# junfeng-chen/position_induced_transformer

Hardware: AMD Instinct MI355X
Metric: PiT fwd+bwd samples/sec on Darcy2D (higher is better)
Workload: dtype f32; 1 GPU; darcy2d 43x43 grid->16x16 latent, pit_fixed hid64 H2 blocks4 loc0.02, RelL2 (train_darcy.py:64-111), fwd+loss+bwd, per-GPU batch 8; per_gpu_batch=8, global_batch=8, parallelism=single, launch=hipgraph, head_scale_route=host

## Files before the change

include/pit_hip.h:

```cpp
#ifndef PIT_HIP_H
#define PIT_HIP_H

#ifdef __cplusplus
extern "C" {
#endif

#define PIT_ABI_VERSION 31
#define PIT_MAX_SPACE_DIM 8
#define PIT_DSCALE_SLOTS 1024

#define PIT_METRIC_EUCLID     0
#define PIT_METRIC_PERIODIC1D 1
#define PIT_METRIC_PERIODIC2D 2

#define PIT_ERR_NULL     -1
#define PIT_ERR_SIZE     -2
#define PIT_ERR_METRIC   -3
#define PIT_ERR_UNSUPPORTED -4

int pit_version(void);
const char* pit_error_string(int code);

#define PIT_MATH_FP32 0
#define PIT_MATH_BF16 1
// ... 33 lines not shown
                   const float* head, int n_head, int head_is_scale,
                   const float* stats, float rank_w, int masked, int self_attn,
                   float* out, long ld_out, long out_bstride, int out_col0, int copy_inputs,
                   float* rowstat, float* scale_out,
                   const int* nbr_idx, const int* nbr_cnt, int nbr_cap, int coord_dims, int math_mode, void* stream);

struct pit_mlp_params_job;

struct pit_block_weights_job {
    const float* mesh; int n_pts, space_dim, metric; float period;
    int n_layers; const float* const* heads; int head_is_scale, n_head;
    float *e, *q, *inv, *rowstat, *scale_out;
};
int pit_posatt_fwd_job(const float* mesh_out, const float* mesh_in, int mesh_batch, int n_out, int n_in,
                       int space_dim, int metric, float period,
                       const float* values, int batch, int dim, long ld_values, long values_bstride,
                       const float* head, int n_head, int head_is_scale,
                       const float* stats, float rank_w, int masked, int self_attn,
                       float* out, long ld_out, long out_bstride, int out_col0, int copy_inputs,
                       float* rowstat, float* scale_out,
                       const int* nbr_idx, const int* nbr_cnt, int nbr_cap, int coord_dims, int math_mode, void* stream,
                       const struct pit_block_weights_job* job);

typedef struct pit_mlp_params_job {
    const float* x; long ldx; int rows, n0, n1, n2; const float* h; int out_gelu;
    const float* d_y; long ld_dy;
    float *d_w1, *d_b1, *d_w2, *d_b2; int accumulate; const float* scratch; int math_mode;
} pit_mlp_params_job;
#define PIT_HEAD_ACCUMULATE 1
#define PIT_HEAD_DEFER      2
#define PIT_HEAD_IS_SCALE   4
int pit_posatt_bwd(const float* mesh_out, const float* mesh_in, int mesh_batch, int n_out, int n_in,
                   int space_dim, int metric, float period,
                   const float* values, int batch, int dim, long ld_values, long values_bstride,
                   const float* head, int n_head, int head_is_scale, const float* scale,
                   const float* rowstat, int masked,
                   const float* d_out, long ld_dout, long dout_bstride, int out_col0,
                   float* d_values, long ld_dvalues, long dvalues_bstride, int add_residual,
                   float* d_head, int accumulate_head, double* workspace,
                   const int* nbr_idx, const int* nbr_cnt, int nbr_cap, int nbr_complete,
                   const int* rev_ptr, const int* rev_row, const pit_mlp_params_job* rider,
                   int coord_dims, int math_mode, void* stream);

int pit_posatt_dmesh(const float* mesh_out, const float* mesh_in, int mesh_batch, int n_out, int n_in,
                     int space_dim, int metric, float period,
                     const float* values, int batch, int dim, long ld_values, long values_bstride,
                     const float* head, int n_head, int head_is_scale, const float* scale,
                     const float* rowstat, int masked,
                     const float* d_out, long ld_dout, long dout_bstride, int out_col0,
                     const int* nbr_idx, const int* nbr_cnt, int nbr_cap, int nbr_complete,
                     const int* rev_ptr, const int* rev_row,
                     float* d_mesh_out, float* d_mesh_in, int accumulate, void* workspace, void* stream);
long pit_posatt_dmesh_workspace(int mesh_batch, int n_out, int n_in, int space_dim, int batch, int n_head);

int pit_posatt_dhead_finish(int n_layers, double* const* workspaces, float* const* d_heads,
                            const float* const* heads, const float* const* scales, const int* n_heads,
                            const int* flags, const pit_mlp_params_job* rider, void* stream);

int pit_block_supported(int n_pts, int n_head, int dim, int batch);

int pit_block_weights(const float* mesh, int n_pts, int space_dim, int metric, float period, int n_layers,
                      const float* const* heads, int head_is_scale, int n_head, float* e, float* q,
                      float* inv, float* rowstat, float* scale_out, void* stream);

int pit_block_fwd(const float* e, const float* inv, int n_pts, int n_head, int dim, int batch, float* xcat,
                  const float* w1, const float* b1, const float* w2, const float* b2, int out_gelu,
                  float* z1, float* h, float* z2, float* y, long ldy, int math_mode, void* stream);

int pit_block_bwd(const float* e, const float* inv, const float* qw, int n_pts, int n_head, int dim, int batch,
                  const float* d_xcat, const float* xcat, double* dscale,
                  const float* w1, const float* w2, const float* z1, const float* z2, int out_gelu, int n0_prev,
                  float* d_xprev, long ld_dxprev, float* scratch_prev,
                  float* d_values, long ld_dvalues,
                  const struct pit_mlp_params_job* rider, const struct pit_mlp_params_job* rider2,
                  int math_mode, void* stream);

#define PIT_SLAB_UNION_MAX 64
typedef struct pit_slab_plan {
    int n_out, n_in, cap, n_slabs, umax;
    const float* stats; float rank_w;
    const int* idx; const int* cnt;
    const float* m; const unsigned short* slot; const int* keys; const int* nkeys;
    int rows;
} pit_slab_plan;
int pit_slab_plan_build(const float* mesh_out, const float* mesh_in, int n_out, int n_in, int space_dim, int metric, float period,
                        const int* nbr_idx, const int* nbr_cnt, int cap, int rows_per_slab, float* m, unsigned short* slot,
                        int* keys, int* nkeys, int* report, void* stream);
int pit_edge_supported(int n_head, int dim, int batch, int rows_per_sample);
int pit_decoder_weights(const pit_slab_plan* plan, const float* head, int head_is_scale, int n_head, int max_union, int max_count,
                        float* pw, float* qw, float* scale_out, const float* w1, float* w1f, int dim, void* stream);
typedef struct pit_decoder_weights_job {
    const pit_slab_plan* plan; const float* head; int head_is_scale, n_head, max_union, max_count;
    float *pw, *qw, *scale_out;
    const float* w1; float* w1f; int dim;
} pit_decoder_weights_job;
int pit_decoder_fwd(const pit_slab_plan* plan, const float* values, long ld_values, long values_bstride, int batch,
                    int n_head, int dim, const float* pw,
                    const float* w1, const float* w1f, const float* b1, const float* w2, const float* b2, int n2,
                    float* x, float* z1, float* h, float* y, float* zero_buf, long zero_n,
                    const float* loss_true, const float* loss_scale, const float* loss_shift, int loss_p, double* loss_part,
                    int max_union, void* stream);
int pit_decoder_bwd(const pit_slab_plan* plan, const float* values, long ld_values, long values_bstride, int batch,
                    int n_head, int dim, const float* pw, const float* qw,
                    const float* w1, const float* w2, int n2, const float* z1,
                    const float* d_y, long ld_dy, float* dz1, float* d_values, long dvalues_bstride, double* dscale,
                    const float* loss_pred, const float* loss_true, const float* loss_scale, const float* loss_shift,
                    const float* loss_seed, int loss_p, const double* loss_part, float* d_pred, float* loss_out,
                    float* norms_out, int max_union, void* stream);
int pit_union_att_supported(int n_head, int dim, int batch, int rows_per_sample);
int pit_union_att_fwd(const pit_slab_plan* plan, const float* values, long ld_values, long values_bstride, int batch,
                      int n_head, int dim, const float* pw, void* out, long ld_out, long out_bstride, int out_bf16,
                      int max_union, void* stream);
int pit_union_att_bwd(const pit_slab_plan* plan, const float* values, long ld_values, long values_bstride, int batch,
                      int n_head, int dim, const float* pw, const float* qw,
                      const void* d_out, long ld_dout, long dout_bstride, int dout_bf16,
                      float* d_values, long ld_dvalues, long dvalues_bstride, double* dscale, int max_union, void* stream);
int pit_fold_supported(int n_head, int dim, int batch, int rows_per_sample, int n_in);
int pit_fold_weights(const pit_slab_plan* plan, const float* head, int head_is_scale, int n_head, int max_union, int max_count,
                     float* pw, float* qw, float* scale_out, unsigned short* pw16, unsigned short* qw16, void* stream);
int pit_fold_att_fwd(const pit_slab_plan* plan, const float* vw, long ld_vw, long vw_bstride, int batch, int n_head, int dim,
                     const void* pw, void* z, long ld_z, long z_bstride, int max_union, int math_mode, void* stream);
int pit_fold_att_bwd(const pit_slab_plan* plan, const float* vw, long ld_vw, long vw_bstride, int batch, int n_head, int dim,
                     const void* pw, const void* qw, const void* dz, long ld_dz, long dz_bstride,
                     float* d_vw, long ld_dvw, long dvw_bstride, double* dscale,
                     float* tiles, const int* rev_ptr, const int* rev_ent, int max_union, int math_mode, void* stream);
int pit_thin_tail_scratch_floats(void);
int pit_thin_tail_fwd(const void* z, long ldz, int rows, int n1, int n2, const float* b1, const float* w2, const float* b2,
                      float* y, long ldy, int math_mode, void* stream);
int pit_thin_tail_bwd(const void* z, long ldz, int rows, int n1, int n2, const float* b1, const float* w2,
                      const float* d_y, long ld_dy, void* dz, long ld_dz, float* d_b1, float* d_w2, float* d_b2,
                      float* scratch, int math_mode, void* stream);
int pit_linear_fwd(const float* x, long ldx, int rows, int n_in, int n_out, const float* w, const float* zero_bias,
                   float* y, long ldy, int math_mode, void* stream);
int pit_linear_bwd(const float* x, long ldx, int rows, int n_in, int n_out, const float* w, const float* d_y, long ld_dy,
                   float* d_x, long ld_dx, float* d_w, int accumulate, int math_mode, void* stream);

struct pit_block_weights_job;
int pit_encoder_fwd(const pit_slab_plan* plan, const float* mesh_in, int space_dim, int coord_dims,
                    const float* values, long ld_values, long values_bstride, int value_dim, int batch,
                    int n_head, int dim, const float* head, int head_is_scale,
                    const float* w1, const float* b1, const float* w2, const float* b2,
                    float* x, float* z1, float* h, float* z2, float* y, long ldy, float* rowstat, float* scale_out,
                    float* clear_buf, long clear_n, const struct pit_block_weights_job* weights,
                    const pit_decoder_weights_job* dec_weights, void* stream);
int pit_encoder_bwd(const pit_slab_plan* plan, const float* mesh_in, int space_dim, int coord_dims,
                    const float* values, long ld_values, long values_bstride, int value_dim, int batch,
                    int n_head, int dim, const float* scale, const float* rowstat,
                    const float* w1, const float* w2, const float* z1, const float* z2,
                    const float* d_y, long ld_dy, float* scratch, double* dscale, void* stream);

int pit_posatt_pre_supported(int n_pts, int n_head, int dim, int batch);
int pit_posatt_pre_fwd(const float* e, const float* rowstat, int n_pts, int n_head, int dim, int batch,
                       const float* values, long ld_values, long values_bstride,
                       float* out, long ld_out, long out_bstride, int out_col0, int copy_inputs, int math_mode, void* stream);
int pit_posatt_pre_bwd(const float* e, const float* q, const float* rowstat, int n_pts, int n_head, int dim, int batch,
                       const float* values, long ld_values, long values_bstride,
                       const float* d_out, long ld_dout, long dout_bstride, int out_col0,
                       float* d_values, long ld_dvalues, long dvalues_bstride, int add_residual,
                       double* workspace, int math_mode, void* stream);

int pit_satt_supported(int n_pts, int n_head, int dim, int batch, int mesh_batch);
int pit_satt_fwd(const float* mesh, int mesh_batch, int n_pts, int space_dim, int metric, float period,
                 const float* values, long ld_values, long values_bstride, int batch, int dim,
                 const float* head, int n_head, int head_is_scale, unsigned short* x16,
                 float* out, long ld_out, long out_bstride, int out_col0, int copy_inputs,
                 float* rowstat, float* scale_out, unsigned short* e_tiles, int x16_ready, void* stream);
int pit_satt_bwd(const float* mesh, int mesh_batch, int n_pts, int space_dim, int metric, float period,
                 int batch, int dim, const float* scale, int n_head, const float* rowstat,
                 const unsigned short* x16, unsigned short* g16,
                 const float* d_out, long ld_dout, long dout_bstride, int out_col0,
                 float* d_values, long ld_dvalues, long dvalues_bstride, int add_residual, double* dscale,
// ... 203 lines not shown
```

position_induced_transformer_amd/_lib.py:

```python
from __future__ import annotations

import ctypes
import os

import torch

_HERE = os.path.dirname(os.path.abspath(__file__))
LIB_PATH = os.environ.get("PIT_LIB_PATH") or os.path.join(_HERE, "csrc", "libpit_hip.so")

_P = ctypes.c_void_p
_I = ctypes.c_int
_L = ctypes.c_long
_F = ctypes.c_float

class MlpParamsJob(ctypes.Structure):
    _fields_ = [("x", _P), ("ldx", _L), ("rows", _I), ("n0", _I), ("n1", _I), ("n2", _I), ("h", _P), ("out_gelu", _I),
                ("d_y", _P), ("ld_dy", _L), ("d_w1", _P), ("d_b1", _P), ("d_w2", _P), ("d_b2", _P),
                ("accumulate", _I), ("scratch", _P), ("math_mode", _I)]


class BlockWeightsJob(ctypes.Structure):
    _fields_ = [("mesh", _P), ("n_pts", _I), ("space_dim", _I), ("metric", _I), ("period", _F),
                ("n_layers", _I), ("heads", _P), ("head_is_scale", _I), ("n_head", _I),
                ("e", _P), ("q", _P), ("inv", _P), ("rowstat", _P), ("scale_out", _P)]


class SlabPlan(ctypes.Structure):
    _fields_ = [("n_out", _I), ("n_in", _I), ("cap", _I), ("n_slabs", _I), ("umax", _I), ("stats", _P), ("rank_w", _F),
                ("idx", _P), ("cnt", _P), ("m", _P), ("slot", _P), ("keys", _P), ("nkeys", _P), ("rows", _I)]


class DecoderWeightsJob(ctypes.Structure):
    _fields_ = [("plan", _P), ("head", _P), ("head_is_scale", _I), ("n_head", _I), ("max_union", _I), ("max_count", _I),
                ("pw", _P), ("qw", _P), ("scale_out", _P), ("w1", _P), ("w1f", _P), ("dim", _I)]


SIGNATURES = {
    "pit_version": [],
    "pit_error_string": [_I],
    "pit_head_scale": [_P, _I, _P, _P],
    "pit_select_fwd": [_P, _P, _I, _I, _I, _I, _I, _F, _I, _I, _P, _P],
    "pit_select_wide_fwd": [_P, _P, _I, _I, _I, _I, _I, _F, _I, _I, _P, _P],
    "pit_plan_fwd": [_P, _P, _I, _I, _I, _I, _I, _F, _I, _P, _I, _P, _P, _P, _P, _P, _I, _P],
    "pit_lists_transpose": [_P, _P, _I, _I, _I, _I, _P, _P, _P, _P],
    "pit_neighbors_fwd": [_P, _P, _I, _I, _I, _I, _I, _F, _P, _I, _P, _P, _P, _P, _P, _P],
    "pit_posatt_fwd": [_P, _P, _I, _I, _I, _I, _I, _F,
                       _P, _I, _I, _L, _L,
                       _P, _I, _I,
                       _P, _F, _I, _I,
                       _P, _L, _L, _I, _I,
                       _P, _P, _P, _P, _I, _I, _I, _P],
    "pit_posatt_fwd_job": [_P, _P, _I, _I, _I, _I, _I, _F,
                           _P, _I, _I, _L, _L,
                           _P, _I, _I,
                           _P, _F, _I, _I,
                           _P, _L, _L, _I, _I,
                           _P, _P, _P, _P, _I, _I, _I, _P, _P],
    "pit_posatt_bwd": [_P, _P, _I, _I, _I, _I, _I, _F,
                       _P, _I, _I, _L, _L,
                       _P, _I, _I, _P,
                       _P, _I,
                       _P, _L, _L, _I,
                       _P, _L, _L, _I,
                       _P, _I, _P, _P, _P, _I, _I, _P, _P, _P, _I, _I, _P],
    "pit_posatt_dmesh": [_P, _P, _I, _I, _I, _I, _I, _F,
                         _P, _I, _I, _L, _L,
                         _P, _I, _I, _P,
                         _P, _I,
                         _P, _L, _L, _I,
                         _P, _P, _I, _I, _P, _P,
                         _P, _P, _I, _P, _P],
    "pit_posatt_dmesh_workspace": [_I, _I, _I, _I, _I, _I],
    "pit_posatt_dhead_finish": [_I, _P, _P, _P, _P, _P, _P, _P, _P],
    "pit_block_supported": [_I, _I, _I, _I],
    "pit_block_weights": [_P, _I, _I, _I, _F, _I, _P, _I, _I, _P, _P, _P, _P, _P, _P],
    "pit_block_fwd": [_P, _P, _I, _I, _I, _I, _P, _P, _P, _P, _P, _I, _P, _P, _P, _P, _L, _I, _P],
    "pit_slab_plan_build": [_P, _P, _I, _I, _I, _I, _F, _P, _P, _I, _I, _P, _P, _P, _P, _P, _P],
    "pit_fold_supported": [_I, _I, _I, _I, _I],
    "pit_fold_weights": [_P, _P, _I, _I, _I, _I, _P, _P, _P, _P, _P, _P],
    "pit_fold_att_fwd": [_P, _P, _L, _L, _I, _I, _I, _P, _P, _L, _L, _I, _I, _P],
    "pit_fold_att_bwd": [_P, _P, _L, _L, _I, _I, _I, _P, _P, _P, _L, _L, _P, _L, _L, _P, _P, _P, _P, _I, _I, _P],
    "pit_thin_tail_scratch_floats": [],
    "pit_thin_tail_fwd": [_P, _L, _I, _I, _I, _P, _P, _P, _P, _L, _I, _P],
    "pit_thin_tail_bwd": [_P, _L, _I, _I, _I, _P, _P, _P, _L, _P, _L, _P, _P, _P, _P, _I, _P],
    "pit_satt_supported": [_I, _I, _I, _I, _I],
    "pit_satt_fwd": [_P, _I, _I, _I, _I, _F, _P, _L, _L, _I, _I, _P, _I, _I, _P, _P, _L, _L, _I, _I, _P, _P, _P, _I, _P],
    "pit_satt_bwd": [_P, _I, _I, _I, _I, _F, _I, _I, _P, _I, _P, _P, _P, _P, _L, _L, _I, _P, _L, _L, _I, _P, _P, _I, _P, _P],
    "pit_satt_tiles_elems": [_I],
    "pit_mlp_chain_supported": [_I, _I, _I, _I],
    "pit_mlp_chain_fwd": [_P, _L, _I, _I, _I, _P, _P, _P, _P, _P, _P, _P, _P, _L, _P, _P],
    "pit_mlp_chain_bwd": [_I, _I, _I, _P, _P, _P, _P, _P, _L, _P, _L, _P, _P, _P, _I, _I, _P],
    "pit_cast_bf16_multi": [_I, _P, _P, _P, _P],
    "pit_linear_fwd": [_P, _L, _I, _I, _I, _P, _P, _P, _L, _I, _P],
    "pit_linear_bwd": [_P, _L, _I, _I, _I, _P, _P, _L, _P, _L, _P, _I, _I, _P],
    "pit_edge_supported": [_I, _I, _I, _I],
    "pit_decoder_weights": [_P, _P, _I, _I, _I, _I, _P, _P, _P, _P, _P, _I, _P],
    "pit_decoder_fwd": [_P, _P, _L, _L, _I, _I, _I, _P, _P, _P, _P, _P, _P, _I, _P, _P, _P, _P, _P, _L,
                        _P, _P, _P, _I, _P, _I, _P],
    "pit_decoder_bwd": [_P, _P, _L, _L, _I, _I, _I, _P, _P, _P, _P, _I, _P, _P, _L, _P, _P, _L, _P,
                        _P, _P, _P, _P, _P, _I, _P, _P, _P, _P, _I, _P],
    "pit_union_att_supported": [_I, _I, _I, _I],
    "pit_union_att_fwd": [_P, _P, _L, _L, _I, _I, _I, _P, _P, _L, _L, _I, _I, _P],
    "pit_union_att_bwd": [_P, _P, _L, _L, _I, _I, _I, _P, _P, _P, _L, _L, _I, _P, _L, _L, _P, _I, _P],
    "pit_encoder_fwd": [_P, _P, _I, _I, _P, _L, _L, _I, _I, _I, _I, _P, _I, _P, _P, _P, _P,
                        _P, _P, _P, _P, _P, _L, _P, _P, _P, _L, _P, _P, _P],
    "pit_encoder_bwd": [_P, _P, _I, _I, _P, _L, _L, _I, _I, _I, _I, _P, _P, _P, _P, _P, _P, _P, _L, _P, _P, _P],
    "pit_posatt_pre_supported": [_I, _I, _I, _I],
    "pit_posatt_pre_fwd": [_P, _P, _I, _I, _I, _I, _P, _L, _L, _P, _L, _L, _I, _I, _I, _P],
    "pit_posatt_pre_bwd": [_P, _P, _P, _I, _I, _I, _I, _P, _L, _L, _P, _L, _L, _I, _P, _L, _L, _I, _P, _I, _P],
    "pit_block_bwd": [_P, _P, _P, _I, _I, _I, _I, _P, _P, _P, _P, _P, _P, _P, _I, _I, _P, _L, _P, _P, _L, _P, _P, _I, _P],
    "pit_mlp_bf16_io_supported": [_I, _I, _I, _I, _I],
    "pit_mlp_fwd": [_P, _L, _I, _I, _I, _I, _P, _P, _P, _P, _I, _P, _P, _P, _P, _L, _I, _P],
    "pit_mlp_bwd": [_P, _L, _I, _I, _I, _I, _P, _P, _P, _P, _P, _I, _P, _L,
                    _P, _L, _P, _P, _P, _P, _I, _P, _I, _P],
    "pit_mlp_bwd_data": [_I, _I, _I, _I, _P, _P, _P, _P, _I, _P, _L, _P, _L, _P, _I, _P],
    "pit_mlp_bwd_params": [_P, _L, _I, _I, _I, _I, _P, _I, _P, _L, _P, _P, _P, _P, _I, _P, _I, _P],
    "pit_mlp_bwd_params_ordered": [_P, _L, _I, _I, _I, _I, _P, _I, _P, _L, _P, _P, _P, _P, _I, _P, _P, _P],
    "pit_mlp_bwd_params_ordered_workspace": [_I, _I, _I, _I],
    "pit_mlp_bwd_params_ordered_mfma": [_P, _L, _I, _I, _I, _I, _P, _I, _P, _L, _P, _P, _P, _P, _I, _P, _P, _P],
    "pit_mlp_bwd_params_ordered_mfma_workspace": [_I, _I, _I, _I],
    "pit_lists_sort_ranges": [_P, _P, _I, _I, _L, _P, _P],
    "pit_posatt_overflow_dv_ordered": [_P, _P, _I, _I, _I, _I, _I, _F, _I, _I, _P, _I, _I, _P, _P,
                                       _P, _L, _L, _I, _P, _L, _L, _P, _I, _I, _P],
    "pit_mlp_bwd_params_deferrable": [_I, _I, _I, _I, _I, _L],
    "pit_rel_lp_loss_fwd": [_P, _P, _P, _P, _I, _I, _I, _I, _P, _P, _P, _P],
    "pit_rel_lp_loss_fwd_grad": [_P, _P, _P, _P, _I, _I, _I, _I, _P, _P, _P, _P, _P, _P, _L, _P],
    "pit_rel_lp_loss_fwd_grad_ordered": [_P, _P, _P, _P, _I, _I, _I, _I, _P, _P, _P, _P, _P, _P, _L, _P],
    "pit_rel_lp_loss_bwd": [_P, _P, _P, _P, _I, _I, _I, _I, _P, _P, _P, _P, _P],
    "pit_plan_ragged_fwd": [_P, _P, _I, _I, _I, _I, _P, _P, _F, _I, _P, _P, _I, _P, _P, _P],
    "pit_posatt_ragged_fwd": [_P, _P, _I, _I, _I, _I, _P, _P,
                              _P, _I, _L, _L,
                              _P, _I, _I,
                              _P, _P, _I,
                              _P, _L, _L, _I, _I,
                              _P, _P, _P, _P, _I, _I, _P],
    "pit_posatt_ragged_bwd": [_P, _P, _I, _I, _I, _I, _P, _P,
                              _P, _I, _L, _L,
                              _P, _I, _I, _P,
                              _P, _I,
                              _P, _L, _L, _I,
                              _P, _L, _L, _I,
                              _P, _I, _P, _P, _P, _I, _P, _P, _I, _P],
    "pit_plan_ragged_strided_fwd": [_P, _P, _I, _I, _I, _I, _L, _L, _P, _P, _F, _I, _P, _P, _I, _P, _P, _P],
    "pit_posatt_ragged_strided_fwd": [_P, _P, _I, _I, _I, _I, _L, _L, _P, _P,
                                      _P, _I, _L, _L,
                                      _P, _I, _I,
                                      _P, _P, _I,
                                      _P, _L, _L, _I, _I,
                                      _P, _P, _P, _P, _I, _I, _P],
    "pit_posatt_ragged_strided_bwd": [_P, _P, _I, _I, _I, _I, _L, _L, _P, _P,
                                      _P, _I, _L, _L,
                                      _P, _I, _I, _P,
                                      _P, _I,
                                      _P, _L, _L, _I,
                                      _P, _L, _L, _I,
                                      _P, _I, _P, _P, _P, _I, _P, _P, _I, _P],
    "pit_rel_lp_loss_ragged_fwd": [_P, _P, _P, _I, _I, _I, _I, _P, _P, _P],
    "pit_rel_lp_loss_ragged_bwd": [_P, _P, _P, _I, _I, _I, _I, _P, _P, _P, _P],
    "pit_distmat_select_fwd": [_P, _L, _L, _I, _I, _I, _I, _I, _P, _P],
    "pit_distmat_fwd": [_P, _L, _L, _I, _I,
# ... 63 lines not shown
```

position_induced_transformer_amd/csrc/pit_edge.hip:

```cpp
#include "pit_common.h"
#include "pit_gemm_rd.h"
#include "pit_block_dev.h"

#ifndef PIT_EDGE_MAX_ROWS
#define PIT_EDGE_MAX_ROWS (1 << 20)
#endif
#ifndef PIT_EDGE_DBG
#define PIT_EDGE_DBG 0
#endif

namespace {

#if PIT_EDGE_DBG & 0x100
__device__ unsigned long long pit_edge_stamps[4][16];
#define ESTAMP(k_, i_) do { if (blockIdx.x == 300 && threadIdx.x == 0) pit_edge_stamps[k_][i_] = __builtin_amdgcn_s_memtime(); } while (0)
#else
#define ESTAMP(k_, i_) do { } while (0)
#endif

constexpr int ER = 16;
constexpr int EU = PIT_SLAB_UNION_MAX;

__device__ __forceinline__ __amdgpu_buffer_rsrc_t wide_rsrc(const void* p) { return make_rsrc(p, 0x7ffffff0u); }
constexpr unsigned OOB = 0x7ffffff8u;
__device__ __forceinline__ float ldg_if(const float* p, long i, bool ok) {
    return buf_load(wide_rsrc(p), ok ? (unsigned)(i * 4) : OOB);
}
__device__ __forceinline__ int ldi_if(const int* p, long i, bool ok) {
    return __builtin_amdgcn_raw_buffer_load_b32(wide_rsrc(p), (int)(ok ? (unsigned)(i * 4) : OOB), 0, 0);
}
__device__ __forceinline__ float4 ldg4_if(const float* p, long i, bool ok) {
    float v[4];
    buf_load4(wide_rsrc(p), ok ? (unsigned)(i * 4) : OOB, v);
    return make_float4(v[0], v[1], v[2], v[3]);
}

__device__ __forceinline__ float pow_abs_p(float x, int p) {
    const float ax = fabsf(x);
    return p == 1 ? ax : ax * ax;
}

struct SlabBuildArgs {
    const float *mesh_out, *mesh_in;
    int n_out, n_in, sdim, used, periodic; float period;
    const int *idx, *cnt; int cap, umax;
    float* m; unsigned short* slot; int* keys; int* nkeys; int* report;
    int er;
};

__global__ __launch_bounds__(256) void slab_plan_kernel(SlabBuildArgs a) {
    __shared__ unsigned bm[512];
    __shared__ int pref[513];
    const int tid = threadIdx.x, slab = blockIdx.x;
    const int nwords = (a.n_in + 31) >> 5;
    for (int w = tid; w < nwords; w += 256) bm[w] = 0u;
    __syncthreads();
    const int er = a.er;
    const int total = er * a.cap;
    for (int e = tid; e < total; e += 256) {
        const int r = e / a.cap, i = e - r * a.cap;
        const int row = slab * er + r;
        float mv = 0.0f;
        if (row < a.n_out) {
            const int c = a.cnt[row];
            if (c > a.cap && i == 0) atomicMax(a.report + 1, 1);
            if (i == 0) atomicMax(a.report + 2, min(c, a.cap));
            if (i < min(c, a.cap)) {
                const int j = a.idx[(long)row * a.cap + i];
                const float* xo = a.mesh_out + (long)row * a.sdim;
                const float* xi = a.mesh_in + (long)j * a.sdim;
                mv = sq_dist3(xo[0], a.used > 1 ? xo[1] : 0.0f, a.used > 2 ? xo[2] : 0.0f,
                              xi[0], a.used > 1 ? xi[1] : 0.0f, a.used > 2 ? xi[2] : 0.0f, a.periodic != 0, a.period);
                atomicOr(&bm[j >> 5], 1u << (j & 31));
            }
        }
        a.m[(long)(slab * er + r) * a.cap + i] = mv;
    }
    __syncthreads();
    if (tid == 0) {
        int run = 0;
        for (int w = 0; w < nwords; ++w) { pref[w] = run; run += __popc(bm[w]); }
        pref[nwords] = run;
        a.nkeys[slab] = run;
        atomicMax(a.report, run);
    }
    __syncthreads();
    const int nk = pref[nwords];
    for (int w = tid; w < nwords; w += 256) {
        unsigned bits = bm[w];
        int s = pref[w];
        while (bits) {
            const int bpos = __ffs(bits) - 1;
            bits &= bits - 1u;
            if (s < a.umax) a.keys[(long)slab * a.umax + s] = w * 32 + bpos;
            ++s;
        }
    }
    for (int s = nk + tid; s < a.umax; s += 256) a.keys[(long)slab * a.umax + s] = 0;
    for (int e = tid; e < total; e += 256) {
        const int r = e / a.cap, i = e - r * a.cap;
        const int row = slab * er + r;
        int s = 0;
        if (row < a.n_out && i < min(a.cnt[row], a.cap)) {
            const int j = a.idx[(long)row * a.cap + i];
            s = pref[j >> 5] + __popc(bm[j >> 5] & ((1u << (j & 31)) - 1u));
        }
        a.slot[(long)(slab * er + r) * a.cap + i] = (unsigned short)min(s, 65535);
    }
}

template <int H>
__device__ __forceinline__ void head_scales(const float (&raw)[H], int is_scale, float (&c)[H]) {
#pragma unroll
    for (int h = 0; h < H; ++h) c[h] = is_scale ? raw[h] : head_scale_from_lmda(raw[h]);
}

struct DecWArgs {
    pit_slab_plan p;
    const float* head; int head_is_scale, n_head, um, lpr;
    float *pw, *qw, *scale_out;
    unsigned short *pw16, *qw16;
    const float* w1; float* w1f; int dim;
    int rb;
};
__device__ __forceinline__ float seg_sum_rt(float v, int lpr) {
    v += dpp_f<0xB1, 0xf>(v);
    v += dpp_f<0x4E, 0xf>(v);
    v += dpp_f<0x124, 0xf>(v);
    v += dpp_f<0x128, 0xf>(v);
    if (lpr >= 32) v += __shfl_xor(v, 16, 64);
    if (lpr >= 64) v += __shfl_xor(v, 32, 64);
    return v;
}
__device__ __forceinline__ void dec_weights_body(const DecWArgs& g, int slab, float* tile) {
    const pit_slab_plan& p = g.p;
    const int tid = threadIdx.x, lane = tid & 63, wave = tid >> 6;
    const int H = g.n_head, um = g.um, lpr = g.lpr;
    const int per = H * ER * um;
    for (int e = tid; e < 2 * per; e += 256) tile[e] = 0.0f;
    float c[2];
#pragma unroll
    for (int h = 0; h < 2; ++h) {
        const float raw = g.head[h < H ? h : 0];
        c[h] = g.head_is_scale ? raw : head_scale_from_lmda(raw);
    }
    __syncthreads();
    const int rpw = 64 / lpr;
    for (int r0 = 0; r0 < ER; r0 += 4 * rpw) {
        const int row_l = r0 + wave * rpw + lane / lpr, i = lane % lpr, n = slab * ER + row_l;
        const int craw = ldi_if(p.cnt, n, n < p.n_out);
        const long off = (long)(slab * ER + row_l) * p.cap + (i < p.cap ? i : 0);
        const float m = p.m[off];
        const int slot = p.slot[off];
        const bool valid = i < min(craw, p.cap);
        const int nn = n < p.n_out ? n : p.n_out - 1;
        const float mk = p.stats[nn], mk1 = p.stats[p.n_out + nn], mmin = p.stats[2 * (long)p.n_out + nn];
        for (int h = 0; h < H; ++h) {
            const float T = quantile_lerp(__fmul_rn(c[h], mk), __fmul_rn(c[h], mk1), p.rank_w);
            const float smin = __fmul_rn(c[h], mmin);
            const float sv = __fmul_rn(m, c[h]);
            const bool keep = valid && sv <= T;
            const float pv = keep ? __expf(smin - sv) : 0.0f;
            const float rs = seg_sum_rt(pv, lpr), qsum = seg_sum_rt(pv * m, lpr);
            const float inv = rs > 0.0f ? 1.0f / rs : 0.0f;
            if (valid && slot < um) {
                tile[(h * ER + row_l) * um + slot] = pv * inv;
                tile[per + (h * ER + row_l) * um + slot] = pv * inv * (m - qsum * inv);
            }
        }
    }
    __syncthreads();
    {
        const int gpb = g.rb / ER, blk = slab / gpb, cg = slab - blk * gpb, perh = ER * um;
        for (int e = 4 * tid; e < per; e += 4 * 256) {
            const int h = e / perh, r = e - h * perh;
            const long o = ((long)(blk * H + h) * g.rb + cg * ER) * um + r;
            const float4 pv4 = *reinterpret_cast<const float4*>(tile + e), qv4 = *reinterpret_cast<const float4*>(tile + per + e);
            *reinterpret_cast<float4*>(g.pw + o) = pv4;
            if (g.qw) *reinterpret_cast<float4*>(g.qw + o) = qv4;
            if (g.pw16) *reinterpret_cast<uint2*>(g.pw16 + o) = make_uint2((unsigned)f_to_bf16(pv4.x) | ((unsigned)f_to_bf16(pv4.y) << 16), (unsigned)f_to_bf16(pv4.z) | ((unsigned)f_to_bf16(pv4.w) << 16));
            if (g.qw16) *reinterpret_cast<uint2*>(g.qw16 + o) = make_uint2((unsigned)f_to_bf16(qv4.x) | ((unsigned)f_to_bf16(qv4.y) << 16), (unsigned)f_to_bf16(qv4.z) | ((unsigned)f_to_bf16(qv4.w) << 16));
        }
    }
    if (slab == 0 && tid < H && g.scale_out) g.scale_out[tid] = c[tid];
    if (g.w1f) {
        const int K0 = H * g.dim, KS = K0 / 16, n4 = g.dim * K0 / 4;
        for (int o = slab * 256 + tid; o < n4; o += p.n_slabs * (g.rb / ER) * 256) {
            const int ln = o & 63, s_ = (o >> 6) % KS, w = (o >> 6) / KS;
            reinterpret_cast<float4*>(g.w1f)[o] =
                *reinterpret_cast<const float4*>(g.w1 + (long)(16 * w + (ln & 15)) * K0 + 16 * s_ + 4 * (ln >> 4));
        }
    }
}
__global__ __launch_bounds__(256) void decoder_weights_kernel(DecWArgs g) {
    __shared__ __attribute__((aligned(16))) float tile[2 * 2 * ER * EU];
    dec_weights_body(g, blockIdx.x, tile);
}

struct DecFwdArgs {
    pit_slab_plan p;
    const float* values; long ld_values, values_bstride; int batch;
    const float* pw;
    const float *w1, *b1, *w2, *b2; int n2;
    const float* w1f;
    float *x, *z1, *h, *y;
    float* zero_buf; long zero_n;
    const float *tru, *lscale, *lshift; int loss_p; double* lpart;
    int um;
};

template <int D>
__device__ __forceinline__ void union_keys(const pit_slab_plan& p, int slab, int tid, int nkup, int (&key)[EU / 16]) {
    const int r0 = tid / (D / 4);
    const int* kp = p.keys + (long)slab * p.umax + r0;
#pragma unroll
    for (int u = 0; u < EU / 16; ++u) key[u] = kp[16 * u];
}
template <int D>
__device__ __forceinline__ void gather_union(const float* __restrict__ vb, long ldv, const int (&key)[EU / 16], int nk, int nkup, int tid,
                                             float4 (&uv)[EU / 16]) {
    const int r0 = tid / (D / 4), q = tid % (D / 4);
#pragma unroll
    for (int u = 0; u < EU / 16; ++u)
        uv[u] = (PIT_EDGE_DBG & 2) ? make_float4(0.f, 0.f, 0.f, 0.f) : ldg4_if(vb, (long)key[u] * ldv + 4 * q, r0 + 16 * u < nk);
}
template <int D>
__device__ __forceinline__ void park_union(float* ut, int nkup, int tid, const float4 (&uv)[EU / 16]) {
    const int r0 = tid / (D / 4), q = tid % (D / 4);
#pragma unroll
    for (int u = 0; u < EU / 16; ++u)
        if (16 * u < nkup) *reinterpret_cast<float4*>(ut + (r0 + 16 * u) * (D + 4) + 4 * q) = uv[u];
}

constexpr int WCP = (2 * ER * EU / 4 + 255) / 256;
template <int NT>
__device__ __forceinline__ void wtile_request(const float* tile, int npc, int tid, float4 (&cp)[WCP * 256 / NT]) {
#pragma unroll
    for (int u = 0; u < WCP * 256 / NT; ++u) cp[u] = ldg4_if(tile, 4L * (tid + u * NT), tid + u * NT < npc);
}
template <int NT>
__device__ __forceinline__ void wtile_park(float* lds, int um, int npc, int tid, const float4 (&cp)[WCP * 256 / NT]) {
#pragma unroll
    for (int u = 0; u < WCP * 256 / NT; ++u) {
        const int e = tid + u * NT;
        if (e < npc) *reinterpret_cast<float4*>(lds + ((4 * e) / um) * (um + 4) + (4 * e) % um) = cp[u];
    }
}
template <int D>
__device__ __forceinline__ f32x4_t tile_times_union(const float* wrow, int up, const float* ut, int nkup, int wave, int l15, int kq) {
    f32x4_t a0 = {0.f, 0.f, 0.f, 0.f}, a1 = {0.f, 0.f, 0.f, 0.f};
    for (int s = 0; s < nkup / 16; ++s) {
        const float4 a = *reinterpret_cast<const float4*>(wrow + l15 * up + 16 * s + 4 * kq);
        const float* bp = ut + (16 * s + 4 * kq) * (D + 4) + 16 * wave + l15;
        a0 = mfma_16x16x4(a.x, bp[0], a0);
        a1 = mfma_16x16x4(a.y, bp[D + 4], a1);
        a0 = mfma_16x16x4(a.z, bp[2 * (D + 4)], a0);
        a1 = mfma_16x16x4(a.w, bp[3 * (D + 4)], a1);
    }
    f32x4_t r;
#pragma unroll
    for (int i = 0; i < 4; ++i) r[i] = a0[i] + a1[i];
    return r;
}

template <int H, int D, bool LOSS>
__global__ __launch_bounds__(4 * D) void decoder_fwd_kernel(DecFwdArgs g) {
    constexpr int NT = 4 * D, NW = D / 16, K0 = H * D, KS = K0 / 16, XP = K0 + 4, HP = D + 4;
    extern __shared__ __attribute__((aligned(16))) float smem[];
    const int UP = g.um + 4;
    float* pt = smem;
    float* ut = pt + H * ER * UP;
    float* xs = ut + g.um * (D + 4);
    float* hs = xs + ER * XP;
    float* w2s = hs + ER * HP;
    const int tid = threadIdx.x, lane = tid & 63, wave = tid >> 6;
    const int l15 = lane & 15, kq = lane >> 4;
    const pit_slab_plan& p = g.p;
    int b, slab;
    if (!slab_of_xcd(blockIdx.x, g.batch, p.n_slabs, b, slab)) return;
    const int nk = min(p.nkeys[slab], EU), nkup = (nk + 15) & ~15;
    const long row0 = (long)b * p.n_out + slab * ER;
    const int c1 = wave * 16 + l15;
    ESTAMP(0, 0);
    int key[EU / 16];
    union_keys<D>(p, slab, tid, nkup, key);
    const int npc = H * ER * g.um / 4;
    float4 pcp[WCP * 256 / NT];
    wtile_request<NT>(g.pw + (long)slab * H * ER * g.um, npc, tid, pcp);
    float4 bv[KS];
    const float* w1base = g.w1f ? g.w1f : g.w1;
#pragma unroll
    for (int s = 0; s < KS; ++s)
        bv[s] = (PIT_EDGE_DBG & 1) ? make_float4(1.f, 2.f, 3.f, 4.f)
              : *reinterpret_cast<const float4*>(w1base + (g.w1f ? ((wave * KS + s) * 64 + lane) * 4 : c1 * K0 + 16 * s + 4 * kq));
    const float bias1 = g.b1[c1];
    const float w2r = ldg_if(g.w2, tid, tid < g.n2 * D);
    const float b2r = ldg_if(g.b2, tid, tid < g.n2);
    float l_t0 = 0.0f, l_sc0 = 1.0f, l_sh0 = 0.0f;
    if (LOSS) {
        const int n = slab * ER + l15;
        const bool rv = n < p.n_out;
        l_t0 = ldg_if(g.tru, (row0 + l15) * g.n2, rv);
        const bool aff = rv && g.lscale != nullptr;
        l_sc0 = ldg_if(g.lscale, (long)n * g.n2, aff);
        l_sh0 = ldg_if(g.lshift, (long)n * g.n2, aff);
    }
    float4 uv[EU / 16];
    gather_union<D>(g.values + (long)b * g.values_bstride, g.ld_values, key, nk, nkup, tid, uv);
    __builtin_amdgcn_sched_barrier(0);
    ESTAMP(0, 1);
    w2s[tid] = w2r;
    if (tid < 4) w2s[4 * D + tid] = b2r;
    wtile_park<NT>(pt, g.um, npc, tid, pcp);
    ESTAMP(0, 2);
    park_union<D>(ut, nkup, tid, uv);
    ESTAMP(0, 3);
    __syncthreads();
    ESTAMP(0, 4);
#pragma unroll
    for (int h = 0; h < H; ++h) {
        const f32x4_t o = tile_times_union<D>(pt + h * ER * UP, UP, ut, nkup, wave, l15, kq);
#pragma unroll
        for (int i = 0; i < 4; ++i) xs[(4 * kq + i) * XP + h * D + c1] = o[i];
    }
    ESTAMP(0, 5);
    __syncthreads();
    ESTAMP(0, 6);
    if (g.x && !(PIT_EDGE_DBG & 4)) {
#pragma unroll
        for (int u = 0; u < (ER * K0 / 4 + NT - 1) / NT; ++u) {
            const int e = tid + u * NT, r = e / (K0 / 4), q = e % (K0 / 4);
            if (e < ER * K0 / 4 && slab * ER + r < p.n_out)
                *reinterpret_cast<float4*>(g.x + (row0 + r) * K0 + 4 * q) = *reinterpret_cast<const float4*>(xs + r * XP + 4 * q);
        }
    }
    {
        f32x4_t a0 = {0.f, 0.f, 0.f, 0.f}, a1 = {0.f, 0.f, 0.f, 0.f};
#pragma unroll
        for (int s = 0; s < KS; ++s) {
            const float4 a = *reinterpret_cast<const float4*>(xs + l15 * XP + 16 * s + 4 * kq);
            a0 = mfma_16x16x4(a.x, bv[s].x, a0);
            a1 = mfma_16x16x4(a.y, bv[s].y, a1);
            a0 = mfma_16x16x4(a.z, bv[s].z, a0);
            a1 = mfma_16x16x4(a.w, bv[s].w, a1);
        }
#pragma unroll
        for (int i = 0; i < 4; ++i) {
            const int r = 4 * kq + i;
            const float z = a0[i] + a1[i] + bias1;
            hs[r * HP + c1] = gelu_erf(z);
            if (g.z1 && slab * ER + r < p.n_out && !(PIT_EDGE_DBG & 4)) g.z1[(row0 + r) * D + c1] = z;
        }
    }
    ESTAMP(0, 7);
    __syncthreads();
    ESTAMP(0, 8);
    if (g.h && !(PIT_EDGE_DBG & (4 | 1024))) {
        const int r = tid / (D / 4), q = tid % (D / 4);
        if (slab * ER + r < p.n_out)
            *reinterpret_cast<float4*>(g.h + (row0 + r) * D + 4 * q) = *reinterpret_cast<const float4*>(hs + r * HP + 4 * q);
    }
    if (wave != 0) {
        if (g.zero_buf) {
            const long wgs = (long)g.batch * p.n_slabs, me = (long)b * p.n_slabs + slab;
            const long per = ((g.zero_n + wgs - 1) / wgs + 3) & ~3L;
            const long beg = me * per, end = min(g.zero_n, beg + per);
            for (long e = beg + 4 * (tid - 64); e < end; e += 4 * (NT - 64)) {
                if (e + 4 <= end) *reinterpret_cast<float4*>(g.zero_buf + e) = make_float4(0.f, 0.f, 0.f, 0.f);
                else for (long q = e; q < end; ++q) g.zero_buf[q] = 0.0f;
            }
        }
        return;
    }
    const int n = slab * ER + l15;
    const bool rv = n < p.n_out;
#pragma unroll
    for (int o = 0; o < 4; ++o) {
        if (o >= g.n2) break;
        float part = 0.0f;
#pragma unroll
        for (int k = 0; k < D / 4; k += 4) {
            const float4 a = *reinterpret_cast<const float4*>(hs + l15 * HP + kq * (D / 4) + k);
            const float4 w = *reinterpret_cast<const float4*>(w2s + o * D + kq * (D / 4) + k);
            part += (a.x * w.x + a.y * w.y) + (a.z * w.z + a.w * w.w);
        }
        part += __shfl_xor(part, 16, 64);
        part += __shfl_xor(part, 32, 64);
        const float pred = part + w2s[4 * D + o];
        if (kq == 0 && rv) g.y[(row0 + l15) * g.n2 + o] = pred;
        if (LOSS) {
            double num = 0.0, den = 0.0;
            float t = l_t0, sc = l_sc0, sh = l_sh0;
            if (o > 0) {
                t = ldg_if(g.tru, (row0 + l15) * g.n2 + o, rv);
                sc = ldg_if(g.lscale, (long)n * g.n2 + o, rv && g.lscale != nullptr);
                sh = ldg_if(g.lshift, (long)n * g.n2 + o, rv && g.lscale != nullptr);
            }
            if (kq == 0 && rv) {
                const float q = g.lscale ? pred * sc + sh : pred;
                num = (double)pow_abs_p(t - q, g.loss_p);
                den = (double)pow_abs_p(t, g.loss_p);
            }
            num = wave_sum_d(num);
            den = wave_sum_d(den);
            if (lane == 0) {
                double* dst = g.lpart + (((long)b * g.n2 + o) * p.n_slabs + slab) * 2;
                dst[0] = num; dst[1] = den;
            }
        }
    }
    ESTAMP(0, 9);
}

struct DecBwdArgs {
    pit_slab_plan p;
    const float* values; long ld_values, values_bstride; int batch;
    const float *pw, *qw;
    const float *w1, *w2; int n2;
    const float* z1;
    const float* d_y; long ld_dy;
    float* dz1;
    float* d_values; long dvalues_bstride;
    double* dscale;
    const float *pred, *tru, *lscale, *lshift, *gseed; int loss_p; const double* lpart; float* d_pred; float* loss_out; float* norms_out;
    int um;
};

__device__ __forceinline__ void series_norms(const double* lpart, int b, int o, int n2, int slabs, int p, int lane, double& nn, double& dn) {
    double num = 0.0, den = 0.0;
    const double* src = lpart + ((long)b * n2 + o) * slabs * 2;
    for (int s = lane; s < slabs; s += 64) { num += src[2 * s]; den += src[2 * s + 1]; }
    num = wave_sum_d(num);
    den = wave_sum_d(den);
    nn = p == 1 ? num : sqrt(num);
    dn = p == 1 ? den : sqrt(den);
}

template <int H, int D, bool LOSS>
__global__ __launch_bounds__(4 * D) void decoder_bwd_kernel(DecBwdArgs g) {
    constexpr int NT = 4 * D, NW = D / 16, K0 = H * D, S1 = D / 16, XP = K0 + 4, P1 = D + 4;
    extern __shared__ __attribute__((aligned(16))) float smem[];
    const int UP = g.um + 4;
    float* ps_ = smem;
    float* qs = ps_ + H * ER * UP;
    float* ut = qs + H * ER * UP;
    float* ds1 = ut + g.um * (D + 4);
    float* dxs = ds1 + ER * P1;
    double* wred = reinterpret_cast<double*>(dxs + ER * XP);
    int* keys_s = reinterpret_cast<int*>(wred + NW * H);
    const int tid = threadIdx.x, lane = tid & 63, wave = tid >> 6;
    const int l15 = lane & 15, kq = lane >> 4;
    const pit_slab_plan& p = g.p;
    int b, slab;
    if (!slab_of_xcd(blockIdx.x, g.batch, p.n_slabs, b, slab)) return;
    const int nk = min(p.nkeys[slab], EU), nkup = (nk + 15) & ~15;
    const long row0 = (long)b * p.n_out + slab * ER;
    const int c1 = wave * 16 + l15;

    ESTAMP(1, 0);
    int key[EU / 16];
    union_keys<D>(p, slab, tid, nkup, key);
    const int akey = p.keys[(long)slab * p.umax + (tid & (EU - 1))];
    const int npc = H * ER * g.um / 4;
    float4 pcp[WCP * 256 / NT], qcp[WCP * 256 / NT];
    wtile_request<NT>(g.pw + (long)slab * H * ER * g.um, npc, tid, pcp);
    wtile_request<NT>(g.qw + (long)slab * H * ER * g.um, npc, tid, qcp);
    const int ec = tid % D;
    float z1v[4], dyv[4], prv[4], trv[4], lsc[4], lsh[4];
    const float w2c0 = g.w2[ec];
#pragma unroll
    for (int u = 0; u < 4; ++u) {
        const int r = (tid + u * NT) / D;
        const bool ok = slab * ER + r < p.n_out;
        z1v[u] = ldg_if(g.z1, (row0 + r) * D + ec, ok);
        dyv[u] = 0.0f; prv[u] = 0.0f; trv[u] = 0.0f; lsc[u] = 1.0f; lsh[u] = 0.0f;
        if (!LOSS) {
            dyv[u] = ldg_if(g.d_y, (row0 + r) * g.ld_dy, ok);
        } else {
            prv[u] = ldg_if(g.pred, (row0 + r) * g.n2, ok);
            trv[u] = ldg_if(g.tru, (row0 + r) * g.n2, ok);
            const bool aff = ok && g.lscale != nullptr;
            const float a = ldg_if(g.lscale, (long)(slab * ER + r) * g.n2, aff), bq = ldg_if(g.lshift, (long)(slab * ER + r) * g.n2, aff);
            lsc[u] = g.lscale ? a : 1.0f;
            lsh[u] = bq;
        }
    }
    float4 np4[4];
#pragma unroll
    for (int cq = 0; cq < 4; ++cq)
        np4[cq] = ldg4_if(reinterpret_cast<const float*>(g.lpart) + (long)b * g.n2 * p.n_slabs * 4, 4L * (lane + 64 * cq),
                          LOSS && lane + 64 * cq < p.n_slabs);
    float4 uv[EU / 16];
    gather_union<D>(g.values + (long)b * g.values_bstride, g.ld_values, key, nk, nkup, tid, uv);
    __builtin_amdgcn_sched_barrier(0);
    ESTAMP(1, 1);
    if (tid < EU) keys_s[tid] = akey;
    float nrm0 = 0.0f, nrm1 = 1.0f;
    if (LOSS) {
        {
            double num = 0.0, den = 0.0;
#pragma unroll
            for (int cq = 0; cq < 4; ++cq) {
                num += __hiloint2double(__float_as_int(np4[cq].y), __float_as_int(np4[cq].x));
                den += __hiloint2double(__float_as_int(np4[cq].w), __float_as_int(np4[cq].z));
            }
            const double* src = g.lpart + (long)b * g.n2 * p.n_slabs * 2;
            for (int sl = lane + 256; sl < p.n_slabs; sl += 64) { num += src[2 * sl]; den += src[2 * sl + 1]; }
            num = wave_sum_d(num);
            den = wave_sum_d(den);
            nrm0 = (float)(g.loss_p == 1 ? num : sqrt(num));
            nrm1 = (float)(g.loss_p == 1 ? den : sqrt(den));
        }
        if (blockIdx.x == 0 && wave == NW - 1) {
            double tot = 0.0;
            for (int bb = 0; bb < g.batch; ++bb)
                for (int o = 0; o < g.n2; ++o) {
                    double nn, dn;
                    series_norms(g.lpart, bb, o, g.n2, p.n_slabs, g.loss_p, lane, nn, dn);
                    tot += (double)((float)(nn / dn / g.n2));
                    if (lane == 0 && g.norms_out) {
                        g.norms_out[((long)bb * g.n2 + o) * 2] = (float)nn;
                        g.norms_out[((long)bb * g.n2 + o) * 2 + 1] = (float)dn;
                    }
                }
            if (lane == 0) *g.loss_out = (float)tot;
        }
    }
    ESTAMP(1, 2);
    wtile_park<NT>(ps_, g.um, npc, tid, pcp);
    wtile_park<NT>(qs, g.um, npc, tid, qcp);
    ESTAMP(1, 3);
    const float gs = (LOSS && g.gseed) ? g.gseed[0] : 1.0f;
    auto dpred = [&](float pr, float tr, float sc, float sh, float nn, float dn) {
        const float d = pr * sc + sh - tr;
        float dnorm;
        if (g.loss_p == 1) dnorm = (d > 0.0f) ? 1.0f : (d < 0.0f ? -1.0f : 0.0f);
        else dnorm = (nn > 0.0f) ? d / nn : 0.0f;
        return gs * dnorm * sc / (dn * g.n2);
    };
    float acc[4];
#pragma unroll
    for (int u = 0; u < 4; ++u) {
        const int r = (tid + u * NT) / D;
        const bool ok = slab * ER + r < p.n_out;
        float v = dyv[u];
        if (LOSS) {
            v = dpred(prv[u], trv[u], lsc[u], lsh[u], nrm0, nrm1);
            if (ec == 0 && ok) g.d_pred[(row0 + r) * g.n2] = v;
        }
        acc[u] = v * w2c0;
    }
    for (int o = 1; o < g.n2; ++o) {
        const float w2o = g.w2[(long)o * D + ec];
        float nn = 0.0f, dn = 1.0f;
        if (LOSS) {
            double a, bq;
            series_norms(g.lpart, b, o, g.n2, p.n_slabs, g.loss_p, lane, a, bq);
            nn = (float)a; dn = (float)bq;
        }
#pragma unroll
        for (int u = 0; u < 4; ++u) {
            const int r = (tid + u * NT) / D;
            const bool ok = slab * ER + r < p.n_out;
            float v;
            if (!LOSS) {
                v = ldg_if(g.d_y, (row0 + r) * g.ld_dy + o, ok);
            } else {
                const long e = (long)(slab * ER + r) * g.n2 + o;
                const bool aff = ok && g.lscale != nullptr;
                const float a = ldg_if(g.lscale, e, aff), bq = ldg_if(g.lshift, e, aff);
                v = dpred(ldg_if(g.pred, (row0 + r) * g.n2 + o, ok), ldg_if(g.tru, (row0 + r) * g.n2 + o, ok),
                          g.lscale ? a : 1.0f, bq, nn, dn);
                if (ec == o && ok) g.d_pred[(row0 + r) * g.n2 + o] = v;
            }
            acc[u] += v * w2o;
        }
    }
#pragma unroll
    for (int u = 0; u < 4; ++u) {
        const int r = (tid + u * NT) / D;
        const bool ok = slab * ER + r < p.n_out;
        const float v = ok ? acc[u] * ((PIT_EDGE_DBG & 32) ? 1.0f : gelu_erf_grad(z1v[u])) : 0.0f;
        ds1[r * P1 + ec] = v;
        if (ok && !(PIT_EDGE_DBG & 512)) g.dz1[(row0 + r) * D + ec] = v;
    }
    ESTAMP(1, 4);
    park_union<D>(ut, nkup, tid, uv);
    ESTAMP(1, 5);
    float w1v[H][S1][4];
#pragma unroll
    for (int hh = 0; hh < H; ++hh)
#pragma unroll
        for (int s = 0; s < S1; ++s)
#pragma unroll
            for (int e = 0; e < 4; ++e) w1v[hh][s][e] = (PIT_EDGE_DBG & 8) ? 0.5f
                : g.w1[(long)(16 * s + 4 * kq + e) * K0 + hh * D + c1];
    __syncthreads();
    ESTAMP(1, 6);
#pragma unroll
    for (int hh = 0; hh < H; ++hh) {
        f32x4_t o0 = {0.f, 0.f, 0.f, 0.f}, o1 = {0.f, 0.f, 0.f, 0.f};
#pragma unroll
        for (int s = 0; s < S1; ++s) {
            const float4 a = *reinterpret_cast<const float4*>(ds1 + l15 * P1 + 16 * s + 4 * kq);
            o0 = mfma_16x16x4(a.x, w1v[hh][s][0], o0);
            o1 = mfma_16x16x4(a.y, w1v[hh][s][1], o1);
            o0 = mfma_16x16x4(a.z, w1v[hh][s][2], o0);
            o1 = mfma_16x16x4(a.w, w1v[hh][s][3], o1);
        }
#pragma unroll
        for (int i = 0; i < 4; ++i) dxs[(4 * kq + i) * XP + hh * D + c1] = o0[i] + o1[i];
    }
    ESTAMP(1, 7);
    __syncthreads();
    ESTAMP(1, 8);
    for (int mt = 0; mt < nkup / 16; ++mt) {
        f32x4_t a0 = {0.f, 0.f, 0.f, 0.f}, a1 = {0.f, 0.f, 0.f, 0.f};
#pragma unroll
        for (int h = 0; h < H; ++h) {
            const float* ap = ps_ + (h * ER + 4 * kq) * UP + 16 * mt + l15;
            const float* bp = dxs + (4 * kq) * XP + h * D + c1;
            a0 = mfma_16x16x4(ap[0], bp[0], a0);
            a1 = mfma_16x16x4(ap[UP], bp[XP], a1);
            a0 = mfma_16x16x4(ap[2 * UP], bp[2 * XP], a0);
            a1 = mfma_16x16x4(ap[3 * UP], bp[3 * XP], a1);
        }
#pragma unroll
        for (int i = 0; i < 4; ++i) {
            const int s = 16 * mt + 4 * kq + i;
            if (s < nk && !(PIT_EDGE_DBG & 16)) atomicAdd(g.d_values + (long)b * g.dvalues_bstride + (long)keys_s[s] * D + c1, a0[i] + a1[i]);
        }
    }
    ESTAMP(1, 9);
    if (g.dscale && !(PIT_EDGE_DBG & 128)) {
#pragma unroll
        for (int h = 0; h < H; ++h) {
            const f32x4_t qu = tile_times_union<D>(qs + h * ER * UP, UP, ut, nkup, wave, l15, kq);
            double part = 0.0;
#pragma unroll
            for (int i = 0; i < 4; ++i) part += (double)qu[i] * (double)dxs[(4 * kq + i) * XP + h * D + c1];
            part = wave_sum_d(part);
            if (lane == 0) wred[wave * H + h] = part;
        }
        __syncthreads();
        if (tid < H) {
            double tot = 0.0;
            for (int w = 0; w < NW; ++w) tot += wred[w * H + tid];
            atomicAdd(g.dscale + (long)tid * PIT_DSCALE_SLOTS + ((int)blockIdx.x & (PIT_DSCALE_SLOTS - 1)), -tot);
        }
    }
    ESTAMP(1, 10);
}

struct EncArgs {
    pit_slab_plan p;
    const float* mesh_in; int sdim, kd;
    const float* values; long ld_values, values_bstride; int dv, batch;
    const float* head; int head_is_scale;
    const float *w1, *b1, *w2, *b2;
    float* x;
    float *z1, *h, *z2, *y; long ldy;
    float* rowstat; float* scale_out;
    float* clear_buf; long clear_n;
    int n_att;
    const float* d_y; long ld_dy; float* scratch; double* dscale;
};

// ... 344 lines not shown
    const int l15 = lane & 15, kq = lane >> 4;
    const pit_slab_plan& p = g.p;
    const int chunks = g.dim / D;
    const int chunk = (int)blockIdx.x % chunks;
    int b, slab;
    if (!slab_of_xcd((int)blockIdx.x / chunks, g.batch, p.n_slabs, b, slab)) return;
    const int nk = min(p.nkeys[slab], EU), nkup = (nk + 15) & ~15;
    const int c1 = wave * 16 + l15;
    int key[EU / 16];
    union_keys<D>(p, slab, tid, nkup, key);
    const int akey = p.keys[(long)slab * p.umax + (tid & (EU - 1))];
    const int npc = H * ER * g.um / 4;
    float4 pcp[WCP], qcp[WCP];
    wtile_request<NT>(g.pw + (long)slab * H * ER * g.um, npc, tid, pcp);
    wtile_request<NT>(g.qw + (long)slab * H * ER * g.um, npc, tid, qcp);
    float4 dv[H * ER * D / 4 / NT];
#pragma unroll
    for (int u = 0; u < H * ER * D / 4 / NT; ++u) {
        const int e = tid + u * NT, r = e / (H * D / 4), q4 = e % (H * D / 4), h = q4 / (D / 4), q = q4 % (D / 4);
        const int n = slab * ER + r;
        const long o = (long)b * g.dout_bstride + (long)n * g.ld_dout + (long)h * g.dim + chunk * D + 4 * q;
        if (g.dout16) {
            const __amdgpu_buffer_rsrc_t r16 = wide_rsrc(g.d_out);
            const unsigned off = n < p.n_out ? (unsigned)(o * 2) : OOB;
            const unsigned lo = (unsigned)__builtin_amdgcn_raw_buffer_load_b32(r16, (int)off, 0, 0);
            const unsigned hi = (unsigned)__builtin_amdgcn_raw_buffer_load_b32(r16, (int)(n < p.n_out ? off + 4u : OOB), 0, 0);
            dv[u] = make_float4(__uint_as_float(lo << 16), __uint_as_float(lo & 0xffff0000u), __uint_as_float(hi << 16),
                                __uint_as_float(hi & 0xffff0000u));
        } else {
            dv[u] = ldg4_if(reinterpret_cast<const float*>(g.d_out), o, n < p.n_out);
        }
    }
    float4 uv[EU / 16];
    gather_union<D>(g.values + (long)b * g.values_bstride + chunk * D, g.ld_values, key, nk, nkup, tid, uv);
    __builtin_amdgcn_sched_barrier(0);
    if (tid < EU) keys_s[tid] = akey;
    wtile_park<NT>(ps_, g.um, npc, tid, pcp);
    wtile_park<NT>(qs, g.um, npc, tid, qcp);
#pragma unroll
    for (int u = 0; u < H * ER * D / 4 / NT; ++u) {
        const int e = tid + u * NT, r = e / (H * D / 4), q4 = e % (H * D / 4);
        *reinterpret_cast<float4*>(dxs + r * XP + 4 * q4) = dv[u];
    }
    park_union<D>(ut, nkup, tid, uv);
    __syncthreads();
    if (g.d_values) {
        for (int mt = 0; mt < nkup / 16; ++mt) {
            f32x4_t a0 = {0.f, 0.f, 0.f, 0.f}, a1 = {0.f, 0.f, 0.f, 0.f};
#pragma unroll
            for (int h = 0; h < H; ++h) {
                const float* ap = ps_ + (h * ER + 4 * kq) * UP + 16 * mt + l15;
                const float* bp = dxs + (4 * kq) * XP + h * D + c1;
                a0 = mfma_16x16x4(ap[0], bp[0], a0);
                a1 = mfma_16x16x4(ap[UP], bp[XP], a1);
                a0 = mfma_16x16x4(ap[2 * UP], bp[2 * XP], a0);
                a1 = mfma_16x16x4(ap[3 * UP], bp[3 * XP], a1);
            }
#pragma unroll
            for (int i = 0; i < 4; ++i) {
                const int sl = 16 * mt + 4 * kq + i;
                if (sl < nk) atomicAdd(g.d_values + (long)b * g.dvalues_bstride + (long)keys_s[sl] * g.ld_dvalues + chunk * D + c1, a0[i] + a1[i]);
            }
        }
    }
    if (g.dscale) {
#pragma unroll
        for (int h = 0; h < H; ++h) {
            const f32x4_t qu = tile_times_union<D>(qs + h * ER * UP, UP, ut, nkup, wave, l15, kq);
            double part = 0.0;
#pragma unroll
            for (int i = 0; i < 4; ++i) part += (double)qu[i] * (double)dxs[(4 * kq + i) * XP + h * D + c1];
            part = wave_sum_d(part);
            if (lane == 0) wred[wave * H + h] = part;
        }
        __syncthreads();
        if (tid < H) {
            double tot = 0.0;
            for (int w = 0; w < NW; ++w) tot += wred[w * H + tid];
            atomicAdd(g.dscale + (long)tid * PIT_DSCALE_SLOTS + ((int)blockIdx.x & (PIT_DSCALE_SLOTS - 1)), -tot);
        }
    }
}

bool plan_ok(const pit_slab_plan* p, bool needs_union) {
    if (!p || !p->stats || !p->idx || !p->cnt || !p->m) return false;
    if (p->rows != ER) return false;
    if (p->n_out <= 0 || p->n_in <= 0 || p->cap <= 0 || p->cap > 64 || p->n_slabs != (p->n_out + ER - 1) / ER) return false;
    if (needs_union && (!p->slot || !p->keys || !p->nkeys || p->umax != EU)) return false;
    return true;
}
bool hid_ok(int n_head, int dim) { return (n_head == 1 || n_head == 2) && (dim == 32 || dim == 64); }

int union_slots(int max_union) { return max_union <= 32 ? 32 : (max_union <= 48 ? 48 : 64); }
template <int H, int D>
size_t dec_fwd_smem(int um) { return (size_t)(H * ER * (um + 4) + um * (D + 4) + ER * (H * D + 4) + ER * (D + 4) + 4 * D + 4) * 4; }
template <int H, int D>
size_t dec_bwd_smem(int um) {
    return (size_t)(2 * H * ER * (um + 4) + um * (D + 4) + ER * (D + 4) + ER * (H * D + 4)) * 4 + (size_t)(D / 16) * H * 8 + EU * 4;
}

}

extern "C" int pit_edge_supported(int n_head, int dim, int batch, int rows_per_sample) {
    if (!hid_ok(n_head, dim) || batch <= 0 || rows_per_sample <= 0) return 0;
    const long rows = (long)batch * rows_per_sample;
    return rows >= 256 && rows <= PIT_EDGE_MAX_ROWS;
}

extern "C" int pit_slab_plan_build(const float* mesh_out, const float* mesh_in, int n_out, int n_in, int space_dim, int metric,
                                   float period, const int* nbr_idx, const int* nbr_cnt, int cap, int rows_per_slab, float* m,
                                   unsigned short* slot, int* keys, int* nkeys, int* report, void* stream) {
    if (!mesh_out || !mesh_in || !nbr_idx || !nbr_cnt || !m || !slot || !keys || !nkeys || !report) return PIT_ERR_NULL;
    if (n_out <= 0 || n_in <= 0 || n_in > 16384 || space_dim < 1 || space_dim > 3 || cap <= 0) return PIT_ERR_SIZE;
    if (rows_per_slab != 16 && rows_per_slab != 64 && rows_per_slab != 128 && rows_per_slab != 256) return PIT_ERR_SIZE;
    if (metric < PIT_METRIC_EUCLID || metric > PIT_METRIC_PERIODIC2D) return PIT_ERR_METRIC;
    SlabBuildArgs a;
    a.mesh_out = mesh_out; a.mesh_in = mesh_in; a.n_out = n_out; a.n_in = n_in; a.sdim = space_dim;
    a.used = (metric == PIT_METRIC_PERIODIC1D) ? 1 : space_dim;
    a.periodic = metric != PIT_METRIC_EUCLID; a.period = period;
    a.idx = nbr_idx; a.cnt = nbr_cnt; a.cap = cap; a.umax = EU;
    a.m = m; a.slot = slot; a.keys = keys; a.nkeys = nkeys; a.report = report; a.er = rows_per_slab;
    hipLaunchKernelGGL(slab_plan_kernel, dim3((unsigned)((n_out + rows_per_slab - 1) / rows_per_slab)), dim3(256), 0, (hipStream_t)stream, a);
    PIT_CHECK_LAUNCH();
    return 0;
}

#define PIT_EDGE_DISPATCH(H_, D_, CALL_)                                         \
    do {                                                                         \
        if ((H_) == 1 && (D_) == 32) { CALL_(1, 32); }                           \
        else if ((H_) == 1) { CALL_(1, 64); }                                    \
        else if ((D_) == 32) { CALL_(2, 32); }                                   \
        else { CALL_(2, 64); }                                                   \
    } while (0)

namespace {
int fill_dec_weights(DecWArgs& g, const pit_slab_plan* plan, const float* head, int head_is_scale, int n_head, int max_union,
                     int max_count, float* pw, float* qw, float* scale_out, const float* w1, float* w1f, int dim) {
    if (!plan_ok(plan, true) || !head || !pw) return PIT_ERR_NULL;
    if ((w1 == nullptr) != (w1f == nullptr)) return PIT_ERR_NULL;
    if (w1f && (dim < 16 || dim % 16 != 0 || !aligned16(w1) || !aligned16(w1f))) return PIT_ERR_SIZE;
    g.w1 = w1; g.w1f = w1f; g.dim = dim; g.rb = ER;
    if ((n_head != 1 && n_head != 2) || max_union < 1 || max_union > EU || max_count < 1 || max_count > 64) return PIT_ERR_UNSUPPORTED;
    if (!aligned16(pw) || (qw && !aligned16(qw))) return PIT_ERR_SIZE;
    g.p = *plan; g.head = head; g.head_is_scale = head_is_scale; g.n_head = n_head; g.um = union_slots(max_union);
    g.lpr = max_count <= 16 ? 16 : (max_count <= 32 ? 32 : 64);
    g.pw = pw; g.qw = qw; g.scale_out = scale_out;
    return 0;
}
}

extern "C" int pit_decoder_weights(const pit_slab_plan* plan, const float* head, int head_is_scale, int n_head, int max_union,
                                   int max_count, float* pw, float* qw, float* scale_out, const float* w1, float* w1f, int dim,
                                   void* stream) {
    DecWArgs g = DecWArgs();
    if (int rc = fill_dec_weights(g, plan, head, head_is_scale, n_head, max_union, max_count, pw, qw, scale_out, w1, w1f, dim)) return rc;
    hipLaunchKernelGGL(decoder_weights_kernel, dim3((unsigned)plan->n_slabs), dim3(256), 0, (hipStream_t)stream, g);
    PIT_CHECK_LAUNCH();
    return 0;
}

extern "C" int pit_fold_weights(const pit_slab_plan* plan, const float* head, int head_is_scale, int n_head, int max_union,
                                int max_count, float* pw, float* qw, float* scale_out, unsigned short* pw16, unsigned short* qw16,
                                void* stream) {
    if (!plan || !plan->stats || !plan->idx || !plan->cnt || !plan->m || !plan->slot || !plan->keys || !plan->nkeys || !head || !pw)
        return PIT_ERR_NULL;
    if ((plan->rows != 64 && plan->rows != 128 && plan->rows != 256) || plan->umax != EU || plan->cap <= 0 || plan->cap > 64 ||
        plan->n_slabs != (plan->n_out + plan->rows - 1) / plan->rows) return PIT_ERR_SIZE;
    if ((n_head != 1 && n_head != 2) || max_union < 1 || max_union > EU || max_count < 1 || max_count > 64) return PIT_ERR_UNSUPPORTED;
    if (!aligned16(pw) || (qw && !aligned16(qw))) return PIT_ERR_SIZE;
    DecWArgs g = DecWArgs();
    g.p = *plan; g.head = head; g.head_is_scale = head_is_scale; g.n_head = n_head; g.um = union_slots(max_union);
    g.lpr = max_count <= 16 ? 16 : (max_count <= 32 ? 32 : 64);
    g.pw = pw; g.qw = qw; g.scale_out = scale_out; g.rb = plan->rows; g.pw16 = pw16; g.qw16 = qw16;
    hipLaunchKernelGGL(decoder_weights_kernel, dim3((unsigned)(plan->n_slabs * (plan->rows / ER))), dim3(256), 0, (hipStream_t)stream, g);
    PIT_CHECK_LAUNCH();
    return 0;
}

extern "C" int pit_decoder_fwd(const pit_slab_plan* plan, const float* values, long ld_values, long values_bstride, int batch,
                               int n_head, int dim, const float* pw,
                               const float* w1, const float* w1f, const float* b1, const float* w2, const float* b2, int n2,
                               float* x, float* z1, float* h, float* y, float* zero_buf, long zero_n,
                               const float* loss_true, const float* loss_scale, const float* loss_shift, int loss_p, double* loss_part,
                               int max_union, void* stream) {
    if (max_union < 1 || max_union > EU) return PIT_ERR_UNSUPPORTED;
    if (w1f && !aligned16(w1f)) return PIT_ERR_SIZE;
    if (!plan_ok(plan, true) || !values || !pw || !w1 || !b1 || !w2 || !b2 || !y) return PIT_ERR_NULL;
    if (!hid_ok(n_head, dim) || n2 < 1 || n2 > 4 || batch <= 0) return PIT_ERR_UNSUPPORTED;
    if ((z1 == nullptr) != (h == nullptr)) return PIT_ERR_NULL;
    if (ld_values % 4 || values_bstride % 4 || !aligned16(values) || !aligned16(w1) || !aligned16(pw) || (zero_buf && !aligned16(zero_buf)))
        return PIT_ERR_SIZE;
    if (loss_part && (!loss_true || (loss_p != 1 && loss_p != 2) || (loss_scale == nullptr) != (loss_shift == nullptr))) return PIT_ERR_UNSUPPORTED;
    DecFwdArgs g;
    g.p = *plan; g.values = values; g.ld_values = ld_values; g.values_bstride = values_bstride; g.batch = batch;
    g.pw = pw; g.w1 = w1; g.w1f = w1f; g.b1 = b1; g.w2 = w2; g.b2 = b2; g.n2 = n2;
    g.x = x; g.z1 = z1; g.h = h; g.y = y; g.zero_buf = zero_buf; g.zero_n = zero_buf ? zero_n : 0;
    g.tru = loss_true; g.lscale = loss_scale; g.lshift = loss_shift; g.loss_p = loss_p; g.lpart = loss_part;
    g.um = union_slots(max_union);
    const dim3 grid((unsigned)slab_grid(batch, plan->n_slabs));
    hipStream_t s = (hipStream_t)stream;
#define PIT_DF(H_, D_)                                                                                                                \
    do {                                                                                                                              \
        if (loss_part) hipLaunchKernelGGL((decoder_fwd_kernel<H_, D_, true>), grid, dim3(4 * D_), (dec_fwd_smem<H_, D_>(g.um)), s, g); \
        else hipLaunchKernelGGL((decoder_fwd_kernel<H_, D_, false>), grid, dim3(4 * D_), (dec_fwd_smem<H_, D_>(g.um)), s, g);          \
    } while (0)
    PIT_EDGE_DISPATCH(n_head, dim, PIT_DF);
#undef PIT_DF
    PIT_CHECK_LAUNCH();
    return 0;
}

extern "C" int pit_decoder_bwd(const pit_slab_plan* plan, const float* values, long ld_values, long values_bstride, int batch,
                               int n_head, int dim, const float* pw, const float* qw,
                               const float* w1, const float* w2, int n2, const float* z1,
                               const float* d_y, long ld_dy, float* dz1, float* d_values, long dvalues_bstride, double* dscale,
                               const float* loss_pred, const float* loss_true, const float* loss_scale, const float* loss_shift,
                               const float* loss_seed, int loss_p, const double* loss_part, float* d_pred, float* loss_out,
                               float* norms_out, int max_union, void* stream) {
    if (max_union < 1 || max_union > EU) return PIT_ERR_UNSUPPORTED;
    if (!plan_ok(plan, true) || !values || !pw || !qw || !w1 || !w2 || !z1 || !dz1 || !d_values) return PIT_ERR_NULL;
    if (!hid_ok(n_head, dim) || n2 < 1 || n2 > 4 || batch <= 0) return PIT_ERR_UNSUPPORTED;
    if (!d_y && (!loss_pred || !loss_true || !loss_part || !d_pred || !loss_out || (loss_p != 1 && loss_p != 2) ||
                 (loss_scale == nullptr) != (loss_shift == nullptr))) return PIT_ERR_NULL;
    if (d_y && ld_dy < n2) return PIT_ERR_SIZE;
    if (ld_values % 4 || values_bstride % 4 || !aligned16(values) || !aligned16(pw) || !aligned16(qw)) return PIT_ERR_SIZE;
    DecBwdArgs g;
    g.p = *plan; g.values = values; g.ld_values = ld_values; g.values_bstride = values_bstride; g.batch = batch;
    g.pw = pw; g.qw = qw; g.w1 = w1; g.w2 = w2; g.n2 = n2; g.z1 = z1; g.d_y = d_y; g.ld_dy = ld_dy;
    g.dz1 = dz1; g.d_values = d_values; g.dvalues_bstride = dvalues_bstride; g.dscale = dscale;
    g.pred = loss_pred; g.tru = loss_true; g.lscale = loss_scale; g.lshift = loss_shift; g.gseed = loss_seed; g.loss_p = loss_p;
    g.lpart = loss_part; g.d_pred = d_pred; g.loss_out = loss_out; g.norms_out = norms_out;
    g.um = union_slots(max_union);
    const dim3 grid((unsigned)slab_grid(batch, plan->n_slabs));
    hipStream_t s = (hipStream_t)stream;
#define PIT_DB(H_, D_)                                                                                                            \
    do {                                                                                                                          \
        if (!d_y) hipLaunchKernelGGL((decoder_bwd_kernel<H_, D_, true>), grid, dim3(4 * D_), (dec_bwd_smem<H_, D_>(g.um)), s, g);  \
        else hipLaunchKernelGGL((decoder_bwd_kernel<H_, D_, false>), grid, dim3(4 * D_), (dec_bwd_smem<H_, D_>(g.um)), s, g);      \
    } while (0)
    PIT_EDGE_DISPATCH(n_head, dim, PIT_DB);
#undef PIT_DB
    PIT_CHECK_LAUNCH();
    return 0;
}

namespace {
int fill_enc(EncArgs& g, const pit_slab_plan* plan, const float* mesh_in, int space_dim, int coord_dims, const float* values,
             long ld_values, long values_bstride, int dv, int batch, int n_head, int dim) {
    if (!plan_ok(plan, false) || !mesh_in || !values) return PIT_ERR_NULL;
    if (!hid_ok(n_head, dim) || batch <= 0 || space_dim < 1 || space_dim > 3 || coord_dims < 0 || coord_dims > space_dim || dv < 0 ||
        coord_dims + dv < 1 || coord_dims + dv > 8 || n_head * (coord_dims + dv) > 16) return PIT_ERR_UNSUPPORTED;
    g = EncArgs();
    g.p = *plan; g.mesh_in = mesh_in; g.sdim = space_dim; g.kd = coord_dims; g.values = values; g.ld_values = ld_values;
    g.values_bstride = values_bstride; g.dv = dv; g.batch = batch;
    return 0;
}
}

extern "C" int pit_encoder_fwd(const pit_slab_plan* plan, const float* mesh_in, int space_dim, int coord_dims,
                               const float* values, long ld_values, long values_bstride, int value_dim, int batch,
                               int n_head, int dim, const float* head, int head_is_scale,
                               const float* w1, const float* b1, const float* w2, const float* b2,
                               float* x, float* z1, float* h, float* z2, float* y, long ldy, float* rowstat, float* scale_out,
                               float* clear_buf, long clear_n, const pit_block_weights_job* weights,
                               const pit_decoder_weights_job* dec_weights, void* stream) {
    EncArgs g;
    if (int rc = fill_enc(g, plan, mesh_in, space_dim, coord_dims, values, ld_values, values_bstride, value_dim, batch, n_head, dim)) return rc;
    if (!head || !w1 || !b1 || !w2 || !b2 || !y) return PIT_ERR_NULL;
    if ((z1 == nullptr) != (h == nullptr) || ldy < dim || !aligned16(w2)) return PIT_ERR_SIZE;
    g.head = head; g.head_is_scale = head_is_scale; g.w1 = w1; g.b1 = b1; g.w2 = w2; g.b2 = b2;
    g.x = x; g.z1 = z1; g.h = h; g.z2 = z2; g.y = y; g.ldy = ldy; g.rowstat = rowstat; g.scale_out = scale_out;
    g.clear_buf = clear_n > 0 ? clear_buf : nullptr; g.clear_n = clear_n;
    g.n_att = slab_grid(batch, plan->n_slabs);
    WeightsArgs wa = WeightsArgs();
    int n_w = 0;
    bool own_launch = false;
    if (weights) {
        if (int rc = fill_weights_args(wa, weights->mesh, weights->n_pts, weights->space_dim, weights->metric, weights->period,
                                       weights->n_layers, weights->heads, weights->head_is_scale, weights->n_head, weights->e, weights->q,
                                       weights->inv, weights->rowstat, weights->scale_out)) return rc;
        if (dim == 64) n_w = block_weights_wgs(wa.n_layers, wa.n_head, wa.L); else own_launch = true;
    }
    DecWArgs da = DecWArgs();
    int n_dw = 0;
    if (dec_weights) {
        if (int rc = fill_dec_weights(da, dec_weights->plan, dec_weights->head, dec_weights->head_is_scale, dec_weights->n_head,
                                      dec_weights->max_union, dec_weights->max_count, dec_weights->pw, dec_weights->qw,
                                      dec_weights->scale_out, dec_weights->w1, dec_weights->w1f, dec_weights->dim)) return rc;
        if (dim == 64) n_dw = da.p.n_slabs;
    }
    const dim3 grid((unsigned)(g.n_att + n_w + n_dw));
    hipStream_t s = (hipStream_t)stream;
#define PIT_EF(H_, D_) do { if (coord_dims + value_dim <= 4) hipLaunchKernelGGL((encoder_fwd_kernel<H_, D_, 4>), grid, dim3(4 * D_), 0, s, g, wa, da, n_w); \
                            else hipLaunchKernelGGL((encoder_fwd_kernel<H_, D_, 8>), grid, dim3(4 * D_), 0, s, g, wa, da, n_w); } while (0)
    PIT_EDGE_DISPATCH(n_head, dim, PIT_EF);
#undef PIT_EF
    PIT_CHECK_LAUNCH();
    if (dec_weights && dim != 64)
        if (int rc = pit_decoder_weights(dec_weights->plan, dec_weights->head, dec_weights->head_is_scale, dec_weights->n_head,
                                         dec_weights->max_union, dec_weights->max_count, dec_weights->pw, dec_weights->qw,
                                         dec_weights->scale_out, dec_weights->w1, dec_weights->w1f, dec_weights->dim, stream)) return rc;
    if (own_launch)
        return pit_block_weights(weights->mesh, weights->n_pts, weights->space_dim, weights->metric, weights->period, weights->n_layers,
                                 weights->heads, weights->head_is_scale, weights->n_head, weights->e, weights->q, weights->inv,
                                 weights->rowstat, weights->scale_out, stream);
    return 0;
}

extern "C" int pit_encoder_bwd(const pit_slab_plan* plan, const float* mesh_in, int space_dim, int coord_dims,
                               const float* values, long ld_values, long values_bstride, int value_dim, int batch,
                               int n_head, int dim, const float* scale, const float* rowstat,
                               const float* w1, const float* w2, const float* z1, const float* z2,
                               const float* d_y, long ld_dy, float* scratch, double* dscale, void* stream) {
    EncArgs g;
    if (int rc = fill_enc(g, plan, mesh_in, space_dim, coord_dims, values, ld_values, values_bstride, value_dim, batch, n_head, dim)) return rc;
// ... 68 lines not shown
```

position_induced_transformer_amd/csrc/pit_fold.hip:

```cpp
#include "pit_common.h"
#include "pit_block_dev.h"

namespace {

constexpr int EU = PIT_SLAB_UNION_MAX;
constexpr int SR = 32;
constexpr int CW = 64;

typedef short v4s_t __attribute__((ext_vector_type(4)));
typedef short v8s_t __attribute__((ext_vector_type(8)));
typedef __bf16 v8bf_t __attribute__((ext_vector_type(8)));

__device__ __forceinline__ __amdgpu_buffer_rsrc_t wide_rsrc(const void* p) { return make_rsrc(p, 0x7ffffff0u); }
constexpr unsigned OOB = 0x7ffffff8u;
__device__ __forceinline__ float4 ldg4_if(const float* p, long i, bool ok) {
    float v[4];
    buf_load4(wide_rsrc(p), ok ? (unsigned)(i * 4) : OOB, v);
    return make_float4(v[0], v[1], v[2], v[3]);
}
__device__ __forceinline__ float4 ldh4_if(const void* p, long i, bool ok) {
    const __amdgpu_buffer_rsrc_t r = wide_rsrc(p);
    const unsigned off = ok ? (unsigned)(i * 2) : OOB;
    const unsigned lo = (unsigned)__builtin_amdgcn_raw_buffer_load_b32(r, (int)off, 0, 0);
    const unsigned hi = (unsigned)__builtin_amdgcn_raw_buffer_load_b32(r, (int)(ok ? off + 4u : OOB), 0, 0);
// ... 328 lines not shown
#pragma unroll
                for (int rt = 0; rt < NRT; ++rt)
                    acc[rt] = F::mma(F::rowfrag(qth, PP, 16 * (rt0 + rt), kg, l15, kq), bf, acc[rt]);
            }
#pragma unroll
            for (int rt = 0; rt < NRT; ++rt)
#pragma unroll
                for (int i = 0; i < 4; ++i)
                    part += (double)acc[rt][i] * (double)F::get(dt + (16 * (rt0 + rt) + 4 * kq + i) * VP + 16 * w4 + l15);
        }
        __syncthreads();
        if (more && !(PIT_FOLD_DBG & 8)) {
            wstore<BF, H, NTB>(pt, PP, g, tid, pr);
            wstore<BF, H, NTB>(qt, PP, g, tid, qr);
            dpark<BF, NTB>(dt, tid, dr);
        }
        __syncthreads();
    }
    if ((PIT_FOLD_DBG & 4) && accT[0][0] != 123.456f) return;
    constexpr int EW = CW * H, EP = EW + 4;
    float* ex = reinterpret_cast<float*>(smem_raw);
#pragma unroll
    for (int mt = 0; mt < NMT; ++mt)
#pragma unroll
        for (int i = 0; i < 4; ++i) ex[(16 * (mt0 + mt) + 4 * kq + i) * EP + (16 * w4 + l15) * H + hh] = accT[mt][i];
    if (want_scale) {
        const double sum = wave_sum_d(part);
        if (lane == 0) wred[wave] = sum;
    }
    __syncthreads();
    if (g.tiles) {
#pragma unroll
        for (int u = 0; u < EU * EW / 4 / NTB; ++u) {
            const int e = tid + NTB * u, sl = e / (EW / 4), q = e % (EW / 4);
            *reinterpret_cast<float4*>(g.tiles + ((long)(b * g.p.n_slabs + slab) * EU + sl) * ((long)g.dim * H) + (long)chunk * EW + 4 * q) =
                *reinterpret_cast<const float4*>(ex + sl * EP + 4 * q);
        }
    } else if (g.d_vw) {
        float* dst = g.d_vw + (long)b * g.dvw_bstride + (long)chunk * EW;
#pragma unroll
        for (int u = 0; u < EU * EW / NTB; ++u) {
            const int e = tid + NTB * u, sl = e / EW, c = e % EW;
            if (sl < nk) atomicAdd(dst + (long)keys_s[sl] * g.ld_dvw + c, ex[sl * EP + c]);
        }
    }
    if (want_scale && tid < H) {
        double tot = 0.0;
        if (H == 2) { for (int w = 0; w < 4; ++w) tot += wred[4 * tid + w]; }
        else { for (int w = 0; w < 8; ++w) tot += wred[w]; }
        atomicAdd(g.dscale + (long)tid * PIT_DSCALE_SLOTS + ((int)blockIdx.x & (PIT_DSCALE_SLOTS - 1)), -tot);
    }
}

__global__ __launch_bounds__(128) void fold_reduce_kernel(FoldArgs g, int n_head) {
    const long width = (long)g.dim * n_head;
    const int tpk = (int)(width / 4 < 128 ? width / 4 : 128), kpw = 128 / tpk;
    const int sub = (int)threadIdx.x / tpk, t = (int)threadIdx.x - sub * tpk;
    const long row = (long)blockIdx.x * kpw + sub;
    if (sub >= kpw || row >= (long)g.batch * g.p.n_in) return;
    const int b = (int)(row / g.p.n_in), key = (int)(row - (long)b * g.p.n_in);
    const int beg = g.rev_ptr[key], end = g.rev_ptr[key + 1];
    const float* tb = g.tiles + (long)b * g.p.n_slabs * EU * width;
    float* dst = g.d_vw + (long)b * g.dvw_bstride + (long)key * g.ld_dvw;
    for (long c = 4L * t; c < width; c += 4L * tpk) {
        float4 acc = make_float4(0.f, 0.f, 0.f, 0.f);
        for (int e = beg; e < end; ++e) {
            const float4 v = *reinterpret_cast<const float4*>(tb + (long)g.rev_ent[e] * width + c);
            acc.x += v.x; acc.y += v.y; acc.z += v.z; acc.w += v.w;
        }
        *reinterpret_cast<float4*>(dst + c) = acc;
    }
}

size_t fold_smem(int H, bool bf, int um, bool bwd) {
    const int es = bf ? 2 : 4, pade = bf ? 8 : 4, umk = bf ? ((um + 31) & ~31) : um;
    const size_t vt = (size_t)H * umk * (CW + pade) * es, wt = (size_t)H * SR * (umk + pade) * es;
    if (!bwd) return vt + wt + (size_t)SR * (CW + 4) * 4;
    return std::max(vt + 2 * wt + (size_t)SR * (CW + pade) * es + 8 * 8 + EU * 4, (size_t)EU * (CW * H + 4) * 4);
}

bool fold_plan_ok(const pit_slab_plan* p) {
    if (!p || !p->stats || !p->idx || !p->cnt || !p->m || !p->slot || !p->keys || !p->nkeys) return false;
    if (p->rows != 64 && p->rows != 128 && p->rows != 256) return false;
    return p->n_out > 0 && p->n_in > 0 && p->cap > 0 && p->cap <= 64 && p->umax == EU && p->n_slabs == (p->n_out + p->rows - 1) / p->rows;
}
int union_slots(int max_union) { return max_union <= 32 ? 32 : (max_union <= 48 ? 48 : 64); }

struct TailArgs {
    const void* z; long ldz; int rows, n1, n2;
    const float *b1, *w2, *b2;
    float* y; long ldy;
    const float* d_y; long ld_dy;
    void* dz; long ld_dz;
    float* acc;
    float *d_b1, *d_w2, *d_b2;
};
constexpr int TMAX = 4, TAIL_SLOTS = 16;

__device__ __forceinline__ float seg_sum(float v, int tpr) {
    v += dpp_f<0xB1, 0xf>(v);
    v += dpp_f<0x4E, 0xf>(v);
    v += dpp_f<0x124, 0xf>(v);
    v += dpp_f<0x128, 0xf>(v);
    if (tpr >= 32) v += __shfl_xor(v, 16, 64);
    if (tpr >= 64) v += __shfl_xor(v, 32, 64);
    return v;
}
template <bool Z16>
__device__ __forceinline__ float4 tail_load(const void* z, long i, bool ok) {
    return Z16 ? ldh4_if(z, i, ok) : ldg4_if(reinterpret_cast<const float*>(z), i, ok);
}
template <bool FAST>
__device__ __forceinline__ void gelu_pair(float t, float& a, float& gp) {
    if (FAST) {
        float e;
        const float cdf = normal_cdf_fast(t, e);
        a = t * cdf;
        gp = fmaf(t * 0.39894228040143267794f, e, cdf);
    } else {
        const float cdf = 0.5f * (1.0f + erff(t * 0.70710678118654752440f));
        const float pdf = 0.39894228040143267794f * __expf(-0.5f * t * t);
        a = t * cdf;
        gp = cdf + t * pdf;
    }
}
template <bool FAST>
__device__ __forceinline__ float gelu_one(float t) {
    if (FAST) { float e; return t * normal_cdf_fast(t, e); }
    return gelu_erf(t);
}

template <int N2, bool FAST, bool Z16>
__global__ __launch_bounds__(256, 4) void thin_tail_fwd_kernel(TailArgs g) {
    constexpr int U = 4;
    const int tpr = g.n1 / 4, rpw = 64 / tpr;
    const int lane = threadIdx.x & 63, q = lane % tpr, sub = lane / tpr, k = 4 * q;
    const long wave0 = ((long)blockIdx.x * blockDim.x + threadIdx.x) >> 6, nwaves = ((long)gridDim.x * blockDim.x) >> 6;
    const float4 bq = *reinterpret_cast<const float4*>(g.b1 + k);
    float4 w[N2];
    float b2v[N2];
#pragma unroll
    for (int o = 0; o < N2; ++o) {
        w[o] = o < g.n2 ? *reinterpret_cast<const float4*>(g.w2 + (long)o * g.n1 + k) : make_float4(0.f, 0.f, 0.f, 0.f);
        b2v[o] = o < g.n2 ? g.b2[o] : 0.0f;
    }
    const long stride = nwaves * rpw;
    for (long mbase = wave0 * rpw; mbase < g.rows; mbase += U * stride) {
        float4 zv[U];
#pragma unroll
        for (int u = 0; u < U; ++u) {
            const long m = mbase + u * stride + sub;
            zv[u] = tail_load<Z16>(g.z, m * g.ldz + k, m < g.rows);
        }
#pragma unroll
        for (int u = 0; u < U; ++u) {
            if (mbase + u * stride >= g.rows) break;
            const long m = mbase + u * stride + sub;
            const float a0 = gelu_one<FAST>(zv[u].x + bq.x), a1 = gelu_one<FAST>(zv[u].y + bq.y);
            const float a2 = gelu_one<FAST>(zv[u].z + bq.z), a3 = gelu_one<FAST>(zv[u].w + bq.w);
#pragma unroll
            for (int o = 0; o < N2; ++o) {
                float s = (a0 * w[o].x + a1 * w[o].y) + (a2 * w[o].z + a3 * w[o].w);
                s = seg_sum(s, tpr);
                if (q == 0 && m < g.rows && o < g.n2) g.y[m * g.ldy + o] = s + b2v[o];
            }
        }
    }
// ... 245 lines not shown
```

position_induced_transformer_amd/ops.py:

```python
from __future__ import annotations

import ctypes
import math
import os
import threading
from collections import OrderedDict
from typing import Optional

import numpy as np
import torch

from . import _lib

METRIC_ID = {"euclid": 0, "periodic1d": 1, "periodic2d": 2}
MAX_SPACE_DIM = 8

FUSED_GRAD_ACCUMULATION = True

SPARSE_MASKED = True

_DSCALE_WS = {}
_LOSS_WS = {}
_PINNED = []

# ... 198 lines not shown
def _dw_slices(job, parts: int):
    st = job[0]
    out, per = [], -(-st.rows // parts // 16) * 16
    for r0 in range(0, st.rows, per):
        n = min(per, st.rows - r0)
        out.append(_lib.MlpParamsJob(st.x + 4 * r0 * st.ldx, st.ldx, n, st.n0, st.n1, st.n2, st.h + 4 * r0 * st.n1, 0,
                                     st.d_y + 4 * r0 * st.ld_dy, st.ld_dy, st.d_w1, st.d_b1, st.d_w2, st.d_b2, 1,
                                     st.scratch + 4 * r0 * st.n1, st.math_mode))
    return out


def _dw_deferrable(rows: int, n0: int, n1: int, n2: int, out_gelu: int, ld_dy: int) -> bool:
    key = (rows, n0, n1, n2, out_gelu, ld_dy)
    v = _DEFERRABLE.get(key)
    if v is None:
        if len(_DEFERRABLE) > 4096:
            _DEFERRABLE.clear()
        v = _DEFERRABLE[key] = bool(_lib.lib().pit_mlp_bwd_params_deferrable(*key))
    return v


def mark_inplace_grad(param, grad_view) -> None:
    param._pit_grad_ptr = grad_view.data_ptr()


def _grad_slot(param) -> Optional[torch.Tensor]:
    if not FUSED_GRAD_ACCUMULATION or param is None:
        return None
    want = getattr(param, "_pit_grad_ptr", None)
    g = getattr(param, "grad", None)
    if want is None or g is None or g.data_ptr() != want:
        return None
    if not g.is_cuda or g.dtype != torch.float32 or not g.is_contiguous():
        return None
    if param._backward_hooks or getattr(param, "_post_accumulate_grad_hooks", None):
        return None
    return g


IO_X_BF16, IO_SAVE_BF16, IO_DX_BF16, IO_OUT_BF16, IO_DOUT_BF16 = 0x100, 0x200, 0x400, 0x800, 0x1000
BF16_STORAGE = os.environ.get("PIT_BF16_STORAGE", "1") != "0"


def mlp_bf16_io_supported(rows: int, n0: int, n1: int, n2: int) -> bool:
    return BF16_STORAGE and get_math_mode() == "bf16" and bool(_lib.lib().pit_mlp_bf16_io_supported(rows, n0, n1, n2, 0))


def _need_gpu_bf16_ok(t) -> None:
    if t is not None and not t.is_cuda:
        raise RuntimeError("position_induced_transformer_amd: the PiT hot path runs on the HIP device only; "
                           "got a CPU tensor (move the model and its inputs to 'cuda')")
    if t is not None and t.dtype not in (torch.float32, torch.bfloat16):
        raise RuntimeError(f"position_induced_transformer_amd: fp32 (or bf16-stored) tensor expected, got {t.dtype}")


def _need_gpu(*tensors) -> None:
    for t in tensors:
        if t is not None and not t.is_cuda:
            raise RuntimeError("position_induced_transformer_amd: the PiT hot path runs on the HIP device only; "
                               "got a CPU tensor (move the model and its inputs to 'cuda')")
        if t is not None and t.dtype != torch.float32:
            raise RuntimeError(f"position_induced_transformer_amd: fp32 tensors expected, got {t.dtype}")


def quantile_rank(locality: float, n_in: int):
    rank = np.float32(locality) * np.float32(n_in - 1)
    k = int(np.floor(rank))
    w = np.float32(rank - np.float32(k))
    return k, float(w)


def mesh_period(metric: str, mesh_in: torch.Tensor) -> float:
    if metric == "periodic1d":
        return float(torch.abs(mesh_in[1, 0] - mesh_in[0, 0]) * mesh_in.shape[0])
    if metric == "periodic2d":
        res = int(mesh_in.shape[0] ** 0.5)
        dx = (torch.max(mesh_in[:, 0]) - torch.min(mesh_in[:, 0])) / (res - 1)
        return float(dx * res)
    return 0.0


SLAB_UNION_MAX = 64
FOLD_SLAB_ROWS = (256, 128, 64)
PLAN_FLAGS = 0
UNION_TILES = os.environ.get("PIT_UNION_TILES", "auto")
UNION_DV = os.environ.get("PIT_UNION_DV", "auto")
_UNION_DECISIONS = {}
ATT_UNION = 0x2000


def as_lengths(lengths, device, batch: int) -> torch.Tensor:
    if torch.is_tensor(lengths):
        if lengths.dtype not in (torch.int32, torch.int64):
            raise TypeError(f"lengths must be an int32 or int64 tensor, got {lengths.dtype}")
        t = lengths.detach().reshape(-1)
        if t.dtype != torch.int32 or t.device != device or not t.is_contiguous():
            t = t.to(device=device, dtype=torch.int32).contiguous()
    else:
        t = torch.tensor([int(v) for v in lengths], dtype=torch.int32, device=device)
    if t.numel() != batch:
        raise ValueError(f"lengths must hold one entry per sample: {t.numel()} entries for a batch of {batch}")
    return t


RAGGED_LIST_CAP = None


def ragged_list_capacity(rank_k: int, n_in: int) -> int:
    if RAGGED_LIST_CAP is not None:
        return int(RAGGED_LIST_CAP)
    want = rank_k + 2
    cap = ((want + max(16, want // 4) + 15) // 16) * 16
    return 0 if (cap * 3 > n_in or n_in > 4096) else cap


def check_ragged(metric: str, mesh_out, mesh_in) -> None:
    if metric != "euclid":
        raise ValueError(f"lengths are defined for per-sample Euclidean meshes only, not for the {metric} metric")
    if mesh_out.dim() != 3 or mesh_in.dim() != 3:
        raise ValueError("lengths need per-sample (batch, n, space_dim) meshes: a batch-free mesh has no per-sample length")
    if mesh_grad_wanted(mesh_out, mesh_in):
        raise NotImplementedError("lengths with a mesh that requires grad: mesh gradients are not implemented for ragged batches")
    if get_math_mode() != "fp32":
        raise NotImplementedError("lengths in the bf16 math mode: ragged batches run in the fp32 math mode only")
    if mesh_out.shape[-1] > 3:
        raise NotImplementedError(f"lengths with space_dim > 3 (got {mesh_out.shape[-1]}): ragged batches take 1 to 3 coordinates")


def mixed_pair(mesh_out, mesh_in):
    if not (torch.is_tensor(mesh_out) and torch.is_tensor(mesh_in)):
        return None
    if mesh_out.dim() == 2 and mesh_in.dim() == 3:
        return "out"
    if mesh_out.dim() == 3 and mesh_in.dim() == 2:
        return "in"
    return None


def check_mixed(metric: str, mesh_out, mesh_in, len_out=None, len_in=None) -> str:
    shared = mixed_pair(mesh_out, mesh_in)
    if (len_out if shared == "out" else len_in) is not None:
        raise ValueError("a length for the mesh shared by the batch: every one of its points is real for every sample - lengths "
                         "belong to the per-sample side only")
    if metric != "euclid":
        if len_out is not None or len_in is not None:
            raise ValueError(f"lengths are defined for per-sample Euclidean meshes only, not for the {metric} metric")
        raise RuntimeError("periodic metrics are defined for batch-free meshes only (pit.py:186-258)")
    if mesh_grad_wanted(mesh_out, mesh_in):
        raise NotImplementedError("a mesh that requires grad in a mixed pair: mesh gradients are not implemented for a shared mesh "
                                  "against per-sample clouds")
    if len_out is not None or len_in is not None:
        if get_math_mode() != "fp32":
            raise NotImplementedError("lengths in the bf16 math mode: ragged batches run in the fp32 math mode only")
        if mesh_out.shape[-1] > 3:
            raise NotImplementedError(f"lengths with space_dim > 3 (got {mesh_out.shape[-1]}): ragged batches take 1 to 3 coordinates")
    return shared


class MeshPlan:

    __slots__ = ("mesh_out", "mesh_in", "mesh_batch", "n_out", "n_in", "sdim", "metric", "metric_id", "period",
                 "rank_k", "rank_w", "masked", "self_attn", "stats", "nbr_idx", "nbr_cnt", "nbr_cap", "rev_ptr",
                 "rev_row", "_complete", "_union", "_slab", "_fold", "len_out", "len_in", "rank_w_dev", "shared", "_rev_sorted")

    def __init__(self, metric: str, mesh_out: torch.Tensor, mesh_in: torch.Tensor, locality: float,
                 self_attn: bool, period: Optional[float] = None, len_out=None, len_in=None):
        self.len_out = self.len_in = self.rank_w_dev = None
        self.shared = mixed_pair(mesh_out, mesh_in)
        if self.shared is not None:
            if metric not in METRIC_ID:
                raise ValueError(f"unknown metric {metric!r}")
            check_mixed(metric, mesh_out, mesh_in, len_out, len_in)
            _need_gpu(mesh_out, mesh_in)
            if mesh_out.shape[-1] != mesh_in.shape[-1]:
                raise RuntimeError("mesh_out and mesh_in must have the same number of coordinates")
            if len_out is None and len_in is None:
                b = (mesh_in if self.shared == "out" else mesh_out).shape[0]
                if self.shared == "out":
                    mesh_out = mesh_out.detach().unsqueeze(0).expand(b, -1, -1).contiguous()
                else:
                    mesh_in = mesh_in.detach().unsqueeze(0).expand(b, -1, -1).contiguous()
        elif len_out is not None or len_in is not None:
            if len_out is None or len_in is None:
                raise ValueError("a ragged plan needs both len_out and len_in")
            if metric not in METRIC_ID:
                raise ValueError(f"unknown metric {metric!r}")
            check_ragged(metric, mesh_out, mesh_in)
        _need_gpu(mesh_out, mesh_in)
        if metric not in METRIC_ID:
            raise ValueError(f"unknown metric {metric!r}")
        ragged_mixed = self.shared is not None and (len_out is not None or len_in is not None)
        if (mesh_out.dim() != mesh_in.dim() and not ragged_mixed) or mesh_out.dim() not in (2, 3) or mesh_in.dim() not in (2, 3):
            raise RuntimeError(f"mesh shapes {tuple(mesh_out.shape)} / {tuple(mesh_in.shape)} not supported")
        if mesh_out.shape[-1] != mesh_in.shape[-1]:
            raise RuntimeError("mesh_out and mesh_in must have the same number of coordinates")
        batched = mesh_out.dim() == 3 or mesh_in.dim() == 3
        if batched and metric != "euclid":
            raise RuntimeError("periodic metrics are defined for batch-free meshes only (pit.py:186-258)")
        if batched and not ragged_mixed and mesh_out.shape[0] != mesh_in.shape[0]:
            raise RuntimeError("batched meshes must share the batch size")
        self.metric = metric
        self.metric_id = METRIC_ID[metric]
        self.mesh_out = mesh_out.detach().contiguous()
        self.mesh_in = self.mesh_out if (self_attn and mesh_in is mesh_out) else mesh_in.detach().contiguous()
        self.mesh_batch = (mesh_out if mesh_out.dim() == 3 else mesh_in).shape[0] if batched else 1
        self.n_out, self.n_in, self.sdim = mesh_out.shape[-2], mesh_in.shape[-2], mesh_out.shape[-1]
        if not 1 <= self.sdim <= MAX_SPACE_DIM:
            raise RuntimeError(f"space_dim must be between 1 and {MAX_SPACE_DIM}, got {self.sdim}")
        self.period = mesh_period(metric, self.mesh_in) if period is None else float(period)
        self.rank_k, self.rank_w = quantile_rank(locality, self.n_in)
        self.masked = bool(locality < 1.0)
        self.self_attn = bool(self_attn)
        self.stats = None
        self.nbr_idx = self.nbr_cnt = self.rev_ptr = self.rev_row = None
        self.nbr_cap = 0
        self._complete = None
        self._rev_sorted = None
        self._union = None
        self._slab = None
        self._fold = None
        if ragged_mixed:
            dev, mb = mesh_out.device, self.mesh_batch
            self.len_out = None if len_out is None else as_lengths(len_out, dev, mb)
            self.len_in = None if len_in is None else as_lengths(len_in, dev, mb)
            self.stats = torch.empty((3, mb, self.n_out), device=dev, dtype=torch.float32)
            self.rank_w_dev = torch.empty((mb,), device=dev, dtype=torch.float32)
            cap = ragged_list_capacity(self.rank_k, self.n_in) if (self.masked and SPARSE_MASKED) else 0
            if cap:
                self.nbr_cap = cap
                self.nbr_idx = torch.empty((mb, self.n_out, cap), device=dev, dtype=torch.int32)
                self.nbr_cnt = torch.empty((mb, self.n_out), device=dev, dtype=torch.int32)
            so, si = self.sample_strides()
            rc = _lib.lib().pit_plan_ragged_strided_fwd(self.mesh_out.data_ptr(), self.mesh_in.data_ptr(), mb, self.n_out,
                                                        self.n_in, self.sdim, so, si, _lib.ptr(self.len_out), _lib.ptr(self.len_in),
                                                        float(np.float32(locality)), 1 if self.masked else 0, self.stats.data_ptr(),
                                                        self.rank_w_dev.data_ptr(), cap, _lib.ptr(self.nbr_idx),
                                                        _lib.ptr(self.nbr_cnt), _lib.stream_ptr())
            _lib.check(rc, "pit_plan_ragged_strided_fwd")
            if cap and torch.is_grad_enabled():
                self.rev_ptr = torch.empty((mb, self.n_in + 1), device=dev, dtype=torch.int32)
                self.rev_row = torch.empty((mb, self.n_out * cap), device=dev, dtype=torch.int32)
                ws = torch.empty((2 * mb * self.n_in,), device=dev, dtype=torch.int32)
                rc = _lib.lib().pit_lists_transpose(self.nbr_idx.data_ptr(), self.nbr_cnt.data_ptr(), mb, self.n_out, self.n_in, cap,
                                                    self.rev_ptr.data_ptr(), self.rev_row.data_ptr(), ws.data_ptr(), _lib.stream_ptr())
                _lib.check(rc, "pit_lists_transpose")
            if _capturing():
                _pin(self.len_out, self.len_in, self.mesh_out, self.mesh_in)
            return
        if len_out is not None:
            self.len_out = as_lengths(len_out, mesh_out.device, self.mesh_batch)
            self.len_in = self.len_out if len_in is len_out else as_lengths(len_in, mesh_out.device, self.mesh_batch)
            dev, mb = mesh_out.device, self.mesh_batch
            self.stats = torch.empty((3, mb, self.n_out), device=dev, dtype=torch.float32)
            self.rank_w_dev = torch.empty((mb,), device=dev, dtype=torch.float32)
            cap = ragged_list_capacity(self.rank_k, self.n_in) if (self.masked and SPARSE_MASKED) else 0
            if cap:
                self.nbr_cap = cap
                self.nbr_idx = torch.empty((mb, self.n_out, cap), device=dev, dtype=torch.int32)
                self.nbr_cnt = torch.empty((mb, self.n_out), device=dev, dtype=torch.int32)
            rc = _lib.lib().pit_plan_ragged_fwd(self.mesh_out.data_ptr(), self.mesh_in.data_ptr(), mb, self.n_out,
                                                self.n_in, self.sdim, self.len_out.data_ptr(), self.len_in.data_ptr(),
                                                float(np.float32(locality)), 1 if self.masked else 0, self.stats.data_ptr(),
                                                self.rank_w_dev.data_ptr(), cap, _lib.ptr(self.nbr_idx), _lib.ptr(self.nbr_cnt),
                                                _lib.stream_ptr())
            _lib.check(rc, "pit_plan_ragged_fwd")
            if cap and torch.is_grad_enabled():
                self.rev_ptr = torch.empty((mb, self.n_in + 1), device=dev, dtype=torch.int32)
                self.rev_row = torch.empty((mb, self.n_out * cap), device=dev, dtype=torch.int32)
                ws = torch.empty((2 * mb * self.n_in,), device=dev, dtype=torch.int32)
                rc = _lib.lib().pit_lists_transpose(self.nbr_idx.data_ptr(), self.nbr_cnt.data_ptr(), mb, self.n_out, self.n_in, cap,
                                                    self.rev_ptr.data_ptr(), self.rev_row.data_ptr(), ws.data_ptr(), _lib.stream_ptr())
                _lib.check(rc, "pit_lists_transpose")
            if _capturing():
                _pin(self.len_out, self.len_in)
            return
        cap = 0
        if self.masked and SPARSE_MASKED:
            want = self.rank_k + 2
            cap = ((want + max(16, want // 4) + 15) // 16) * 16
            if cap * 3 > self.n_in:
                cap = 0
        if self.masked or not self.self_attn:
            self.stats = torch.empty((3, self.mesh_batch, self.n_out), device=mesh_out.device, dtype=torch.float32)
        if cap:
            self._build_lists(cap, self._wants_reverse_lists(cap))
        elif self.stats is not None:
            name = "pit_select_fwd" if self.sdim <= 3 else "pit_select_wide_fwd"
            rc = getattr(_lib.lib(), name)(self.mesh_out.data_ptr(), self.mesh_in.data_ptr(), self.mesh_batch,
                                           self.n_out, self.n_in, self.sdim, self.metric_id, self.period,
                                           self.rank_k, 1 if self.masked else 0, self.stats.data_ptr(),
                                           _lib.stream_ptr())
            _lib.check(rc, name)

    def ragged(self) -> bool:
        return self.len_out is not None or self.len_in is not None

    def sample_strides(self):
        return (0 if self.mesh_out.dim() == 2 else self.n_out, 0 if self.mesh_in.dim() == 2 else self.n_in)

    def _union_key(self, cap):
        return (self.metric, self.n_out, self.n_in, cap, self.mesh_batch > 1, self.sdim)

    def _wants_reverse_lists(self, cap: int) -> bool:
        return self.mesh_batch == 1

    def ensure_reverse_lists(self) -> None:
        if self.nbr_idx is None or self.rev_ptr is not None:
            return
        dev = self.mesh_out.device
        rev_ptr = torch.empty((self.mesh_batch, self.n_in + 1), device=dev, dtype=torch.int32)
        rev_row = torch.empty((self.mesh_batch, self.n_out * self.nbr_cap), device=dev, dtype=torch.int32)
        work = torch.empty((2 * self.mesh_batch * self.n_in,), device=dev, dtype=torch.int32)
        rc = _lib.lib().pit_lists_transpose(self.nbr_idx.data_ptr(), self.nbr_cnt.data_ptr(), self.mesh_batch, self.n_out,
                                            self.n_in, self.nbr_cap, rev_ptr.data_ptr(), rev_row.data_ptr(), work.data_ptr(),
                                            _lib.stream_ptr())
        if rc == -4:
            self._build_lists(self.nbr_cap, True)
            return
        _lib.check(rc, "pit_lists_transpose")
        self.rev_ptr, self.rev_row = rev_ptr, rev_row

    def sorted_reverse_lists(self) -> torch.Tensor:
        if self._rev_sorted is None or self._rev_sorted[0] is not self.rev_row:
            out = self.rev_row.clone()
            rc = _lib.lib().pit_lists_sort_ranges(self.rev_ptr.data_ptr(), self.rev_row.data_ptr(), self.mesh_batch, self.n_in,
                                                  self.n_out * self.nbr_cap, out.data_ptr(), _lib.stream_ptr())
            _lib.check(rc, "pit_lists_sort_ranges")
            self._rev_sorted = (self.rev_row, out)
        return self._rev_sorted[1]

    def union_tiles(self) -> bool:
        if self._union is not None:
            return self._union
        if self.nbr_idx is None or UNION_TILES == "0" or self.n_in > 4096 or self.n_out < 16 or self.nbr_cap > 64 \
                or (self.mesh_batch == 1 and UNION_TILES != "1"):
            self._union = False
            return False
        if UNION_TILES == "1":
            self._union = True
            return True
        key = self._union_key(self.nbr_cap)
        hit = _UNION_DECISIONS.get(key)
        if hit is None:
            if torch.cuda.is_current_stream_capturing():
                return False
            cap, tiles = self.nbr_cap, min(32, self.n_out // 16)
            first = (torch.linspace(0, self.n_out // 16 - 1, tiles).long() * 16).to(self.nbr_idx.device)
            rows = (first[:, None] + torch.arange(16, device=first.device)[None, :]).reshape(-1)
            idx = self.nbr_idx.view(-1, cap)[rows].long()
            cnt = self.nbr_cnt[rows].long()
            keys = torch.where(torch.arange(cap, device=first.device)[None, :] < cnt[:, None], idx, -1).view(tiles, 16 * cap)
            srt = torch.sort(keys, dim=1).values
            union = (srt[:, 1:] != srt[:, :-1]).sum(1) + 1 - (srt[:, 0] < 0).long()
            mean_u, mean_k, over = (float(v) for v in torch.stack(
                [union.float().mean(), cnt.float().mean(), (cnt > cap).float().max()]).tolist())
            hit = over == 0.0 and mean_u <= min(64.0, 4.0 * mean_k)
            _UNION_DECISIONS[key] = hit
        self._union = hit
        return hit

    def slab_plan(self):
        if self._slab is not None:
            return self._slab or None
        if self.nbr_idx is None or self.mesh_batch != 1 or not self.masked or self.n_in > 16384 or self.nbr_cap > 64:
            self._slab = False
            return None
        if torch.cuda.is_current_stream_capturing():
            return None
        dev = self.mesh_out.device
        built = self._build_slab_plan(16)
        if built is None:
            self._slab = False
            return None
        self._slab = built
        return self._slab

    def _build_slab_plan(self, rows: int):
        dev = self.mesh_out.device
        n_slabs = (self.n_out + rows - 1) // rows
        m = torch.empty((n_slabs * rows, self.nbr_cap), device=dev, dtype=torch.float32)
        slot = torch.empty((n_slabs * rows, self.nbr_cap), device=dev, dtype=torch.int16)
        keys = torch.empty((n_slabs, SLAB_UNION_MAX), device=dev, dtype=torch.int32)
        nkeys = torch.empty((n_slabs,), device=dev, dtype=torch.int32)
        report = torch.zeros((3,), device=dev, dtype=torch.int32)
        rc = _lib.lib().pit_slab_plan_build(self.mesh_out.data_ptr(), self.mesh_in.data_ptr(), self.n_out, self.n_in, self.sdim,
                                            self.metric_id, self.period, self.nbr_idx.data_ptr(), self.nbr_cnt.data_ptr(),
                                            self.nbr_cap, rows, m.data_ptr(), slot.data_ptr(), keys.data_ptr(), nkeys.data_ptr(),
                                            report.data_ptr(), _lib.stream_ptr())
        _lib.check(rc, "pit_slab_plan_build")
        max_union, overflowed, max_count = report.tolist()
        if overflowed:
            return None
        sp = _lib.SlabPlan(self.n_out, self.n_in, self.nbr_cap, n_slabs, SLAB_UNION_MAX, self.stats.data_ptr(), self.rank_w,
                           self.nbr_idx.data_ptr(), self.nbr_cnt.data_ptr(), m.data_ptr(), slot.data_ptr(), keys.data_ptr(),
                           nkeys.data_ptr(), rows)
        return (sp, int(max_union), (m, slot, keys, nkeys), max(1, int(max_count)))

    def fold_plan(self):
        if self._fold is not None:
            return self._fold or None
        if self.nbr_idx is None or self.mesh_batch != 1 or not self.masked or self.n_in > 16384 or self.nbr_cap > 64 \
                or self.n_out < 64:
            self._fold = False
            return None
        if torch.cuda.is_current_stream_capturing():
            return None
        for rows in FOLD_SLAB_ROWS:
            built = self._build_slab_plan(rows)
            if built is None:
                break
            if built[1] <= SLAB_UNION_MAX:
                sp, mu, keep, mc = built
                keys, nkeys = keep[2], keep[3]
                n_slabs = keys.shape[0]
                slot = torch.arange(SLAB_UNION_MAX, device=keys.device, dtype=torch.int64)[None, :].expand(n_slabs, -1)
                valid = slot < nkeys[:, None].long()
                ent = (torch.arange(n_slabs, device=keys.device, dtype=torch.int64)[:, None] * SLAB_UNION_MAX + slot)[valid]
                key = keys.long()[valid]
                order = torch.sort(key, stable=True).indices
                rev_ent = ent[order].to(torch.int32).contiguous()
                rev_ptr = torch.zeros((self.n_in + 1,), device=keys.device, dtype=torch.int64)
                rev_ptr[1:] = torch.cumsum(torch.bincount(key, minlength=self.n_in), 0)
                rev_ptr = rev_ptr.to(torch.int32).contiguous()
                self._fold = (sp, mu, keep + (rev_ptr, rev_ent), mc)
                return self._fold
        self._fold = False
        return None

    def lists_complete(self) -> int:
        if self.nbr_cnt is None or self.mesh_batch != 1:
            return 0
        if self._complete is None:
            if torch.cuda.is_current_stream_capturing():
                return 0
            self._complete = int(bool((self.nbr_cnt <= self.nbr_cap).all().item()))
        return self._complete

    def _build_lists(self, cap: int, reverse: bool = True) -> None:
        dev = self.mesh_out.device
        rows = self.mesh_batch * self.n_out
        L = _lib.lib()
        self.nbr_cap = cap
        self.nbr_idx = torch.empty((rows, cap), device=dev, dtype=torch.int32)
        self.nbr_cnt = torch.empty((rows,), device=dev, dtype=torch.int32)
        work = None
        if reverse:
            self.rev_ptr = torch.empty((self.mesh_batch, self.n_in + 1), device=dev, dtype=torch.int32)
            self.rev_row = torch.empty((self.mesh_batch, self.n_out * cap), device=dev, dtype=torch.int32)
            work = torch.empty((2 * self.mesh_batch * self.n_in,), device=dev, dtype=torch.int32)
        rc = L.pit_plan_fwd(self.mesh_out.data_ptr(), self.mesh_in.data_ptr(), self.mesh_batch, self.n_out,
                            self.n_in, self.sdim, self.metric_id, self.period, self.rank_k, self.stats.data_ptr(), cap,
                            self.nbr_idx.data_ptr(), self.nbr_cnt.data_ptr(), _lib.ptr(self.rev_ptr),
                            _lib.ptr(self.rev_row), _lib.ptr(work), int(PLAN_FLAGS), _lib.stream_ptr())
        _lib.check(rc, "pit_plan_fwd")


def _row_view(t: torch.Tensor) -> torch.Tensor:
    if t.dim() != 3:
        raise RuntimeError(f"expected a (batch, points, channels) tensor, got {tuple(t.shape)}")
    if t.stride(2) != 1 or t.stride(1) < t.shape[2]:
        t = t.contiguous()
    return t


UNION_ATT = os.environ.get("PIT_UNION_ATT", "1") != "0"
SATT = os.environ.get("PIT_SATT", "auto")
SATT_TILES = os.environ.get("PIT_SATT_TILES", "1") != "0"
SATT_FUSE_PREP = os.environ.get("PIT_SATT_FUSE_PREP", "1") != "0"
SATT_DW_RIDER = os.environ.get("PIT_SATT_DW_RIDER", "1") != "0"
WIDE_DW_RIDER = os.environ.get("PIT_WIDE_DW_RIDER", "1") != "0"


def _satt_pays(n_pts: int, n_head: int, d: int) -> bool:
    if SATT == "auto":
        return n_pts >= 256
    return SATT not in ("0", "", False)


# ... 95 lines not shown
        if head.numel() != n_head:
            raise RuntimeError("lmda must hold one value per head")
        width = (n_head + (1 if concat else 0)) * d
        out = torch.empty((b, plan.n_out, width), device=values.device, dtype=torch.float32)
        rowstat = torch.empty((b, n_head, plan.n_out, 4), device=values.device, dtype=torch.float32)
        scale = torch.empty((n_head,), device=values.device, dtype=torch.float32)
        entry, extra = ("pit_posatt_ragged_fwd", ()) if plan.shared is None else ("pit_posatt_ragged_strided_fwd", plan.sample_strides())
        rc = getattr(_lib.lib(), entry)(
            plan.mesh_out.data_ptr(), plan.mesh_in.data_ptr(), b, plan.n_out, plan.n_in, plan.sdim, *extra,
            _lib.ptr(plan.len_out), _lib.ptr(plan.len_in),
            values.data_ptr(), d, values.stride(1), values.stride(0),
            head.data_ptr(), n_head, 1 if head_is_scale else 0,
            plan.stats.data_ptr(), plan.rank_w_dev.data_ptr(), 1 if plan.masked else 0,
            out.data_ptr(), out.stride(1), out.stride(0), d if concat else 0, 1 if concat else 0,
            rowstat.data_ptr(), scale.data_ptr(), _lib.ptr(plan.nbr_idx), _lib.ptr(plan.nbr_cnt), plan.nbr_cap,
            MATH_MODES["fp32"], _lib.stream_ptr())
        _lib.check(rc, entry)
        ctx.plan, ctx.n_head, ctx.concat, ctx.head_is_scale = plan, n_head, concat, head_is_scale
        ctx.save_for_backward(values, head, rowstat, scale)
        return out

    @staticmethod
    def backward(ctx, d_out):
        values, head, rowstat, scale = ctx.saved_tensors
        plan, n_head = ctx.plan, ctx.n_head
        b, j, d = values.shape
        d_out = d_out.contiguous()
        _need_gpu(d_out)
        need_v, need_h = ctx.needs_input_grad[0], ctx.needs_input_grad[1]
        d_values = torch.empty((b, j, d), device=values.device, dtype=torch.float32) if need_v else None
        d_head = torch.empty((n_head,), device=values.device, dtype=torch.float32) if need_h else None
        work = _dscale_workspace(values.device, n_head) if need_h else None
        if need_v or need_h:
            entry, extra = ("pit_posatt_ragged_bwd", ()) if plan.shared is None else ("pit_posatt_ragged_strided_bwd", plan.sample_strides())
            rc = getattr(_lib.lib(), entry)(
                plan.mesh_out.data_ptr(), plan.mesh_in.data_ptr(), b, plan.n_out, plan.n_in, plan.sdim, *extra,
                _lib.ptr(plan.len_out), _lib.ptr(plan.len_in),
                values.data_ptr(), d, values.stride(1), values.stride(0),
                head.data_ptr(), n_head, 1 if ctx.head_is_scale else 0, scale.data_ptr(),
                rowstat.data_ptr(), 1 if plan.masked else 0,
                d_out.data_ptr(), d_out.stride(1), d_out.stride(0), d if ctx.concat else 0,
                _lib.ptr(d_values), d, j * d, 1 if ctx.concat else 0,
                _lib.ptr(d_head), 0, _lib.ptr(work), _lib.ptr(plan.nbr_idx), _lib.ptr(plan.nbr_cnt), plan.nbr_cap,
                _lib.ptr(plan.rev_ptr), _lib.ptr(plan.rev_row), MATH_MODES["fp32"], _lib.stream_ptr())
            _lib.check(rc, entry)
        return d_values, d_head, None, None, None, None


class _PosAtt(torch.autograd.Function):

    @staticmethod
    def forward(ctx, values, head, plan: MeshPlan, n_head: int, concat: bool, head_is_scale: bool,
                head_param=None, out_slot=None, coord_dims: int = 0, scale_in=None, out_bf16: bool = False, link=None,
                mesh_out=None, mesh_in=None):
        _need_gpu(values, head)
        ctx.math = _math_code()
        ctx.repro = reproducible_wanted()
        ctx.mesh_grad = mesh_out is not None or mesh_in is not None
        ctx.mesh_same = mesh_out is mesh_in
        ctx.mesh_shapes = (tuple(mesh_out.shape) if mesh_out is not None else None,
                           tuple(mesh_in.shape) if mesh_in is not None else None)
        if ctx.mesh_grad:
            _check_mesh_grad(plan.metric)
            if coord_dims:
                raise RuntimeError("mesh gradients need the coordinate concat materialised (ops.materialize_coords)")
            out_bf16 = False
        out_bf16 = bool(out_bf16 and not concat and plan.nbr_idx is not None and ctx.math == MATH_MODES["bf16"])
        ctx.coord_dims = int(coord_dims)
        ctx.union = ATT_UNION if (plan.masked and plan.nbr_idx is not None and not coord_dims and n_head <= 2
                                  and values.shape[-1] % 8 == 0 and plan.union_tiles()) else 0
        out_buf = out_slot[0].detach() if out_slot else None
        values = _row_view(values)
        b, j, d = values.shape
        d += int(coord_dims)
        if j != plan.n_in:
            raise RuntimeError(f"inputs have {j} points but mesh_in has {plan.n_in}")
        if plan.mesh_batch not in (1, b):
            raise RuntimeError("mesh batch and input batch differ")
        head = head.detach().reshape(-1).contiguous()
        if head.numel() != n_head:
            raise RuntimeError("lmda must hold one value per head")
        ctx.uatt = None
        if UNION_ATT and not ctx.mesh_grad and not ctx.repro and not concat and not coord_dims and out_buf is None and _union_att_ok(plan, n_head, d, b, values):
            w = _new_decoder_weights(plan, head, scale_in, n_head, head_is_scale, True)
            _launch_decoder_weights(w)
            out = torch.empty((b, plan.n_out, n_head * d), device=values.device, dtype=torch.bfloat16 if out_bf16 else torch.float32)
            sp, max_union = plan.slab_plan()[0], plan.slab_plan()[1]
            rc = _lib.lib().pit_union_att_fwd(ctypes.byref(sp), values.data_ptr(), values.stride(1), values.stride(0), b, n_head, d,
                                              w.pw.data_ptr(), out.data_ptr(), out.stride(1), out.stride(0), 1 if out_bf16 else 0,
                                              max_union, _lib.stream_ptr())
            _lib.check(rc, "pit_union_att_fwd")
            ctx.uatt = w
            ctx.plan, ctx.n_head, ctx.concat, ctx.head_is_scale = plan, n_head, concat, head_is_scale
            ctx.head_param = head_param
            ctx.union = 0
            ctx.save_for_backward(values, head, w.scale, w.scale)
            return out
        ctx.satt = None
        if not ctx.mesh_grad and _satt_pays(int(plan.n_in), int(n_head), int(d)) and concat and not coord_dims and plan.self_attn and not plan.masked and ctx.math == MATH_MODES["bf16"] \
                and values.dtype == torch.float32 and values.stride(1) % 4 == 0 and values.stride(0) % 4 == 0 and values.data_ptr() % 16 == 0 \
                and plan.sdim <= 3 and _lib.lib().pit_satt_supported(int(plan.n_in), int(n_head), int(d), int(b), int(plan.mesh_batch)):
            k_head, k_is_scale = (scale_in, True) if scale_in is not None else (head, head_is_scale)
            out = out_buf if out_buf is not None else torch.empty((b, plan.n_out, (n_head + 1) * d), device=values.device, dtype=torch.float32)
            x16 = link.get("x16") if (link is not None and out_buf is not None) else None
            x16_ready = x16 is not None and tuple(x16.shape) == (b * j, d) and x16.dtype == torch.bfloat16 and x16.is_contiguous()
            if not x16_ready:
                x16 = torch.empty((b, j, d), device=values.device, dtype=torch.bfloat16)
            rowstat = torch.empty((plan.mesh_batch, n_head, plan.n_out, 4), device=values.device, dtype=torch.float32)
            scale = torch.empty((n_head,), device=values.device, dtype=torch.float32)
            et = torch.empty((plan.mesh_batch, n_head, int(_lib.lib().pit_satt_tiles_elems(int(plan.n_in)))), device=values.device,
                             dtype=torch.bfloat16) if SATT_TILES else None
            rc = _lib.lib().pit_satt_fwd(plan.mesh_in.data_ptr(), plan.mesh_batch, plan.n_in, plan.sdim, plan.metric_id, plan.period,
                                         values.data_ptr(), values.stride(1), values.stride(0), b, d, k_head.data_ptr(), n_head,
                                         1 if k_is_scale else 0, x16.data_ptr(), out.data_ptr(), out.stride(1), out.stride(0), d,
                                         1 if out_buf is None else 0, rowstat.data_ptr(), scale.data_ptr(), _lib.ptr(et),
                                         1 if x16_ready else 0, _lib.stream_ptr())
            _lib.check(rc, "pit_satt_fwd")
            ctx.satt = x16
            ctx.satt_tiles = et
            ctx.satt_link = link
            if link is not None:
                link.update(rowstat=rowstat, n_head=n_head, pts=int(j), mesh_batch=int(plan.mesh_batch), dim=int(d), batch=int(b), g16=None,
                            dx_ptr=None, dx_version=None)
            ctx.union = 0
            ctx.plan, ctx.n_head, ctx.concat, ctx.head_is_scale = plan, n_head, concat, head_is_scale
            ctx.head_param = head_param
            ctx.save_for_backward(values, head, rowstat, scale)
            return out
        width = (n_head + (1 if concat else 0)) * d
        copy_inputs = 1 if concat else 0
        if out_buf is not None:
            out, copy_inputs = out_buf, 0
        else:
            out = torch.empty((b, plan.n_out, width), device=values.device,
                              dtype=torch.bfloat16 if out_bf16 else torch.float32)
        rowstat = torch.empty((plan.mesh_batch, n_head, plan.n_out, 4), device=values.device, dtype=torch.float32)
        scale = torch.empty((n_head,), device=values.device, dtype=torch.float32)
        k_head, k_is_scale = (scale_in, True) if scale_in is not None else (head, head_is_scale)
        wjob = getattr(_STEP, "fwd_job", None)
        if wjob is not None:
            _STEP.fwd_job = None
        rc = _lib.lib().pit_posatt_fwd_job(
            plan.mesh_out.data_ptr(), plan.mesh_in.data_ptr(), plan.mesh_batch, plan.n_out, plan.n_in, plan.sdim,
            plan.metric_id, plan.period,
            values.data_ptr(), b, d, values.stride(1), values.stride(0),
            k_head.data_ptr(), n_head, 1 if k_is_scale else 0,
            _lib.ptr(plan.stats), plan.rank_w, 1 if plan.masked else 0, 1 if plan.self_attn else 0,
            out.data_ptr(), out.stride(1), out.stride(0), d if concat else 0, copy_inputs,
            rowstat.data_ptr(), scale.data_ptr(),
            _lib.ptr(plan.nbr_idx), _lib.ptr(plan.nbr_cnt), plan.nbr_cap, ctx.coord_dims,
            ctx.math | (IO_OUT_BF16 if out_bf16 else 0) | ctx.union, _lib.stream_ptr(),
            ctypes.cast(ctypes.pointer(wjob.job), ctypes.c_void_p) if wjob is not None else None)
        _lib.check(rc, "pit_posatt_fwd")
        ctx.plan, ctx.n_head, ctx.concat, ctx.head_is_scale = plan, n_head, concat, head_is_scale
        ctx.head_param = head_param
        ctx.save_for_backward(values, head, rowstat, scale)
        return out

    @staticmethod
    def backward(ctx, d_out):
        values, head, rowstat, scale = ctx.saved_tensors
        plan, n_head, concat = ctx.plan, ctx.n_head, ctx.concat
        b, j, dv = values.shape
        d = dv + ctx.coord_dims
        d_out = _row_view(d_out)
        _need_gpu_bf16_ok(d_out)
        io = IO_DOUT_BF16 if d_out.dtype == torch.bfloat16 else 0
# ... 879 lines not shown
                _defer_head_begin(ws)
            else:
                ws = torch.zeros(H * 1024, device=dev, dtype=torch.float64)
            work.append(ws)
        extra = _dw_take(dev)
        slices = []
        if extra is not None:
            st = extra[0]
            if not st.out_gelu and st.accumulate and (st.math_mode & 0xff) == 0:
                slices = _dw_slices(extra, n if ctx.hook is None else max(1, n - ctx.hook[1]))
            else:
                _dw_run(extra)
        w1, _, w2, _ = wts[n - 1]
        rc = L_.pit_mlp_bwd_data(rows, W, D, D, w1.data_ptr(), w2.data_ptr(), z1[n - 1].data_ptr(), z2[n - 1].data_ptr(), 1,
                                 d_out.data_ptr(), D, dxc[n - 1].data_ptr(), W, scratch[n - 1].data_ptr(), ctx.math,
                                 _lib.stream_ptr())
        _lib.check(rc, "pit_mlp_bwd_data")
        for i in range(n - 1, -1, -1):
            dw1, db1, dw2, db2 = w_slots[i]
            job = _lib.MlpParamsJob(bufs[i].data_ptr(), W, rows, W, D, D, hh[i].data_ptr(), 1, scratch[i].data_ptr(), D,
                                    dw1.data_ptr(), db1.data_ptr(), dw2.data_ptr(), db2.data_ptr(), 1,
                                    scratch[i].data_ptr(), ctx.math)
            if i > 0:
                pw1, _, pw2, _ = wts[i - 1]
                prev = (pw1.data_ptr(), pw2.data_ptr(), z1[i - 1].data_ptr(), z2[i - 1].data_ptr(), 1, W,
                        dxc[i - 1].data_ptr(), W, scratch[i - 1].data_ptr(), None, 0)
            else:
                prev = (None, None, None, None, 0, 0, None, 0, None, dx.data_ptr(), D)
            k = n - 1 - i
            job2 = ctypes.cast(ctypes.pointer(slices[k]), ctypes.c_void_p) if k < len(slices) else None
            rc = L_.pit_block_bwd(E[i].data_ptr(), inv[i].data_ptr(), Q[i].data_ptr(), L, H, D, b, dxc[i].data_ptr(),
                                  bufs[i].data_ptr(), work[i].data_ptr(), *prev,
                                  ctypes.cast(ctypes.pointer(job), ctypes.c_void_p), job2, ctx.math,
                                  _lib.stream_ptr())
            _lib.check(rc, "pit_block_bwd")
            if ctx.hook is not None:
                ctx.hook[0](i)
        d_heads = [None] * n
        now = [i for i in range(n) if not defer[i]]
        for i in range(n):
            if defer[i]:
                _defer_head_finish(work[i], lm_slots[i], heads[i], scale[i], H, 1)
        if now:
            m = len(now)
            for i in now:
                d_heads[i] = lm_slots[i] if lm_slots[i] is not None else torch.empty((H,), device=dev, dtype=torch.float32)
            ws = (ctypes.c_void_p * m)(*[work[i].data_ptr() for i in now])
            dh = (ctypes.c_void_p * m)(*[d_heads[i].data_ptr() for i in now])
            hd = (ctypes.c_void_p * m)(*[heads[i].data_ptr() for i in now])
            sc = (ctypes.c_void_p * m)(*[scale[i].data_ptr() for i in now])
            nh = (ctypes.c_int * m)(*[H] * m)
            fl = (ctypes.c_int * m)(*[1 if lm_slots[i] is not None else 0 for i in now])
            _lib.check(L_.pit_posatt_dhead_finish(m, ws, dh, hd, sc, nh, fl, None, _lib.stream_ptr()), "pit_posatt_dhead_finish")
        grads = [dx, None, None, None, None, None]
        for i in range(n):
            g = None if lm_slots[i] is not None else d_heads[i]
            grads.append(g)
        for i in range(n):
            grads.extend(w_grads[i] if w_grads[i] is not None else [None, None, None, None])
        return tuple(grads)




@torch.compiler.disable
def processor_apply(x: torch.Tensor, plan: MeshPlan, n_head: int, lmdas, mlps, early=None) -> torch.Tensor:
    scales = None
    if get_head_scale_route() == "host":
        scales = [host_head_scale(p) for p in lmdas]
    flat = [p.reshape(-1) for p in lmdas] + [t for m in mlps for t in m]
    return _Processor.apply(x, plan, n_head, scales, (tuple(lmdas), tuple(tuple(m) for m in mlps)), early, *flat)


EDGE_FUSION = os.environ.get("PIT_EDGE_FUSION", "1") != "0"


def edge_fusion_supported(plan: MeshPlan, n_head: int, dim: int, batch: int, needs_union: bool) -> bool:
    if not EDGE_FUSION or plan.mesh_batch != 1 or plan.self_attn or not plan.masked or plan.nbr_idx is None or plan.sdim > 3:
        return False
    if needs_union and torch.are_deterministic_algorithms_enabled():
        return False
    if not _lib.lib().pit_edge_supported(int(n_head), int(dim), int(batch), int(plan.n_out)):
        return False
    sp = plan.slab_plan()
    return sp is not None and (not needs_union or sp[1] <= SLAB_UNION_MAX)


def _finish_heads_now(work, d_head, head, scale, n_head: int, flags: int) -> None:
    one = lambda t: (ctypes.c_void_p * 1)(_lib.ptr(t))
    rc = _lib.lib().pit_posatt_dhead_finish(1, one(work), one(d_head), one(head), one(scale), (ctypes.c_int * 1)(n_head),
                                            (ctypes.c_int * 1)(flags), None, _lib.stream_ptr())
    _lib.check(rc, "pit_posatt_dhead_finish")


def _mlp_grad_slots(params, shapes, needs, device):
    slots = [_grad_slot(p) if isinstance(p, torch.nn.Parameter) else None for p in params]
    if all(s is not None for s in slots) and all(needs):
        return slots, True
    return [torch.zeros(tuple(sh), device=device, dtype=torch.float32) for sh in shapes], False


class LossSpec:
    __slots__ = ("true", "scale", "shift", "p", "out_dim", "seed", "partials", "pred", "token", "value")

    def __init__(self, true, scale, shift, out_dim: int, p: int, seed=None):
        b = true.size(0)
        self.true = true.reshape(b, -1, out_dim).contiguous()
        npts = self.true.shape[1]
        self.scale = scale.reshape(npts, out_dim).contiguous() if scale is not None else None
        self.shift = shift.reshape(npts, out_dim).contiguous() if shift is not None else None
        self.p, self.out_dim, self.seed = int(p), int(out_dim), seed
        self.partials = self.pred = self.token = self.value = None

    def fits(self, batch: int, npts: int, n2: int) -> bool:
        return self.p in (1, 2) and n2 == self.out_dim and tuple(self.true.shape) == (batch, npts, n2) and not self.true.requires_grad


class DecoderWeights:
    __slots__ = ("key", "pw", "qw", "scale", "job", "keep", "w1f")


def _dec_weights_key(plan: MeshPlan, lmda, scale_in, n_head: int, head_is_scale: bool, w1=None):
    return (id(plan), n_head, _PARAM_EPOCH[0], lmda._version, lmda.data_ptr(), bool(head_is_scale),
            scale_in.data_ptr() if scale_in is not None else None,
            (w1.data_ptr(), w1._version, tuple(w1.shape)) if w1 is not None else None)


def _new_decoder_weights(plan: MeshPlan, lmda, scale_in, n_head: int, head_is_scale: bool, need_q: bool, w1=None) -> DecoderWeights:
    sp, max_union, _t, max_count = plan.slab_plan()
    um = 32 if max_union <= 32 else (48 if max_union <= 48 else 64)
    dev = plan.mesh_out.device
    w = DecoderWeights()
    w.key = _dec_weights_key(plan, lmda, scale_in, n_head, head_is_scale, w1)
    w1c = w1.detach() if (w1 is not None and w1.is_contiguous() and w1.dtype == torch.float32 and w1.dim() == 2
                          and w1.shape[0] % 16 == 0 and w1.shape[1] == n_head * w1.shape[0] and w1.data_ptr() % 16 == 0) else None
    w.w1f = torch.empty_like(w1c) if w1c is not None else None
    w.pw = torch.empty((sp.n_slabs, n_head, 16, um), device=dev, dtype=torch.float32)
    w.qw = torch.empty((sp.n_slabs, n_head, 16, um), device=dev, dtype=torch.float32) if need_q else None
    w.scale = torch.empty((n_head,), device=dev, dtype=torch.float32)
    head = scale_in if scale_in is not None else lmda.detach().reshape(-1).contiguous()
    w.keep = (head, plan, sp, w1c)
    w.job = _lib.DecoderWeightsJob(ctypes.cast(ctypes.pointer(sp), ctypes.c_void_p), head.data_ptr(),
                                   1 if (scale_in is not None or head_is_scale) else 0, n_head, max_union, max_count,
                                   w.pw.data_ptr(), _lib.ptr(w.qw), w.scale.data_ptr(),
                                   _lib.ptr(w1c), _lib.ptr(w.w1f), w1c.shape[0] if w1c is not None else 0)
    return w


def _launch_decoder_weights(w: DecoderWeights) -> None:
    j = w.job
    rc = _lib.lib().pit_decoder_weights(j.plan, j.head, j.head_is_scale, j.n_head, j.max_union, j.max_count, j.pw, j.qw,
                                        j.scale_out, j.w1, j.w1f, j.dim, _lib.stream_ptr())
    _lib.check(rc, "pit_decoder_weights")


def early_decoder_weights(plan: MeshPlan, lmda, n_head: int, need_q: bool, w1=None) -> None:
    scale_in = host_head_scale(lmda) if get_head_scale_route() == "host" else None
    _STEP.dec_job = _new_decoder_weights(plan, lmda, scale_in, n_head, False, need_q, w1)
    _STEP.dec_ready = None


class _Decoder(torch.autograd.Function):

    @staticmethod
    def forward(ctx, values, head, plan: MeshPlan, n_head: int, head_is_scale: bool, head_param, weights, params, loss, w1, b1, w2, b2):
        _need_gpu(values, head, w1, b1, w2, b2)
        values = _row_view(values)
        if values.stride(1) % 4 or values.stride(0) % 4 or values.data_ptr() % 16:
            values = values.contiguous()
        b, j, d = values.shape
        n2 = w2.shape[0]
        dev = values.device
        sp = plan.slab_plan()[0]
        head = head.detach().reshape(-1).contiguous()
        w1c, b1c, w2c, b2c = (t.detach().contiguous() for t in (w1, b1, w2, b2))
        rows = b * plan.n_out
        need = weights.qw is not None
        y = torch.empty((b, plan.n_out, n2), device=dev, dtype=torch.float32)
        x = z1 = h = dvals = None
        if need:
            x = torch.empty((rows, n_head * d), device=dev, dtype=torch.float32)
            z1 = torch.empty((rows, d), device=dev, dtype=torch.float32)
            h = torch.empty((rows, d), device=dev, dtype=torch.float32)
            dvals = torch.empty((b, j, d), device=dev, dtype=torch.float32)
        lt = ls = lh = lpart = None
        lp = 0
        if loss is not None and need:
            lt, ls, lh, lp = loss.true, loss.scale, loss.shift, loss.p
            lpart = loss.partials = torch.empty((b, n2, sp.n_slabs, 2), device=dev, dtype=torch.float64)
            loss.value = torch.empty((), device=dev, dtype=torch.float32)
        w1f = weights.w1f if (weights.w1f is not None and weights.keep[3].data_ptr() == w1c.data_ptr()) else None
        rc = _lib.lib().pit_decoder_fwd(ctypes.byref(sp), values.data_ptr(), values.stride(1), values.stride(0), b, n_head, d,
                                        weights.pw.data_ptr(), w1c.data_ptr(), _lib.ptr(w1f), b1c.data_ptr(), w2c.data_ptr(),
                                        b2c.data_ptr(), n2, _lib.ptr(x), _lib.ptr(z1), _lib.ptr(h), y.data_ptr(),
                                        _lib.ptr(dvals), dvals.numel() if dvals is not None else 0,
                                        _lib.ptr(lt), _lib.ptr(ls), _lib.ptr(lh), lp, _lib.ptr(lpart), plan.slab_plan()[1],
                                        _lib.stream_ptr())
        _lib.check(rc, "pit_decoder_fwd")
        ctx.plan, ctx.n_head, ctx.head_is_scale, ctx.head_param, ctx.params = plan, n_head, head_is_scale, head_param, params
        ctx.loss = loss if lpart is not None else None
        if ctx.loss is not None:
            loss.pred = y
        ctx.dvals_clean = True
        ctx.keep = (values, head, w1c, w2c, x, z1, h, weights, dvals)
        return y

    @staticmethod
    def backward(ctx, d_y):
        values, head, w1, w2, x, z1, h, weights, dvals = ctx.keep
        scale = weights.scale
        plan, n_head = ctx.plan, ctx.n_head
        b, j, d = values.shape
        n2, rows = w2.shape[0], b * plan.n_out
        dev = values.device
        sp = plan.slab_plan()[0]
        loss = ctx.loss
        inside = loss is not None and loss.token is not None and d_y.data_ptr() == loss.token.data_ptr()
        if loss is not None and loss.token is not None and not inside:
            raise RuntimeError("the fused loss's gradient token reached pit.decoder's backward as a copy: the prediction must reach "
                               "the loss through views only (engine.TrainStep)")
        if not ctx.dvals_clean:
            dvals.zero_()
        ctx.dvals_clean = False
        dz1 = torch.empty((rows, d), device=dev, dtype=torch.float32)
        if inside:
            d_pred = torch.empty((rows, n2), device=dev, dtype=torch.float32)
            dyp, ld = None, n2
        else:
            d_pred = d_y.reshape(rows, n2)
            if d_pred.stride(1) != 1 or d_pred.stride(0) < n2:
                d_pred = d_pred.contiguous()
            dyp, ld = d_pred, d_pred.stride(0)
        need_h = ctx.needs_input_grad[1]
        slot = _grad_slot(ctx.head_param) if need_h else None
        defer = DEFER_HEAD_FINISH and slot is not None
        work = None
        if need_h:
            work = _layer_workspace(slot, n_head) if defer else torch.zeros(n_head * 1024, device=dev, dtype=torch.float64)
            if defer:
                _defer_head_begin(work)
        L = _lib.lib()
        rc = L.pit_decoder_bwd(ctypes.byref(sp), values.data_ptr(), values.stride(1), values.stride(0), b, n_head, d,
                               weights.pw.data_ptr(), weights.qw.data_ptr(), w1.data_ptr(), w2.data_ptr(), n2, z1.data_ptr(),
                               _lib.ptr(dyp), ld, dz1.data_ptr(), dvals.data_ptr(), dvals.stride(0), _lib.ptr(work),
                               loss.pred.data_ptr() if inside else None, _lib.ptr(loss.true) if inside else None,
                               _lib.ptr(loss.scale) if inside else None, _lib.ptr(loss.shift) if inside else None,
                               _lib.ptr(loss.seed) if inside else None, loss.p if inside else 0,
                               _lib.ptr(loss.partials) if inside else None, d_pred.data_ptr() if inside else None,
                               loss.value.data_ptr() if inside else None, None, plan.slab_plan()[1], _lib.stream_ptr())
        _lib.check(rc, "pit_decoder_bwd")
        d_head = None
        if need_h:
            flags = 1 | (4 if ctx.head_is_scale else 0)
            if defer:
                _defer_head_finish(work, slot, head, scale, n_head, flags)
            else:
                d_head = slot if slot is not None else torch.empty((n_head,), device=dev, dtype=torch.float32)
                _finish_heads_now(work, d_head, head, scale, n_head, flags if slot is not None else flags & ~1)
                if slot is not None:
                    d_head = None
        grads, inplace = _mlp_grad_slots(ctx.params, (w1.shape, (d,), w2.shape, (n2,)), ctx.needs_input_grad[9:13], dev)
        d_w1, d_b1, d_w2, d_b2 = grads
        st = _lib.MlpParamsJob(x.data_ptr(), x.stride(0), rows, n_head * d, d, n2, h.data_ptr(), 0, d_pred.data_ptr(),
                               d_pred.stride(0), d_w1.data_ptr(), d_b1.data_ptr(), d_w2.data_ptr(), d_b2.data_ptr(), 1,
                               dz1.data_ptr(), 0)
        keep = (x, h, d_pred, dz1, d_w1, d_b1, d_w2, d_b2)
        if inplace and MLP_PARAMS_RIDER and _dw_deferrable(rows, n_head * d, d, n2, 0, d_pred.stride(0)):
            _dw_defer(st, keep, dev)
        else:
            _dw_run((st, keep, torch.cuda.current_stream(dev)))
        dv = dvals if ctx.needs_input_grad[0] else None
        w = (None, None, None, None) if inplace else (d_w1, d_b1, d_w2, d_b2)
        return (dv, d_head, None, None, None, None, None, None, None) + w


@torch.compiler.disable
def decoder_apply(values: torch.Tensor, lmda: torch.Tensor, plan: MeshPlan, n_head: int, mlp, head_is_scale: bool = False) -> torch.Tensor:
    param = lmda if isinstance(lmda, torch.nn.Parameter) else None
    c = host_head_scale(lmda) if (not head_is_scale and get_head_scale_route() == "host") else None
    need_q = torch.is_grad_enabled() and (values.requires_grad or lmda.requires_grad or any(t.requires_grad for t in mlp))
    weights = getattr(_STEP, "dec_ready", None)
    _STEP.dec_ready = None
    if weights is None or weights.key != _dec_weights_key(plan, lmda, c, n_head, head_is_scale, mlp[0]) or (need_q and weights.qw is None):
        weights = _new_decoder_weights(plan, lmda, c, n_head, head_is_scale, need_q, mlp[0])
        _launch_decoder_weights(weights)
    loss = getattr(_STEP, "loss", None)
    if loss is not None:
        _STEP.loss = None
        if not loss.fits(values.shape[0], plan.n_out, mlp[2].shape[0]):
            loss = None
        else:
            _STEP.loss_issued = loss
    return _Decoder.apply(values, lmda.reshape(-1), plan, n_head, head_is_scale, param, weights, tuple(mlp), loss, *mlp)


FOLD_DECODER = os.environ.get("PIT_FOLD_DECODER", "1") != "0"
FOLD_TILES = os.environ.get("PIT_FOLD_TILES", "auto")
FOLD_TILES_MAX_BYTES = 64 << 20


def _fold_tiles(nbytes: int) -> bool:
    if FOLD_TILES in ("0", False):
        return False
    return FOLD_TILES in ("1", True) or nbytes <= FOLD_TILES_MAX_BYTES or torch.are_deterministic_algorithms_enabled()
FOLD_EDGE_ROWS = int(os.environ.get("PIT_FOLD_EDGE_ROWS", "300000"))
_ZERO_BIAS = {}


def _zero_bias(n: int, device) -> torch.Tensor:
    key = (device.index, n)
    z = _ZERO_BIAS.get(key)
    if z is None:
        z = _ZERO_BIAS[key] = torch.zeros((n,), device=device, dtype=torch.float32)
        _pin(z)
    return z


def _rows2d(t: torch.Tensor) -> torch.Tensor:
    t = _row_view(t)
    if t.stride(0) != t.shape[1] * t.stride(1) or t.stride(1) % 4 or t.data_ptr() % 16:
        t = t.contiguous()
    return t


class _Linear(torch.autograd.Function):

    @staticmethod
    def forward(ctx, x, w, w_param):
        _need_gpu(x, w)
        x = _rows2d(x)
        b, j, d = x.shape
        wc = w.detach()
# ... 650 lines not shown
```

Baseline: 55000 samples/s.

## Group decoder slab rows into 2D grid patches and prune union keys by rank threshold

Decoder slabs now cover 2D rectangular patches of the row-major output grid instead of contiguous row ranges. Spatially compact patches share more latent neighbours, which shrinks the per-slab key union and allows a smaller 16-slot union buffer. The plan build also drops neighbours beyond the per-row quantile threshold from the union, so fewer keys are staged in shared memory and fewer redundant products are computed. The cost is extra index arithmetic for every row mapping, a new plan-build path, and the risk that the threshold pruning marks neighbours invalid (slot 65535) in a way that must match the kernel's mask exactly.

```diff
diff --git a/include/pit_hip.h b/include/pit_hip.h
--- a/include/pit_hip.h
+++ b/include/pit_hip.h
@@ -139,11 +139,17 @@
     const int* idx; const int* cnt;
     const float* m; const unsigned short* slot; const int* keys; const int* nkeys;
     int rows;
+    int grid_w, grid_h, patch_w, patch_h;
 } pit_slab_plan;
 int pit_slab_plan_build(const float* mesh_out, const float* mesh_in, int n_out, int n_in, int space_dim, int metric, float period,
                         const int* nbr_idx, const int* nbr_cnt, int cap, int rows_per_slab, float* m, unsigned short* slot,
                         int* keys, int* nkeys, int* report, void* stream);
+int pit_slab_plan_build_patch(const float* mesh_out, const float* mesh_in, int n_out, int n_in, int space_dim, int metric,
+                              float period, const int* nbr_idx, const int* nbr_cnt, int cap, int grid_w, int grid_h, int patch_w,
+                              int patch_h, const float* stats, float rank_w, float* m, unsigned short* slot, int* keys, int* nkeys,
+                              int* report, void* stream);
 int pit_edge_supported(int n_head, int dim, int batch, int rows_per_sample);
+int pit_decoder_union_slots(const pit_slab_plan* plan, int max_union);
 int pit_decoder_weights(const pit_slab_plan* plan, const float* head, int head_is_scale, int n_head, int max_union, int max_count,
                         float* pw, float* qw, float* scale_out, const float* w1, float* w1f, int dim, void* stream);
 typedef struct pit_decoder_weights_job {
diff --git a/position_induced_transformer_amd/_lib.py b/position_induced_transformer_amd/_lib.py
--- a/position_induced_transformer_amd/_lib.py
+++ b/position_induced_transformer_amd/_lib.py
@@ -27,7 +27,8 @@
 
 class SlabPlan(ctypes.Structure):
     _fields_ = [("n_out", _I), ("n_in", _I), ("cap", _I), ("n_slabs", _I), ("umax", _I), ("stats", _P), ("rank_w", _F),
-                ("idx", _P), ("cnt", _P), ("m", _P), ("slot", _P), ("keys", _P), ("nkeys", _P), ("rows", _I)]
+                ("idx", _P), ("cnt", _P), ("m", _P), ("slot", _P), ("keys", _P), ("nkeys", _P), ("rows", _I),
+                ("grid_w", _I), ("grid_h", _I), ("patch_w", _I), ("patch_h", _I)]
 
 
 class DecoderWeightsJob(ctypes.Structure):
@@ -76,6 +77,8 @@
     "pit_block_weights": [_P, _I, _I, _I, _F, _I, _P, _I, _I, _P, _P, _P, _P, _P, _P],
     "pit_block_fwd": [_P, _P, _I, _I, _I, _I, _P, _P, _P, _P, _P, _I, _P, _P, _P, _P, _L, _I, _P],
     "pit_slab_plan_build": [_P, _P, _I, _I, _I, _I, _F, _P, _P, _I, _I, _P, _P, _P, _P, _P, _P],
+    "pit_decoder_union_slots": [_P, _I],
+    "pit_slab_plan_build_patch": [_P, _P, _I, _I, _I, _I, _F, _P, _P, _I, _I, _I, _I, _I, _P, _F, _P, _P, _P, _P, _P, _P],
     "pit_fold_supported": [_I, _I, _I, _I, _I],
     "pit_fold_weights": [_P, _P, _I, _I, _I, _I, _P, _P, _P, _P, _P, _P],
     "pit_fold_att_fwd": [_P, _P, _L, _L, _I, _I, _I, _P, _P, _L, _L, _I, _I, _P],
diff --git a/position_induced_transformer_amd/csrc/pit_edge.hip b/position_induced_transformer_amd/csrc/pit_edge.hip
--- a/position_induced_transformer_amd/csrc/pit_edge.hip
+++ b/position_induced_transformer_amd/csrc/pit_edge.hip
@@ -40,12 +40,28 @@
     return p == 1 ? ax : ax * ax;
 }
 
+struct SlabGeo { int i0, j0, sh, gw, gh; };
+__device__ __forceinline__ SlabGeo slab_geo(const pit_slab_plan& p, int slab) {
+    SlabGeo g;
+    g.sh = 31 - __clz(p.patch_w);
+    const int ppr = (p.grid_w + p.patch_w - 1) >> g.sh, pi = slab / ppr;
+    g.i0 = pi * p.patch_h; g.j0 = (slab - pi * ppr) << g.sh; g.gw = p.grid_w; g.gh = p.grid_h;
+    return g;
+}
+__device__ __forceinline__ int slab_row(const SlabGeo& g, int r, bool& ok) {
+    const int i = g.i0 + (r >> g.sh), j = g.j0 + (r & ((1 << g.sh) - 1));
+    ok = i < g.gh && j < g.gw;
+    return i * g.gw + j;
+}
+
 struct SlabBuildArgs {
     const float *mesh_out, *mesh_in;
     int n_out, n_in, sdim, used, periodic; float period;
     const int *idx, *cnt; int cap, umax;
     float* m; unsigned short* slot; int* keys; int* nkeys; int* report;
     int er;
+    pit_slab_plan geo;
+    const float* stats; float rank_w;
 };
 
 __global__ __launch_bounds__(256) void slab_plan_kernel(SlabBuildArgs a) {
@@ -57,11 +73,13 @@
     __syncthreads();
     const int er = a.er;
     const int total = er * a.cap;
+    const SlabGeo sg = slab_geo(a.geo, slab);
     for (int e = tid; e < total; e += 256) {
         const int r = e / a.cap, i = e - r * a.cap;
-        const int row = slab * er + r;
+        bool rok;
+        const int row = slab_row(sg, r, rok);
         float mv = 0.0f;
-        if (row < a.n_out) {
+        if (rok) {
             const int c = a.cnt[row];
             if (c > a.cap && i == 0) atomicMax(a.report + 1, 1);
             if (i == 0) atomicMax(a.report + 2, min(c, a.cap));
@@ -71,7 +89,12 @@
                 const float* xi = a.mesh_in + (long)j * a.sdim;
                 mv = sq_dist3(xo[0], a.used > 1 ? xo[1] : 0.0f, a.used > 2 ? xo[2] : 0.0f,
                               xi[0], a.used > 1 ? xi[1] : 0.0f, a.used > 2 ? xi[2] : 0.0f, a.periodic != 0, a.period);
-                atomicOr(&bm[j >> 5], 1u << (j & 31));
+                bool joins = true;
+                if (a.stats) {
+                    const float mk = a.stats[row], mk1 = a.stats[a.n_out + row];
+                    joins = mv <= quantile_lerp(mk, mk1, a.rank_w) + mk1 * 0x1p-20f;
+                }
+                if (joins) atomicOr(&bm[j >> 5], 1u << (j & 31));
             }
         }
         a.m[(long)(slab * er + r) * a.cap + i] = mv;
@@ -99,11 +122,12 @@
     for (int s = nk + tid; s < a.umax; s += 256) a.keys[(long)slab * a.umax + s] = 0;
     for (int e = tid; e < total; e += 256) {
         const int r = e / a.cap, i = e - r * a.cap;
-        const int row = slab * er + r;
+        bool rok;
+        const int row = slab_row(sg, r, rok);
         int s = 0;
-        if (row < a.n_out && i < min(a.cnt[row], a.cap)) {
+        if (rok && i < min(a.cnt[row], a.cap)) {
             const int j = a.idx[(long)row * a.cap + i];
-            s = pref[j >> 5] + __popc(bm[j >> 5] & ((1u << (j & 31)) - 1u));
+            s = (bm[j >> 5] >> (j & 31) & 1u) ? pref[j >> 5] + __popc(bm[j >> 5] & ((1u << (j & 31)) - 1u)) : 65535;
         }
         a.slot[(long)(slab * er + r) * a.cap + i] = (unsigned short)min(s, 65535);
     }
@@ -146,14 +170,17 @@
     }
     __syncthreads();
     const int rpw = 64 / lpr;
+    const SlabGeo sg = slab_geo(p, slab);
     for (int r0 = 0; r0 < ER; r0 += 4 * rpw) {
-        const int row_l = r0 + wave * rpw + lane / lpr, i = lane % lpr, n = slab * ER + row_l;
-        const int craw = ldi_if(p.cnt, n, n < p.n_out);
+        const int row_l = r0 + wave * rpw + lane / lpr, i = lane % lpr;
+        bool rok;
+        const int n = slab_row(sg, row_l, rok);
+        const int craw = ldi_if(p.cnt, n, rok);
         const long off = (long)(slab * ER + row_l) * p.cap + (i < p.cap ? i : 0);
         const float m = p.m[off];
         const int slot = p.slot[off];
         const bool valid = i < min(craw, p.cap);
-        const int nn = n < p.n_out ? n : p.n_out - 1;
+        const int nn = rok ? n : p.n_out - 1;
         const float mk = p.stats[nn], mk1 = p.stats[p.n_out + nn], mmin = p.stats[2 * (long)p.n_out + nn];
         for (int h = 0; h < H; ++h) {
             const float T = quantile_lerp(__fmul_rn(c[h], mk), __fmul_rn(c[h], mk1), p.rank_w);
@@ -279,7 +306,10 @@
     int b, slab;
     if (!slab_of_xcd(blockIdx.x, g.batch, p.n_slabs, b, slab)) return;
     const int nk = min(p.nkeys[slab], EU), nkup = (nk + 15) & ~15;
-    const long row0 = (long)b * p.n_out + slab * ER;
+    const long rowb = (long)b * p.n_out;
+    const SlabGeo sg = slab_geo(p, slab);
+    bool rv;
+    const int n = slab_row(sg, l15, rv);
     const int c1 = wave * 16 + l15;
     ESTAMP(0, 0);
     int key[EU / 16];
@@ -298,9 +328,7 @@
     const float b2r = ldg_if(g.b2, tid, tid < g.n2);
     float l_t0 = 0.0f, l_sc0 = 1.0f, l_sh0 = 0.0f;
     if (LOSS) {
-        const int n = slab * ER + l15;
-        const bool rv = n < p.n_out;
-        l_t0 = ldg_if(g.tru, (row0 + l15) * g.n2, rv);
+        l_t0 = ldg_if(g.tru, (rowb + n) * g.n2, rv);
         const bool aff = rv && g.lscale != nullptr;
         l_sc0 = ldg_if(g.lscale, (long)n * g.n2, aff);
         l_sh0 = ldg_if(g.lshift, (long)n * g.n2, aff);
@@ -330,8 +358,10 @@
 #pragma unroll
         for (int u = 0; u < (ER * K0 / 4 + NT - 1) / NT; ++u) {
             const int e = tid + u * NT, r = e / (K0 / 4), q = e % (K0 / 4);
-            if (e < ER * K0 / 4 && slab * ER + r < p.n_out)
-                *reinterpret_cast<float4*>(g.x + (row0 + r) * K0 + 4 * q) = *reinterpret_cast<const float4*>(xs + r * XP + 4 * q);
+            bool ok;
+            const int nr = slab_row(sg, r, ok);
+            if (e < ER * K0 / 4 && ok)
+                *reinterpret_cast<float4*>(g.x + (rowb + nr) * K0 + 4 * q) = *reinterpret_cast<const float4*>(xs + r * XP + 4 * q);
         }
     }
     {
@@ -349,7 +379,9 @@
             const int r = 4 * kq + i;
             const float z = a0[i] + a1[i] + bias1;
             hs[r * HP + c1] = gelu_erf(z);
-            if (g.z1 && slab * ER + r < p.n_out && !(PIT_EDGE_DBG & 4)) g.z1[(row0 + r) * D + c1] = z;
+            bool ok;
+            const int nr = slab_row(sg, r, ok);
+            if (g.z1 && ok && !(PIT_EDGE_DBG & 4)) g.z1[(rowb + nr) * D + c1] = z;
         }
     }
     ESTAMP(0, 7);
@@ -357,8 +389,10 @@
     ESTAMP(0, 8);
     if (g.h && !(PIT_EDGE_DBG & (4 | 1024))) {
         const int r = tid / (D / 4), q = tid % (D / 4);
-        if (slab * ER + r < p.n_out)
-            *reinterpret_cast<float4*>(g.h + (row0 + r) * D + 4 * q) = *reinterpret_cast<const float4*>(hs + r * HP + 4 * q);
+        bool ok;
+        const int nr = slab_row(sg, r, ok);
+        if (ok)
+            *reinterpret_cast<float4*>(g.h + (rowb + nr) * D + 4 * q) = *reinterpret_cast<const float4*>(hs + r * HP + 4 * q);
     }
     if (wave != 0) {
         if (g.zero_buf) {
@@ -372,8 +406,6 @@
         }
         return;
     }
-    const int n = slab * ER + l15;
-    const bool rv = n < p.n_out;
 #pragma unroll
     for (int o = 0; o < 4; ++o) {
         if (o >= g.n2) break;
@@ -387,12 +419,12 @@
         part += __shfl_xor(part, 16, 64);
         part += __shfl_xor(part, 32, 64);
         const float pred = part + w2s[4 * D + o];
-        if (kq == 0 && rv) g.y[(row0 + l15) * g.n2 + o] = pred;
+        if (kq == 0 && rv) g.y[(rowb + n) * g.n2 + o] = pred;
         if (LOSS) {
             double num = 0.0, den = 0.0;
             float t = l_t0, sc = l_sc0, sh = l_sh0;
             if (o > 0) {
-                t = ldg_if(g.tru, (row0 + l15) * g.n2 + o, rv);
+                t = ldg_if(g.tru, (rowb + n) * g.n2 + o, rv);
                 sc = ldg_if(g.lscale, (long)n * g.n2 + o, rv && g.lscale != nullptr);
                 sh = ldg_if(g.lshift, (long)n * g.n2 + o, rv && g.lscale != nullptr);
             }
@@ -454,7 +486,8 @@
     int b, slab;
     if (!slab_of_xcd(blockIdx.x, g.batch, p.n_slabs, b, slab)) return;
     const int nk = min(p.nkeys[slab], EU), nkup = (nk + 15) & ~15;
-    const long row0 = (long)b * p.n_out + slab * ER;
+    const long rowb = (long)b * p.n_out;
+    const SlabGeo sg = slab_geo(p, slab);
     const int c1 = wave * 16 + l15;
 
     ESTAMP(1, 0);
@@ -470,17 +503,17 @@
     const float w2c0 = g.w2[ec];
 #pragma unroll
     for (int u = 0; u < 4; ++u) {
-        const int r = (tid + u * NT) / D;
-        const bool ok = slab * ER + r < p.n_out;
-        z1v[u] = ldg_if(g.z1, (row0 + r) * D + ec, ok);
+        bool ok;
+        const int n = slab_row(sg, (tid + u * NT) / D, ok);
+        z1v[u] = ldg_if(g.z1, (rowb + n) * D + ec, ok);
         dyv[u] = 0.0f; prv[u] = 0.0f; trv[u] = 0.0f; lsc[u] = 1.0f; lsh[u] = 0.0f;
         if (!LOSS) {
-            dyv[u] = ldg_if(g.d_y, (row0 + r) * g.ld_dy, ok);
+            dyv[u] = ldg_if(g.d_y, (rowb + n) * g.ld_dy, ok);
         } else {
-            prv[u] = ldg_if(g.pred, (row0 + r) * g.n2, ok);
-            trv[u] = ldg_if(g.tru, (row0 + r) * g.n2, ok);
+            prv[u] = ldg_if(g.pred, (rowb + n) * g.n2, ok);
+            trv[u] = ldg_if(g.tru, (rowb + n) * g.n2, ok);
             const bool aff = ok && g.lscale != nullptr;
-            const float a = ldg_if(g.lscale, (long)(slab * ER + r) * g.n2, aff), bq = ldg_if(g.lshift, (long)(slab * ER + r) * g.n2, aff);
+            const float a = ldg_if(g.lscale, (long)n * g.n2, aff), bq = ldg_if(g.lshift, (long)n * g.n2, aff);
             lsc[u] = g.lscale ? a : 1.0f;
             lsh[u] = bq;
         }
@@ -541,12 +574,12 @@
     float acc[4];
 #pragma unroll
     for (int u = 0; u < 4; ++u) {
-        const int r = (tid + u * NT) / D;
-        const bool ok = slab * ER + r < p.n_out;
+        bool ok;
+        const int n = slab_row(sg, (tid + u * NT) / D, ok);
         float v = dyv[u];
         if (LOSS) {
             v = dpred(prv[u], trv[u], lsc[u], lsh[u], nrm0, nrm1);
-            if (ec == 0 && ok) g.d_pred[(row0 + r) * g.n2] = v;
+            if (ec == 0 && ok) g.d_pred[(rowb + n) * g.n2] = v;
         }
         acc[u] = v * w2c0;
     }
@@ -560,18 +593,18 @@
         }
 #pragma unroll
         for (int u = 0; u < 4; ++u) {
-            const int r = (tid + u * NT) / D;
-            const bool ok = slab * ER + r < p.n_out;
+            bool ok;
+            const int n = slab_row(sg, (tid + u * NT) / D, ok);
             float v;
             if (!LOSS) {
-                v = ldg_if(g.d_y, (row0 + r) * g.ld_dy + o, ok);
+                v = ldg_if(g.d_y, (rowb + n) * g.ld_dy + o, ok);
             } else {
-                const long e = (long)(slab * ER + r) * g.n2 + o;
+                const long e = (long)n * g.n2 + o;
                 const bool aff = ok && g.lscale != nullptr;
                 const float a = ldg_if(g.lscale, e, aff), bq = ldg_if(g.lshift, e, aff);
-                v = dpred(ldg_if(g.pred, (row0 + r) * g.n2 + o, ok), ldg_if(g.tru, (row0 + r) * g.n2 + o, ok),
+                v = dpred(ldg_if(g.pred, (rowb + n) * g.n2 + o, ok), ldg_if(g.tru, (rowb + n) * g.n2 + o, ok),
                           g.lscale ? a : 1.0f, bq, nn, dn);
-                if (ec == o && ok) g.d_pred[(row0 + r) * g.n2 + o] = v;
+                if (ec == o && ok) g.d_pred[(rowb + n) * g.n2 + o] = v;
             }
             acc[u] += v * w2o;
         }
@@ -579,10 +612,11 @@
 #pragma unroll
     for (int u = 0; u < 4; ++u) {
         const int r = (tid + u * NT) / D;
-        const bool ok = slab * ER + r < p.n_out;
+        bool ok;
+        const int n = slab_row(sg, r, ok);
         const float v = ok ? acc[u] * ((PIT_EDGE_DBG & 32) ? 1.0f : gelu_erf_grad(z1v[u])) : 0.0f;
         ds1[r * P1 + ec] = v;
-        if (ok && !(PIT_EDGE_DBG & 512)) g.dz1[(row0 + r) * D + ec] = v;
+        if (ok && !(PIT_EDGE_DBG & 512)) g.dz1[(rowb + n) * D + ec] = v;
     }
     ESTAMP(1, 4);
     park_union<D>(ut, nkup, tid, uv);
@@ -1093,16 +1127,31 @@
     }
 }
 
-bool plan_ok(const pit_slab_plan* p, bool needs_union) {
+bool patch_ok(int n_out, int rows, int gw, int gh, int pw, int ph) {
+    return gw > 0 && gh > 0 && pw > 0 && ph > 0 && (pw & (pw - 1)) == 0 && (long)gw * gh == n_out && pw * ph == rows;
+}
+int patch_slabs(int gw, int gh, int pw, int ph) { return ((gh + ph - 1) / ph) * ((gw + pw - 1) / pw); }
+bool plan_ok(const pit_slab_plan* p, bool needs_union, bool patches = false) {
     if (!p || !p->stats || !p->idx || !p->cnt || !p->m) return false;
     if (p->rows != ER) return false;
-    if (p->n_out <= 0 || p->n_in <= 0 || p->cap <= 0 || p->cap > 64 || p->n_slabs != (p->n_out + ER - 1) / ER) return false;
+    if (p->n_out <= 0 || p->n_in <= 0 || p->cap <= 0 || p->cap > 64) return false;
+    if (p->patch_w != 0) {
+        if (!patches || !patch_ok(p->n_out, ER, p->grid_w, p->grid_h, p->patch_w, p->patch_h) ||
+            p->n_slabs != patch_slabs(p->grid_w, p->grid_h, p->patch_w, p->patch_h)) return false;
+    } else if (p->n_slabs != (p->n_out + ER - 1) / ER) return false;
     if (needs_union && (!p->slot || !p->keys || !p->nkeys || p->umax != EU)) return false;
     return true;
 }
+pit_slab_plan slab_geometry(const pit_slab_plan& plan, int rows) {
+    pit_slab_plan p = plan;
+    if (p.patch_w == 0) { p.grid_w = p.n_out; p.grid_h = 1; p.patch_w = rows; p.patch_h = 1; }
+    return p;
+}
 bool hid_ok(int n_head, int dim) { return (n_head == 1 || n_head == 2) && (dim == 32 || dim == 64); }
 
-int union_slots(int max_union) { return max_union <= 32 ? 32 : (max_union <= 48 ? 48 : 64); }
+int union_slots(int max_union, bool patches = false) {
+    return (patches && max_union <= 16) ? 16 : (max_union <= 32 ? 32 : (max_union <= 48 ? 48 : 64));
+}
 template <int H, int D>
 size_t dec_fwd_smem(int um) { return (size_t)(H * ER * (um + 4) + um * (D + 4) + ER * (H * D + 4) + ER * (D + 4) + 4 * D + 4) * 4; }
 template <int H, int D>
@@ -1118,12 +1167,12 @@
     return rows >= 256 && rows <= PIT_EDGE_MAX_ROWS;
 }
 
-extern "C" int pit_slab_plan_build(const float* mesh_out, const float* mesh_in, int n_out, int n_in, int space_dim, int metric,
-                                   float period, const int* nbr_idx, const int* nbr_cnt, int cap, int rows_per_slab, float* m,
-                                   unsigned short* slot, int* keys, int* nkeys, int* report, void* stream) {
-    if (!mesh_out || !mesh_in || !nbr_idx || !nbr_cnt || !m || !slot || !keys || !nkeys || !report) return PIT_ERR_NULL;
+namespace {
+int slab_plan_launch(const float* mesh_out, const float* mesh_in, int n_out, int n_in, int space_dim, int metric, float period,
+                     const int* nbr_idx, const int* nbr_cnt, int cap, int rows_per_slab, int grid_w, int grid_h, int patch_w,
+                     int patch_h, const float* stats, float rank_w, float* m, unsigned short* slot, int* keys, int* nkeys,
+                     int* report, void* stream) {
     if (n_out <= 0 || n_in <= 0 || n_in > 16384 || space_dim < 1 || space_dim > 3 || cap <= 0) return PIT_ERR_SIZE;
-    if (rows_per_slab != 16 && rows_per_slab != 64 && rows_per_slab != 128 && rows_per_slab != 256) return PIT_ERR_SIZE;
     if (metric < PIT_METRIC_EUCLID || metric > PIT_METRIC_PERIODIC2D) return PIT_ERR_METRIC;
     SlabBuildArgs a;
     a.mesh_out = mesh_out; a.mesh_in = mesh_in; a.n_out = n_out; a.n_in = n_in; a.sdim = space_dim;
@@ -1131,9 +1180,32 @@
     a.periodic = metric != PIT_METRIC_EUCLID; a.period = period;
     a.idx = nbr_idx; a.cnt = nbr_cnt; a.cap = cap; a.umax = EU;
     a.m = m; a.slot = slot; a.keys = keys; a.nkeys = nkeys; a.report = report; a.er = rows_per_slab;
-    hipLaunchKernelGGL(slab_plan_kernel, dim3((unsigned)((n_out + rows_per_slab - 1) / rows_per_slab)), dim3(256), 0, (hipStream_t)stream, a);
+    a.geo = pit_slab_plan();
+    a.geo.grid_w = grid_w; a.geo.grid_h = grid_h; a.geo.patch_w = patch_w; a.geo.patch_h = patch_h;
+    a.stats = stats; a.rank_w = rank_w;
+    hipLaunchKernelGGL(slab_plan_kernel, dim3((unsigned)patch_slabs(grid_w, grid_h, patch_w, patch_h)), dim3(256), 0, (hipStream_t)stream, a);
     PIT_CHECK_LAUNCH();
     return 0;
+}
+}
+
+extern "C" int pit_slab_plan_build(const float* mesh_out, const float* mesh_in, int n_out, int n_in, int space_dim, int metric,
+                                   float period, const int* nbr_idx, const int* nbr_cnt, int cap, int rows_per_slab, float* m,
+                                   unsigned short* slot, int* keys, int* nkeys, int* report, void* stream) {
+    if (!mesh_out || !mesh_in || !nbr_idx || !nbr_cnt || !m || !slot || !keys || !nkeys || !report) return PIT_ERR_NULL;
+    if (rows_per_slab != 16 && rows_per_slab != 64 && rows_per_slab != 128 && rows_per_slab != 256) return PIT_ERR_SIZE;
+    return slab_plan_launch(mesh_out, mesh_in, n_out, n_in, space_dim, metric, period, nbr_idx, nbr_cnt, cap, rows_per_slab,
+                            n_out, 1, rows_per_slab, 1, nullptr, 0.0f, m, slot, keys, nkeys, report, stream);
+}
+
+extern "C" int pit_slab_plan_build_patch(const float* mesh_out, const float* mesh_in, int n_out, int n_in, int space_dim, int metric,
+                                         float period, const int* nbr_idx, const int* nbr_cnt, int cap, int grid_w, int grid_h,
+                                         int patch_w, int patch_h, const float* stats, float rank_w, float* m,
+                                         unsigned short* slot, int* keys, int* nkeys, int* report, void* stream) {
+    if (!mesh_out || !mesh_in || !nbr_idx || !nbr_cnt || !stats || !m || !slot || !keys || !nkeys || !report) return PIT_ERR_NULL;
+    if (n_out <= 0 || !patch_ok(n_out, ER, grid_w, grid_h, patch_w, patch_h)) return PIT_ERR_SIZE;
+    return slab_plan_launch(mesh_out, mesh_in, n_out, n_in, space_dim, metric, period, nbr_idx, nbr_cnt, cap, ER,
+                            grid_w, grid_h, patch_w, patch_h, stats, rank_w, m, slot, keys, nkeys, report, stream);
 }
 
 #define PIT_EDGE_DISPATCH(H_, D_, CALL_)                                         \
@@ -1147,17 +1219,23 @@
 namespace {
 int fill_dec_weights(DecWArgs& g, const pit_slab_plan* plan, const float* head, int head_is_scale, int n_head, int max_union,
                      int max_count, float* pw, float* qw, float* scale_out, const float* w1, float* w1f, int dim) {
-    if (!plan_ok(plan, true) || !head || !pw) return PIT_ERR_NULL;
+    if (!plan_ok(plan, true, true) || !head || !pw) return PIT_ERR_NULL;
     if ((w1 == nullptr) != (w1f == nullptr)) return PIT_ERR_NULL;
     if (w1f && (dim < 16 || dim % 16 != 0 || !aligned16(w1) || !aligned16(w1f))) return PIT_ERR_SIZE;
     g.w1 = w1; g.w1f = w1f; g.dim = dim; g.rb = ER;
     if ((n_head != 1 && n_head != 2) || max_union < 1 || max_union > EU || max_count < 1 || max_count > 64) return PIT_ERR_UNSUPPORTED;
     if (!aligned16(pw) || (qw && !aligned16(qw))) return PIT_ERR_SIZE;
-    g.p = *plan; g.head = head; g.head_is_scale = head_is_scale; g.n_head = n_head; g.um = union_slots(max_union);
+    g.p = slab_geometry(*plan, ER); g.head = head; g.head_is_scale = head_is_scale; g.n_head = n_head;
+    g.um = union_slots(max_union, plan->patch_w != 0);
     g.lpr = max_count <= 16 ? 16 : (max_count <= 32 ? 32 : 64);
     g.pw = pw; g.qw = qw; g.scale_out = scale_out;
     return 0;
 }
+}
+
+extern "C" int pit_decoder_union_slots(const pit_slab_plan* plan, int max_union) {
+    if (!plan || max_union < 1 || max_union > EU) return PIT_ERR_UNSUPPORTED;
+    return union_slots(max_union, plan->patch_w != 0);
 }
 
 extern "C" int pit_decoder_weights(const pit_slab_plan* plan, const float* head, int head_is_scale, int n_head, int max_union,
@@ -1176,11 +1254,12 @@
     if (!plan || !plan->stats || !plan->idx || !plan->cnt || !plan->m || !plan->slot || !plan->keys || !plan->nkeys || !head || !pw)
         return PIT_ERR_NULL;
     if ((plan->rows != 64 && plan->rows != 128 && plan->rows != 256) || plan->umax != EU || plan->cap <= 0 || plan->cap > 64 ||
-        plan->n_slabs != (plan->n_out + plan->rows - 1) / plan->rows) return PIT_ERR_SIZE;
+        plan->n_slabs != (plan->n_out + plan->rows - 1) / plan->rows || plan->patch_w != 0) return PIT_ERR_SIZE;
     if ((n_head != 1 && n_head != 2) || max_union < 1 || max_union > EU || max_count < 1 || max_count > 64) return PIT_ERR_UNSUPPORTED;
     if (!aligned16(pw) || (qw && !aligned16(qw))) return PIT_ERR_SIZE;
     DecWArgs g = DecWArgs();
-    g.p = *plan; g.head = head; g.head_is_scale = head_is_scale; g.n_head = n_head; g.um = union_slots(max_union);
+    g.p = slab_geometry(*plan, ER);
+    g.head = head; g.head_is_scale = head_is_scale; g.n_head = n_head; g.um = union_slots(max_union);
     g.lpr = max_count <= 16 ? 16 : (max_count <= 32 ? 32 : 64);
     g.pw = pw; g.qw = qw; g.scale_out = scale_out; g.rb = plan->rows; g.pw16 = pw16; g.qw16 = qw16;
     hipLaunchKernelGGL(decoder_weights_kernel, dim3((unsigned)(plan->n_slabs * (plan->rows / ER))), dim3(256), 0, (hipStream_t)stream, g);
@@ -1196,18 +1275,18 @@
                                int max_union, void* stream) {
     if (max_union < 1 || max_union > EU) return PIT_ERR_UNSUPPORTED;
     if (w1f && !aligned16(w1f)) return PIT_ERR_SIZE;
-    if (!plan_ok(plan, true) || !values || !pw || !w1 || !b1 || !w2 || !b2 || !y) return PIT_ERR_NULL;
+    if (!plan_ok(plan, true, true) || !values || !pw || !w1 || !b1 || !w2 || !b2 || !y) return PIT_ERR_NULL;
     if (!hid_ok(n_head, dim) || n2 < 1 || n2 > 4 || batch <= 0) return PIT_ERR_UNSUPPORTED;
     if ((z1 == nullptr) != (h == nullptr)) return PIT_ERR_NULL;
     if (ld_values % 4 || values_bstride % 4 || !aligned16(values) || !aligned16(w1) || !aligned16(pw) || (zero_buf && !aligned16(zero_buf)))
         return PIT_ERR_SIZE;
     if (loss_part && (!loss_true || (loss_p != 1 && loss_p != 2) || (loss_scale == nullptr) != (loss_shift == nullptr))) return PIT_ERR_UNSUPPORTED;
     DecFwdArgs g;
-    g.p = *plan; g.values = values; g.ld_values = ld_values; g.values_bstride = values_bstride; g.batch = batch;
+    g.p = slab_geometry(*plan, ER); g.values = values; g.ld_values = ld_values; g.values_bstride = values_bstride; g.batch = batch;
     g.pw = pw; g.w1 = w1; g.w1f = w1f; g.b1 = b1; g.w2 = w2; g.b2 = b2; g.n2 = n2;
     g.x = x; g.z1 = z1; g.h = h; g.y = y; g.zero_buf = zero_buf; g.zero_n = zero_buf ? zero_n : 0;
     g.tru = loss_true; g.lscale = loss_scale; g.lshift = loss_shift; g.loss_p = loss_p; g.lpart = loss_part;
-    g.um = union_slots(max_union);
+    g.um = union_slots(max_union, plan->patch_w != 0);
     const dim3 grid((unsigned)slab_grid(batch, plan->n_slabs));
     hipStream_t s = (hipStream_t)stream;
 #define PIT_DF(H_, D_)                                                                                                                \
@@ -1229,19 +1308,19 @@
                                const float* loss_seed, int loss_p, const double* loss_part, float* d_pred, float* loss_out,
                                float* norms_out, int max_union, void* stream) {
     if (max_union < 1 || max_union > EU) return PIT_ERR_UNSUPPORTED;
-    if (!plan_ok(plan, true) || !values || !pw || !qw || !w1 || !w2 || !z1 || !dz1 || !d_values) return PIT_ERR_NULL;
+    if (!plan_ok(plan, true, true) || !values || !pw || !qw || !w1 || !w2 || !z1 || !dz1 || !d_values) return PIT_ERR_NULL;
     if (!hid_ok(n_head, dim) || n2 < 1 || n2 > 4 || batch <= 0) return PIT_ERR_UNSUPPORTED;
     if (!d_y && (!loss_pred || !loss_true || !loss_part || !d_pred || !loss_out || (loss_p != 1 && loss_p != 2) ||
                  (loss_scale == nullptr) != (loss_shift == nullptr))) return PIT_ERR_NULL;
     if (d_y && ld_dy < n2) return PIT_ERR_SIZE;
     if (ld_values % 4 || values_bstride % 4 || !aligned16(values) || !aligned16(pw) || !aligned16(qw)) return PIT_ERR_SIZE;
     DecBwdArgs g;
-    g.p = *plan; g.values = values; g.ld_values = ld_values; g.values_bstride = values_bstride; g.batch = batch;
+    g.p = slab_geometry(*plan, ER); g.values = values; g.ld_values = ld_values; g.values_bstride = values_bstride; g.batch = batch;
     g.pw = pw; g.qw = qw; g.w1 = w1; g.w2 = w2; g.n2 = n2; g.z1 = z1; g.d_y = d_y; g.ld_dy = ld_dy;
     g.dz1 = dz1; g.d_values = d_values; g.dvalues_bstride = dvalues_bstride; g.dscale = dscale;
     g.pred = loss_pred; g.tru = loss_true; g.lscale = loss_scale; g.lshift = loss_shift; g.gseed = loss_seed; g.loss_p = loss_p;
     g.lpart = loss_part; g.d_pred = d_pred; g.loss_out = loss_out; g.norms_out = norms_out;
-    g.um = union_slots(max_union);
+    g.um = union_slots(max_union, plan->patch_w != 0);
     const dim3 grid((unsigned)slab_grid(batch, plan->n_slabs));
     hipStream_t s = (hipStream_t)stream;
 #define PIT_DB(H_, D_)                                                                                                            \
diff --git a/position_induced_transformer_amd/csrc/pit_fold.hip b/position_induced_transformer_amd/csrc/pit_fold.hip
--- a/position_induced_transformer_amd/csrc/pit_fold.hip
+++ b/position_induced_transformer_amd/csrc/pit_fold.hip
@@ -434,7 +434,8 @@
 bool fold_plan_ok(const pit_slab_plan* p) {
     if (!p || !p->stats || !p->idx || !p->cnt || !p->m || !p->slot || !p->keys || !p->nkeys) return false;
     if (p->rows != 64 && p->rows != 128 && p->rows != 256) return false;
-    return p->n_out > 0 && p->n_in > 0 && p->cap > 0 && p->cap <= 64 && p->umax == EU && p->n_slabs == (p->n_out + p->rows - 1) / p->rows;
+    return p->n_out > 0 && p->n_in > 0 && p->cap > 0 && p->cap <= 64 && p->umax == EU && p->patch_w == 0 &&
+           p->n_slabs == (p->n_out + p->rows - 1) / p->rows;
 }
 int union_slots(int max_union) { return max_union <= 32 ? 32 : (max_union <= 48 ? 48 : 64); }
 
diff --git a/position_induced_transformer_amd/ops.py b/position_induced_transformer_amd/ops.py
--- a/position_induced_transformer_amd/ops.py
+++ b/position_induced_transformer_amd/ops.py
@@ -304,6 +304,28 @@
 
 SLAB_UNION_MAX = 64
 FOLD_SLAB_ROWS = (256, 128, 64)
+PATCH_SLABS = os.environ.get("PIT_PATCH_SLABS", "1") != "0"
+PATCH_W = PATCH_H = 4
+
+
+def row_major_grid(mesh: torch.Tensor):
+    if not torch.is_tensor(mesh) or mesh.dim() != 2 or mesh.shape[1] != 2 or mesh.shape[0] < 16 or not mesh.dtype.is_floating_point:
+        return None
+    m = mesh.detach().cpu()
+    n = m.shape[0]
+    moved = (m[:, 1] != m[0, 1]).nonzero()
+    if moved.numel() == 0:
+        return None
+    gw = int(moved[0])
+    if gw < 4 or n % gw or n // gw < 4:
+        return None
+    gh = n // gw
+    g = m.view(gh, gw, 2)
+    xs, ys = g[0, :, 0], g[:, 0, 1]
+    if not (bool((g[:, :, 0] == xs[None, :]).all()) and bool((g[:, :, 1] == ys[:, None]).all())):
+        return None
+    mono = lambda v: bool((v[1:] > v[:-1]).all()) or bool((v[1:] < v[:-1]).all())
+    return (gw, gh) if mono(xs) and mono(ys) else None
 PLAN_FLAGS = 0
 UNION_TILES = os.environ.get("PIT_UNION_TILES", "auto")
 UNION_DV = os.environ.get("PIT_UNION_DV", "auto")
@@ -383,7 +405,7 @@
 
     __slots__ = ("mesh_out", "mesh_in", "mesh_batch", "n_out", "n_in", "sdim", "metric", "metric_id", "period",
                  "rank_k", "rank_w", "masked", "self_attn", "stats", "nbr_idx", "nbr_cnt", "nbr_cap", "rev_ptr",
-                 "rev_row", "_complete", "_union", "_slab", "_fold", "len_out", "len_in", "rank_w_dev", "shared", "_rev_sorted")
+                 "rev_row", "_complete", "_union", "_slab", "_patch", "_fold", "len_out", "len_in", "rank_w_dev", "shared", "_rev_sorted")
 
     def __init__(self, metric: str, mesh_out: torch.Tensor, mesh_in: torch.Tensor, locality: float,
                  self_attn: bool, period: Optional[float] = None, len_out=None, len_in=None):
@@ -440,6 +462,7 @@
         self._rev_sorted = None
         self._union = None
         self._slab = None
+        self._patch = None
         self._fold = None
         if ragged_mixed:
             dev, mb = mesh_out.device, self.mesh_batch
@@ -581,7 +604,18 @@
         self._union = hit
         return hit
 
-    def slab_plan(self):
+    def slab_plan(self, patch: bool = False):
+        if patch and PATCH_SLABS and self._patch is not False and not (self._patch is None and torch.cuda.is_current_stream_capturing()):
+            if self._patch is None:
+                self._patch = False
+                eligible = not (self.nbr_idx is None or self.mesh_batch != 1 or not self.masked or self.n_in > 16384 or self.nbr_cap > 64)
+                grid = row_major_grid(self.mesh_out) if eligible else None
+                if grid is not None:
+                    built = self._build_slab_plan(16, grid + (PATCH_W, PATCH_H))
+                    if built is not None and built[1] <= SLAB_UNION_MAX:
+                        self._patch = built
+            if self._patch:
+                return self._patch
         if self._slab is not None:
             return self._slab or None
         if self.nbr_idx is None or self.mesh_batch != 1 or not self.masked or self.n_in > 16384 or self.nbr_cap > 64:
@@ -597,25 +631,36 @@
         self._slab = built
         return self._slab
 
-    def _build_slab_plan(self, rows: int):
+    def _build_slab_plan(self, rows: int, geo=None):
         dev = self.mesh_out.device
-        n_slabs = (self.n_out + rows - 1) // rows
+        if geo is not None:
+            gw, gh, pw, ph = geo
+            n_slabs = -(-gh // ph) * -(-gw // pw)
+        else:
+            n_slabs = (self.n_out + rows - 1) // rows
         m = torch.empty((n_slabs * rows, self.nbr_cap), device=dev, dtype=torch.float32)
         slot = torch.empty((n_slabs * rows, self.nbr_cap), device=dev, dtype=torch.int16)
         keys = torch.empty((n_slabs, SLAB_UNION_MAX), device=dev, dtype=torch.int32)
         nkeys = torch.empty((n_slabs,), device=dev, dtype=torch.int32)
         report = torch.zeros((3,), device=dev, dtype=torch.int32)
-        rc = _lib.lib().pit_slab_plan_build(self.mesh_out.data_ptr(), self.mesh_in.data_ptr(), self.n_out, self.n_in, self.sdim,
-                                            self.metric_id, self.period, self.nbr_idx.data_ptr(), self.nbr_cnt.data_ptr(),
-                                            self.nbr_cap, rows, m.data_ptr(), slot.data_ptr(), keys.data_ptr(), nkeys.data_ptr(),
-                                            report.data_ptr(), _lib.stream_ptr())
+        if geo is not None:
+            rc = _lib.lib().pit_slab_plan_build_patch(self.mesh_out.data_ptr(), self.mesh_in.data_ptr(), self.n_out, self.n_in,
+                                                      self.sdim, self.metric_id, self.period, self.nbr_idx.data_ptr(),
+                                                      self.nbr_cnt.data_ptr(), self.nbr_cap, gw, gh, pw, ph, self.stats.data_ptr(),
+                                                      self.rank_w, m.data_ptr(), slot.data_ptr(), keys.data_ptr(),
+                                                      nkeys.data_ptr(), report.data_ptr(), _lib.stream_ptr())
+        else:
+            rc = _lib.lib().pit_slab_plan_build(self.mesh_out.data_ptr(), self.mesh_in.data_ptr(), self.n_out, self.n_in, self.sdim,
+                                                self.metric_id, self.period, self.nbr_idx.data_ptr(), self.nbr_cnt.data_ptr(),
+                                                self.nbr_cap, rows, m.data_ptr(), slot.data_ptr(), keys.data_ptr(), nkeys.data_ptr(),
+                                                report.data_ptr(), _lib.stream_ptr())
         _lib.check(rc, "pit_slab_plan_build")
         max_union, overflowed, max_count = report.tolist()
         if overflowed:
             return None
         sp = _lib.SlabPlan(self.n_out, self.n_in, self.nbr_cap, n_slabs, SLAB_UNION_MAX, self.stats.data_ptr(), self.rank_w,
                            self.nbr_idx.data_ptr(), self.nbr_cnt.data_ptr(), m.data_ptr(), slot.data_ptr(), keys.data_ptr(),
-                           nkeys.data_ptr(), rows)
+                           nkeys.data_ptr(), rows, *(geo or (0, 0, 0, 0)))
         return (sp, int(max_union), (m, slot, keys, nkeys), max(1, int(max_count)))
 
     def fold_plan(self):
@@ -877,7 +922,7 @@
             raise RuntimeError("lmda must hold one value per head")
         ctx.uatt = None
         if UNION_ATT and not ctx.mesh_grad and not ctx.repro and not concat and not coord_dims and out_buf is None and _union_att_ok(plan, n_head, d, b, values):
-            w = _new_decoder_weights(plan, head, scale_in, n_head, head_is_scale, True)
+            w = _new_decoder_weights(plan, head, scale_in, n_head, head_is_scale, True, patch=False)
             _launch_decoder_weights(w)
             out = torch.empty((b, plan.n_out, n_head * d), device=values.device, dtype=torch.bfloat16 if out_bf16 else torch.float32)
             sp, max_union = plan.slab_plan()[0], plan.slab_plan()[1]
@@ -1923,7 +1968,7 @@
         return False
     if not _lib.lib().pit_edge_supported(int(n_head), int(dim), int(batch), int(plan.n_out)):
         return False
-    sp = plan.slab_plan()
+    sp = plan.slab_plan(patch=needs_union)
     return sp is not None and (not needs_union or sp[1] <= SLAB_UNION_MAX)
 
 
@@ -1958,7 +2003,7 @@
 
 
 class DecoderWeights:
-    __slots__ = ("key", "pw", "qw", "scale", "job", "keep", "w1f")
+    __slots__ = ("key", "pw", "qw", "scale", "job", "keep", "w1f", "slab", "max_union")
 
 
 def _dec_weights_key(plan: MeshPlan, lmda, scale_in, n_head: int, head_is_scale: bool, w1=None):
@@ -1967,12 +2012,14 @@
             (w1.data_ptr(), w1._version, tuple(w1.shape)) if w1 is not None else None)
 
 
-def _new_decoder_weights(plan: MeshPlan, lmda, scale_in, n_head: int, head_is_scale: bool, need_q: bool, w1=None) -> DecoderWeights:
-    sp, max_union, _t, max_count = plan.slab_plan()
-    um = 32 if max_union <= 32 else (48 if max_union <= 48 else 64)
+def _new_decoder_weights(plan: MeshPlan, lmda, scale_in, n_head: int, head_is_scale: bool, need_q: bool, w1=None,
+                         patch: bool = True) -> DecoderWeights:
+    sp, max_union, _t, max_count = plan.slab_plan(patch)
+    um = _lib.lib().pit_decoder_union_slots(ctypes.byref(sp), max_union)
     dev = plan.mesh_out.device
     w = DecoderWeights()
     w.key = _dec_weights_key(plan, lmda, scale_in, n_head, head_is_scale, w1)
+    w.slab, w.max_union = sp, max_union
     w1c = w1.detach() if (w1 is not None and w1.is_contiguous() and w1.dtype == torch.float32 and w1.dim() == 2
                           and w1.shape[0] % 16 == 0 and w1.shape[1] == n_head * w1.shape[0] and w1.data_ptr() % 16 == 0) else None
     w.w1f = torch.empty_like(w1c) if w1c is not None else None
@@ -2012,7 +2059,7 @@
         b, j, d = values.shape
         n2 = w2.shape[0]
         dev = values.device
-        sp = plan.slab_plan()[0]
+        sp = weights.slab
         head = head.detach().reshape(-1).contiguous()
         w1c, b1c, w2c, b2c = (t.detach().contiguous() for t in (w1, b1, w2, b2))
         rows = b * plan.n_out
@@ -2035,7 +2082,7 @@
                                         weights.pw.data_ptr(), w1c.data_ptr(), _lib.ptr(w1f), b1c.data_ptr(), w2c.data_ptr(),
                                         b2c.data_ptr(), n2, _lib.ptr(x), _lib.ptr(z1), _lib.ptr(h), y.data_ptr(),
                                         _lib.ptr(dvals), dvals.numel() if dvals is not None else 0,
-                                        _lib.ptr(lt), _lib.ptr(ls), _lib.ptr(lh), lp, _lib.ptr(lpart), plan.slab_plan()[1],
+                                        _lib.ptr(lt), _lib.ptr(ls), _lib.ptr(lh), lp, _lib.ptr(lpart), weights.max_union,
                                         _lib.stream_ptr())
         _lib.check(rc, "pit_decoder_fwd")
         ctx.plan, ctx.n_head, ctx.head_is_scale, ctx.head_param, ctx.params = plan, n_head, head_is_scale, head_param, params
@@ -2054,7 +2101,7 @@
         b, j, d = values.shape
         n2, rows = w2.shape[0], b * plan.n_out
         dev = values.device
-        sp = plan.slab_plan()[0]
+        sp = weights.slab
         loss = ctx.loss
         inside = loss is not None and loss.token is not None and d_y.data_ptr() == loss.token.data_ptr()
         if loss is not None and loss.token is not None and not inside:
@@ -2088,7 +2135,7 @@
                                _lib.ptr(loss.scale) if inside else None, _lib.ptr(loss.shift) if inside else None,
                                _lib.ptr(loss.seed) if inside else None, loss.p if inside else 0,
                                _lib.ptr(loss.partials) if inside else None, d_pred.data_ptr() if inside else None,
-                               loss.value.data_ptr() if inside else None, None, plan.slab_plan()[1], _lib.stream_ptr())
+                               loss.value.data_ptr() if inside else None, None, weights.max_union, _lib.stream_ptr())
         _lib.check(rc, "pit_decoder_bwd")
         d_head = None
         if need_h:
```

Measured after the change: 55850 samples/s (median of 6 runs). 1.5% higher.
